# acg-team/ProGraphMSA

Hardware: AMD Instinct MI355X
Metric: DP cell-updates/sec (GCUPS) + wall-clock on 256 seqs × 1000 aa, WAG (higher is better)
Workload: dtype f32

## Files before the change

include/pgm_hip.h:

```cpp
#ifndef PGM_HIP_H_
#define PGM_HIP_H_

#include <stdint.h>
#include <stddef.h>

#ifdef __cplusplus
extern "C" {
#endif

#define PGM_OK 0
#define PGM_ERR_INVALID 1
#define PGM_ERR_DEVICE 2
#define PGM_ERR_BACKTRACK 3
#define PGM_ERR_NOMEM 4

#define PGM_GAP 0xFFFFFFFFu


typedef struct pgm_graph {
    uint32_t n;
    uint32_t dim;
    const double *sites;
    const int32_t *e_rowptr;
    const uint32_t *e_col;
    const float *e_val;
    const int32_t *r_rowptr;
    const uint32_t *r_col;
    const uint32_t *r_units;
} pgm_graph;

typedef struct pgm_model {
    const double *M;
    const double *pi;
} pgm_model;

typedef struct pgm_scores {
    float gap_init, gap_extend, match_init, end_match, end_gap, end_skip;
    float start_gap, start_init, repeat_init, repeat_ext;
} pgm_scores;

typedef struct pgm_align_out {
    float score;
    uint32_t n_tr_indels;
    uint32_t len;
    int32_t status;
    uint32_t *map1;
    uint32_t *map2;
} pgm_align_out;

typedef struct pgm_ctx pgm_ctx;
typedef struct pgm_align_batch pgm_align_batch;

int pgm_device_count(void);
int pgm_ctx_create(int device, pgm_ctx **out);
void pgm_ctx_destroy(pgm_ctx *ctx);
const char *pgm_last_error(void);
int pgm_ctx_device_info(pgm_ctx *ctx, char *name, size_t name_len, int *cu_count);

int pgm_align_graphs_batch(pgm_ctx *ctx, uint32_t njobs, const pgm_graph *const *g1,
                           const pgm_graph *const *g2, const pgm_model *const *model,
                           const pgm_scores *scores, pgm_align_out *out);

int pgm_align_batch_create(pgm_ctx *ctx, uint32_t njobs, const pgm_graph *const *g1,
                           const pgm_graph *const *g2, const pgm_model *const *model,
                           const pgm_scores *scores, pgm_align_batch **out);
#define PGM_BATCH_KEEP_MATRICES 1u
int pgm_align_batch_create_ex(pgm_ctx *ctx, uint32_t njobs, const pgm_graph *const *g1,
                              const pgm_graph *const *g2, const pgm_model *const *model,
                              const pgm_scores *scores, uint32_t flags, pgm_align_batch **out);
typedef struct pgm_site_ref {
    const double *dev_sites;
    const uint32_t *node_map;
    uint32_t ncols;
} pgm_site_ref;
int pgm_align_batch_create_res(pgm_ctx *ctx, uint32_t njobs, const pgm_graph *const *g1,
                               const pgm_graph *const *g2, const pgm_model *const *model,
                               const pgm_scores *scores, uint32_t flags, const pgm_site_ref *res1,
                               const pgm_site_ref *res2, pgm_align_batch **out);
int pgm_align_graphs_batch_res(pgm_ctx *ctx, uint32_t njobs, const pgm_graph *const *g1,
                               const pgm_graph *const *g2, const pgm_model *const *model,
                               const pgm_scores *scores, const pgm_site_ref *res1,
                               const pgm_site_ref *res2, pgm_align_out *out);
int pgm_align_batch_run(pgm_ctx *ctx, pgm_align_batch *b);
int pgm_align_batch_fetch(pgm_ctx *ctx, pgm_align_batch *b, pgm_align_out *out);
void pgm_align_batch_destroy(pgm_ctx *ctx, pgm_align_batch *b);
uint64_t pgm_align_batch_cells(const pgm_align_batch *b);
int pgm_align_batch_time(pgm_ctx *ctx, pgm_align_batch *b, int reps, float *ms_prep,
                         float *ms_emission, float *ms_fill, float *ms_traceback);
int pgm_align_batch_stage_times(pgm_align_batch *b, int reset, float *ms_prep, float *ms_emission, float *ms_fill,
                                uint32_t *launches);
int pgm_align_batch_job_times(pgm_ctx *ctx, pgm_align_batch *b, uint64_t *ticks);
int pgm_align_batch_test_stall(pgm_align_batch *b, uint32_t job, uint32_t band, uint32_t spin_limit);
int pgm_test_cu_shares(uint32_t cus, double lean_cost, uint32_t nlean, double band_cost, uint32_t nbands, double rest_cost,
                       uint32_t nrest, uint32_t ncrit, double longest_chain, uint32_t *out4);
#define PGM_PLAN_HEAD 23
#define PGM_PLAN_DHEAD 9
#define PGM_PLAN_JOB 19
int pgm_test_batch_plan(uint32_t njobs, const pgm_graph *const *g1, const pgm_graph *const *g2, const pgm_model *const *model,
                        const pgm_scores *scores, uint32_t flags, const pgm_site_ref *res1, const pgm_site_ref *res2, uint32_t cus,
                        uint32_t *head, double *dhead, uint32_t *job_fields, uint32_t *items, uint32_t *bands, uint32_t *lean_list, int32_t *tblist);
int pgm_align_batch_read_matrices(pgm_ctx *ctx, pgm_align_batch *b, uint32_t job, float *M,
                                  float *X, float *Y, float *W, float *S);

int pgm_nw_pairs_batch(pgm_ctx *ctx, uint32_t dim, const int32_t *score, int32_t gap_open,
                       int32_t gap_extend, uint32_t nseq, const int8_t *syms,
                       const uint32_t *offs, uint32_t npairs, const uint32_t *pi,
                       const uint32_t *pj, int32_t *counts, uint32_t *gaps);
#define PGM_NW_REDUCED 1u
int pgm_nw_pairs_submit(pgm_ctx *ctx, uint32_t dim, const int32_t *score, int32_t gap_open,
                        int32_t gap_extend, uint32_t nseq, const int8_t *syms,
                        const uint32_t *offs, uint32_t npairs, const uint32_t *pi,
                        const uint32_t *pj, uint32_t flags, int32_t *counts, uint32_t *gaps, int *ticket);
int pgm_nw_pairs_wait(pgm_ctx *ctx, int ticket);
float pgm_nw_last_kernel_ms(pgm_ctx *ctx);
void *pgm_host_alloc(size_t bytes);
void pgm_host_free(void *p);

int pgm_csprofile_load(pgm_ctx *ctx, uint32_t K, uint32_t ncols, const double *lprofiles,
                       const double *centre, const double *priors);
int pgm_csprofile_create_batch(pgm_ctx *ctx, uint32_t nseq, const int8_t *syms,
                               const uint32_t *offs, const double *tau, const double *pi,
                               const double *p_uniform, double *out, const uint64_t *out_offs);
int pgm_csprofile_create_batch_res(pgm_ctx *ctx, uint32_t nseq, const int8_t *syms,
                                   const uint32_t *offs, const double *tau, const double *pi,
                                   const double *p_uniform, const double **dev);
float pgm_csprofile_last_kernel_ms(pgm_ctx *ctx);

typedef struct pgm_mldist_model {
    uint32_t dim;
    const double *Q, *V, *Vi, *sigma;
    double dist_max, var_max, var_min, cutoff_dist, min_dist, max_dist, indel_rate;
    int32_t mldist, mldist_gap;
} pgm_mldist_model;
int pgm_mldist_batch(pgm_ctx *ctx, const pgm_mldist_model *model, uint32_t npairs, const int32_t *counts,
                     const uint32_t *gaps, const double *seqlen, double *dist, double *var);

int pgm_prealigned_counts_batch(pgm_ctx *ctx, uint32_t dim, uint32_t nrows, uint32_t ncols, const int8_t *rows,
                                uint32_t npairs, const uint32_t *pi, const uint32_t *pj, int32_t *counts,
                                uint32_t *gaps);
int pgm_kmer_cosine(pgm_ctx *ctx, uint32_t nseq, uint32_t ncols, const int32_t *counts, double *cosine);
int pgm_kmer_cosine_multi(pgm_ctx *ctx, uint32_t nfam, const uint32_t *nseq, uint32_t ncols, const int32_t *counts, double *cosine);
int pgm_prealigned_counts_multi(pgm_ctx *ctx, uint32_t dim, uint32_t nfam, const uint32_t *nrows, const uint32_t *ncols,
                                const int8_t *rows, uint32_t npairs, const uint32_t *fam, const uint32_t *pi, const uint32_t *pj,
                                int32_t *counts, uint32_t *gaps);
int pgm_prealigned_counts_resampled(pgm_ctx *ctx, uint32_t dim, uint32_t nrows, uint32_t ncols, const int8_t *rows, uint32_t nrep,
                                    const uint32_t *cols, uint32_t npairs, const uint32_t *pi, const uint32_t *pj, int32_t *counts,
                                    uint32_t *gaps);
float pgm_dist_last_kernel_ms(pgm_ctx *ctx);

typedef struct pgm_merge_job {
    uint32_t dim, n1, n2, nnodes;
    const double *sites1, *sites2;
    const double *P1, *P2;
    const uint32_t *k1, *k2;
    const uint8_t *g2_with_P1;
    double *profiles;
} pgm_merge_job;
int pgm_merge_profiles_batch(pgm_ctx *ctx, uint32_t njobs, const pgm_merge_job *jobs);
#define PGM_MERGE_RESIDENT 1u
int pgm_merge_profiles_batch_ex(pgm_ctx *ctx, uint32_t njobs, const pgm_merge_job *jobs, uint32_t flags,
                                const double **dev_profiles);
int pgm_resident_reset(pgm_ctx *ctx);
int pgm_resident_onehot(pgm_ctx *ctx, uint32_t dim, uint32_t nseq, const int8_t *syms, const uint32_t *offs,
                        const double **dev);
int pgm_resident_import(pgm_ctx *ctx, pgm_ctx *src_ctx, const double *src, uint64_t count, const double **dst);
float pgm_merge_last_kernel_ms(pgm_ctx *ctx);


typedef struct pgm_gapmask_job {
    const uint64_t *src;
    const uint32_t *mapping;
    uint64_t *dst;
    uint32_t nrows, ncols_in, ncols_out;
} pgm_gapmask_job;
int pgm_gapmask_extend_batch(pgm_ctx *ctx, uint32_t njobs, const pgm_gapmask_job *jobs);

typedef struct pgm_parsimony_job {
    const uint64_t *masks;
    const uint32_t *children;
    uint32_t nleaves, ncols;
} pgm_parsimony_job;
int pgm_gap_parsimony_batch(pgm_ctx *ctx, uint32_t njobs, const pgm_parsimony_job *jobs, uint32_t *scores);
float pgm_parsimony_last_kernel_ms(pgm_ctx *ctx);

#define PGM_WLS_MAX_N 32768
int pgm_wls_load(pgm_ctx *ctx, uint32_t n, const double *D, const double *W);

#define PGM_WLS_OUT 20
typedef struct pgm_wls_job {
    const int8_t *label;
    const double *offset;
    uint32_t nsub;
} pgm_wls_job;
int pgm_wls_pair_sums_batch(pgm_ctx *ctx, uint32_t njobs, const pgm_wls_job *jobs, double *out);
float pgm_wls_last_kernel_ms(pgm_ctx *ctx);
uint32_t pgm_wls_last_launches(pgm_ctx *ctx);

typedef struct pgm_bionj_join { uint32_t index1, index2; double dist1, dist2; } pgm_bionj_join;
#define PGM_BIONJ_MAX_N 32768
int pgm_bionj(pgm_ctx *ctx, uint32_t n, const double *D, const double *V, pgm_bionj_join *joins, double *final_d);
int pgm_bionj_multi(pgm_ctx *ctx, uint32_t nfam, const uint32_t *n, const double *D, const double *V,
                    pgm_bionj_join *joins, double *final_d);
uint32_t pgm_bionj_last_launches(pgm_ctx *ctx);
float pgm_bionj_last_kernel_ms(pgm_ctx *ctx);

typedef struct pgm_bionj_pair { uint32_t index1, index2; } pgm_bionj_pair;
int pgm_bionj_plan(pgm_ctx *ctx, uint32_t n, const double *D, const double *V, const pgm_bionj_pair *plan,
                   pgm_bionj_join *joins, double *final_d);
int pgm_bionj_plan_multi(pgm_ctx *ctx, uint32_t nfam, const uint32_t *n, const double *D, const double *V,
                         const pgm_bionj_pair *plan, pgm_bionj_join *joins, double *final_d);

int pgm_msa_agreement(pgm_ctx *ctx, uint32_t nrows, uint32_t ncols, uint32_t nrep, const int32_t *where,
                      uint32_t *res_hits , uint32_t *pair_hits );
float pgm_agreement_last_kernel_ms(pgm_ctx *ctx);

int pgm_transfer_min(pgm_ctx *ctx, uint32_t nleaves, uint32_t nref, const uint64_t *ref ,
                     uint32_t nrep, const uint32_t *rep_off ,
                     const uint64_t *rep , uint32_t *phi );
float pgm_transfer_last_kernel_ms(pgm_ctx *ctx);

#define PGM_TRANSFER_NONE 0xffffffffu
int pgm_transfer_taxa(pgm_ctx *ctx, uint32_t nleaves, uint32_t nref, const uint64_t *ref , const uint32_t *thr ,
                      uint32_t nrep, const uint32_t *rep_off , const uint64_t *rep ,
                      uint32_t *phi , uint32_t *arg , uint32_t *moved ,
                      uint32_t *counted );

#ifdef __cplusplus
}
#endif
#endif
```

prographmsa_amd/__init__.py:

```python
import ctypes as C
import os

_HERE = os.path.dirname(os.path.abspath(__file__))
LIB_PATH = os.path.join(_HERE, "lib", "libpgm_hip.so")
PGMSA_PATH = os.path.join(_HERE, "bin", "pgmsa")

PGM_OK, PGM_ERR_INVALID, PGM_ERR_DEVICE, PGM_ERR_BACKTRACK, PGM_ERR_NOMEM = 0, 1, 2, 3, 4
PGM_GAP = 0xFFFFFFFF
PGM_BATCH_KEEP_MATRICES = 1
PGM_NW_REDUCED = 1
PGM_MERGE_RESIDENT = 1


class pgm_graph(C.Structure):
    _fields_ = [("n", C.c_uint32), ("dim", C.c_uint32), ("sites", C.POINTER(C.c_double)),
                ("e_rowptr", C.POINTER(C.c_int32)), ("e_col", C.POINTER(C.c_uint32)), ("e_val", C.POINTER(C.c_float)),
                ("r_rowptr", C.POINTER(C.c_int32)), ("r_col", C.POINTER(C.c_uint32)), ("r_units", C.POINTER(C.c_uint32))]


class pgm_model(C.Structure):
    _fields_ = [("M", C.POINTER(C.c_double)), ("pi", C.POINTER(C.c_double))]


class pgm_scores(C.Structure):
    _fields_ = [(n, C.c_float) for n in ("gap_init", "gap_extend", "match_init", "end_match", "end_gap", "end_skip",
                                         "start_gap", "start_init", "repeat_init", "repeat_ext")]


class pgm_mldist_model(C.Structure):
    _fields_ = [("dim", C.c_uint32), ("Q", C.POINTER(C.c_double)), ("V", C.POINTER(C.c_double)), ("Vi", C.POINTER(C.c_double)),
                ("sigma", C.POINTER(C.c_double))] + [(n, C.c_double) for n in ("dist_max", "var_max", "var_min", "cutoff_dist", "min_dist", "max_dist", "indel_rate")] \
        + [("mldist", C.c_int32), ("mldist_gap", C.c_int32)]


class pgm_merge_job(C.Structure):
    _fields_ = [("dim", C.c_uint32), ("n1", C.c_uint32), ("n2", C.c_uint32), ("nnodes", C.c_uint32),
                ("sites1", C.POINTER(C.c_double)), ("sites2", C.POINTER(C.c_double)), ("P1", C.POINTER(C.c_double)), ("P2", C.POINTER(C.c_double)),
                ("k1", C.POINTER(C.c_uint32)), ("k2", C.POINTER(C.c_uint32)), ("g2_with_P1", C.POINTER(C.c_uint8)), ("profiles", C.POINTER(C.c_double))]


class pgm_site_ref(C.Structure):
    _fields_ = [("dev_sites", C.POINTER(C.c_double)), ("node_map", C.POINTER(C.c_uint32)), ("ncols", C.c_uint32)]


class pgm_gapmask_job(C.Structure):
    _fields_ = [("src", C.POINTER(C.c_uint64)), ("mapping", C.POINTER(C.c_uint32)), ("dst", C.POINTER(C.c_uint64)),
                ("nrows", C.c_uint32), ("ncols_in", C.c_uint32), ("ncols_out", C.c_uint32)]


class pgm_parsimony_job(C.Structure):
    _fields_ = [("masks", C.POINTER(C.c_uint64)), ("children", C.POINTER(C.c_uint32)), ("nleaves", C.c_uint32), ("ncols", C.c_uint32)]


class pgm_wls_job(C.Structure):
    _fields_ = [("label", C.POINTER(C.c_int8)), ("offset", C.POINTER(C.c_double)), ("nsub", C.c_uint32)]


class pgm_bionj_join(C.Structure):
    _fields_ = [("index1", C.c_uint32), ("index2", C.c_uint32), ("dist1", C.c_double), ("dist2", C.c_double)]


class pgm_bionj_pair(C.Structure):
    _fields_ = [("index1", C.c_uint32), ("index2", C.c_uint32)]


class pgm_align_out(C.Structure):
    _fields_ = [("score", C.c_float), ("n_tr_indels", C.c_uint32), ("len", C.c_uint32), ("status", C.c_int32),
                ("map1", C.POINTER(C.c_uint32)), ("map2", C.POINTER(C.c_uint32))]


EXPORTS = [
    "pgm_device_count", "pgm_ctx_create", "pgm_ctx_destroy", "pgm_last_error", "pgm_ctx_device_info",
    "pgm_align_graphs_batch", "pgm_align_batch_create", "pgm_align_batch_create_ex", "pgm_align_batch_create_res", "pgm_align_graphs_batch_res", "pgm_align_batch_run", "pgm_align_batch_fetch",
    "pgm_align_batch_destroy", "pgm_align_batch_cells", "pgm_align_batch_test_stall", "pgm_test_cu_shares", "pgm_test_batch_plan", "pgm_align_batch_stage_times", "pgm_align_batch_job_times", "pgm_align_batch_time", "pgm_align_batch_read_matrices",
    "pgm_nw_pairs_batch", "pgm_nw_pairs_submit", "pgm_nw_pairs_wait", "pgm_nw_last_kernel_ms", "pgm_host_alloc", "pgm_host_free", "pgm_csprofile_load", "pgm_csprofile_create_batch", "pgm_csprofile_create_batch_res",
    "pgm_csprofile_last_kernel_ms", "pgm_mldist_batch", "pgm_prealigned_counts_batch", "pgm_kmer_cosine", "pgm_dist_last_kernel_ms",
    "pgm_kmer_cosine_multi", "pgm_prealigned_counts_multi", "pgm_prealigned_counts_resampled",
    "pgm_merge_profiles_batch", "pgm_merge_profiles_batch_ex", "pgm_resident_reset", "pgm_resident_onehot", "pgm_resident_import", "pgm_merge_last_kernel_ms",
    "pgm_gapmask_extend_batch", "pgm_gap_parsimony_batch", "pgm_parsimony_last_kernel_ms",
    "pgm_wls_load", "pgm_wls_pair_sums_batch", "pgm_wls_last_kernel_ms", "pgm_wls_last_launches",
    "pgm_bionj", "pgm_bionj_multi", "pgm_bionj_last_launches", "pgm_bionj_last_kernel_ms",
    "pgm_bionj_plan", "pgm_bionj_plan_multi",
    "pgm_msa_agreement", "pgm_agreement_last_kernel_ms",
    "pgm_transfer_min", "pgm_transfer_last_kernel_ms", "pgm_transfer_taxa",
]


def _load():
    if not os.path.exists(LIB_PATH):
        raise ImportError("libpgm_hip.so is not built (%s); run `python -c 'import __graft_entry__ as g; g.build()'` "
                          "— there is no CPU fallback for the hot path" % LIB_PATH)
    lib = C.CDLL(LIB_PATH)
    vp, u32, i32 = C.c_void_p, C.c_uint32, C.c_int32
    PG, PM = C.POINTER(C.POINTER(pgm_graph)), C.POINTER(C.POINTER(pgm_model))
    sig = {
        "pgm_device_count": (C.c_int, []),
        "pgm_ctx_create": (C.c_int, [C.c_int, C.POINTER(vp)]),
        "pgm_ctx_destroy": (None, [vp]),
        "pgm_last_error": (C.c_char_p, []),
        "pgm_ctx_device_info": (C.c_int, [vp, C.c_char_p, C.c_size_t, C.POINTER(C.c_int)]),
        "pgm_align_graphs_batch": (C.c_int, [vp, u32, PG, PG, PM, C.POINTER(pgm_scores), C.POINTER(pgm_align_out)]),
        "pgm_align_batch_create": (C.c_int, [vp, u32, PG, PG, PM, C.POINTER(pgm_scores), C.POINTER(vp)]),
        "pgm_align_batch_create_ex": (C.c_int, [vp, u32, PG, PG, PM, C.POINTER(pgm_scores), u32, C.POINTER(vp)]),
        "pgm_align_batch_create_res": (C.c_int, [vp, u32, PG, PG, PM, C.POINTER(pgm_scores), u32, C.POINTER(pgm_site_ref), C.POINTER(pgm_site_ref), C.POINTER(vp)]),
        "pgm_align_graphs_batch_res": (C.c_int, [vp, u32, PG, PG, PM, C.POINTER(pgm_scores), C.POINTER(pgm_site_ref), C.POINTER(pgm_site_ref), C.POINTER(pgm_align_out)]),
        "pgm_align_batch_run": (C.c_int, [vp, vp]),
        "pgm_align_batch_fetch": (C.c_int, [vp, vp, C.POINTER(pgm_align_out)]),
        "pgm_align_batch_destroy": (None, [vp, vp]),
        "pgm_align_batch_cells": (C.c_uint64, [vp]),
        "pgm_align_batch_test_stall": (C.c_int, [vp, u32, u32, u32]),
        "pgm_test_cu_shares": (C.c_int, [u32, C.c_double, u32, C.c_double, u32, C.c_double, u32, u32, C.c_double, C.POINTER(C.c_uint32)]),
        "pgm_test_batch_plan": (C.c_int, [u32, PG, PG, PM, C.POINTER(pgm_scores), u32, C.POINTER(pgm_site_ref), C.POINTER(pgm_site_ref), u32,
                                          C.POINTER(u32), C.POINTER(C.c_double)] + [C.POINTER(u32)] * 4 + [C.POINTER(i32)]),
        "pgm_align_batch_stage_times": (C.c_int, [vp, C.c_int] + [C.POINTER(C.c_float)] * 3 + [C.POINTER(u32)]),
        "pgm_align_batch_job_times": (C.c_int, [vp, vp, C.POINTER(C.c_uint64)]),
        "pgm_align_batch_time": (C.c_int, [vp, vp, C.c_int] + [C.POINTER(C.c_float)] * 4),
        "pgm_align_batch_read_matrices": (C.c_int, [vp, vp, u32] + [C.POINTER(C.c_float)] * 5),
        "pgm_nw_pairs_batch": (C.c_int, [vp, u32, C.POINTER(i32), i32, i32, u32, C.POINTER(C.c_int8), C.POINTER(u32), u32,
                                         C.POINTER(u32), C.POINTER(u32), C.POINTER(i32), C.POINTER(u32)]),
        "pgm_nw_pairs_submit": (C.c_int, [vp, u32, C.POINTER(i32), i32, i32, u32, C.POINTER(C.c_int8), C.POINTER(u32), u32,
                                          C.POINTER(u32), C.POINTER(u32), u32, C.POINTER(i32), C.POINTER(u32), C.POINTER(C.c_int)]),
        "pgm_nw_pairs_wait": (C.c_int, [vp, C.c_int]),
        "pgm_host_alloc": (vp, [C.c_size_t]),
        "pgm_host_free": (None, [vp]),
        "pgm_nw_last_kernel_ms": (C.c_float, [vp]),
        "pgm_csprofile_load": (C.c_int, [vp, u32, u32] + [C.POINTER(C.c_double)] * 3),
        "pgm_csprofile_create_batch": (C.c_int, [vp, u32, C.POINTER(C.c_int8), C.POINTER(u32)] + [C.POINTER(C.c_double)] * 4
                                       + [C.POINTER(C.c_uint64)]),
        "pgm_csprofile_create_batch_res": (C.c_int, [vp, u32, C.POINTER(C.c_int8), C.POINTER(u32)] + [C.POINTER(C.c_double)] * 3
                                           + [C.POINTER(C.POINTER(C.c_double))]),
        "pgm_csprofile_last_kernel_ms": (C.c_float, [vp]),
        "pgm_mldist_batch": (C.c_int, [vp, C.POINTER(pgm_mldist_model), u32, C.POINTER(i32), C.POINTER(u32)] + [C.POINTER(C.c_double)] * 3),
        "pgm_prealigned_counts_batch": (C.c_int, [vp, u32, u32, u32, C.POINTER(C.c_int8), u32, C.POINTER(u32), C.POINTER(u32), C.POINTER(i32), C.POINTER(u32)]),
        "pgm_kmer_cosine": (C.c_int, [vp, u32, u32, C.POINTER(i32), C.POINTER(C.c_double)]),
        "pgm_dist_last_kernel_ms": (C.c_float, [vp]),
        "pgm_kmer_cosine_multi": (C.c_int, [vp, u32, C.POINTER(u32), u32, C.POINTER(i32), C.POINTER(C.c_double)]),
        "pgm_prealigned_counts_multi": (C.c_int, [vp, u32, u32, C.POINTER(u32), C.POINTER(u32), C.POINTER(C.c_int8), u32, C.POINTER(u32), C.POINTER(u32),
                                                  C.POINTER(u32), C.POINTER(i32), C.POINTER(u32)]),
        "pgm_prealigned_counts_resampled": (C.c_int, [vp, u32, u32, u32, C.POINTER(C.c_int8), u32, C.POINTER(u32), u32, C.POINTER(u32), C.POINTER(u32),
                                                      C.POINTER(i32), C.POINTER(u32)]),
        "pgm_merge_profiles_batch": (C.c_int, [vp, u32, C.POINTER(pgm_merge_job)]),
        "pgm_merge_profiles_batch_ex": (C.c_int, [vp, u32, C.POINTER(pgm_merge_job), u32, C.POINTER(C.POINTER(C.c_double))]),
        "pgm_resident_reset": (C.c_int, [vp]),
        "pgm_resident_onehot": (C.c_int, [vp, u32, u32, C.POINTER(C.c_int8), C.POINTER(u32), C.POINTER(C.POINTER(C.c_double))]),
        "pgm_resident_import": (C.c_int, [vp, vp, C.POINTER(C.c_double), C.c_uint64, C.POINTER(C.POINTER(C.c_double))]),
        "pgm_merge_last_kernel_ms": (C.c_float, [vp]),
        "pgm_gapmask_extend_batch": (C.c_int, [vp, u32, C.POINTER(pgm_gapmask_job)]),
        "pgm_gap_parsimony_batch": (C.c_int, [vp, u32, C.POINTER(pgm_parsimony_job), C.POINTER(u32)]),
        "pgm_parsimony_last_kernel_ms": (C.c_float, [vp]),
        "pgm_wls_load": (C.c_int, [vp, u32, C.POINTER(C.c_double), C.POINTER(C.c_double)]),
        "pgm_wls_pair_sums_batch": (C.c_int, [vp, u32, C.POINTER(pgm_wls_job), C.POINTER(C.c_double)]),
        "pgm_wls_last_kernel_ms": (C.c_float, [vp]),
        "pgm_wls_last_launches": (C.c_uint32, [vp]),
        "pgm_bionj": (C.c_int, [vp, u32, C.POINTER(C.c_double), C.POINTER(C.c_double), C.POINTER(pgm_bionj_join), C.POINTER(C.c_double)]),
        "pgm_bionj_multi": (C.c_int, [vp, u32, C.POINTER(u32), C.POINTER(C.c_double), C.POINTER(C.c_double), C.POINTER(pgm_bionj_join), C.POINTER(C.c_double)]),
        "pgm_bionj_last_launches": (C.c_uint32, [vp]),
        "pgm_bionj_last_kernel_ms": (C.c_float, [vp]),
        "pgm_bionj_plan": (C.c_int, [vp, u32, C.POINTER(C.c_double), C.POINTER(C.c_double), C.POINTER(pgm_bionj_pair), C.POINTER(pgm_bionj_join), C.POINTER(C.c_double)]),
        "pgm_bionj_plan_multi": (C.c_int, [vp, u32, C.POINTER(u32), C.POINTER(C.c_double), C.POINTER(C.c_double), C.POINTER(pgm_bionj_pair), C.POINTER(pgm_bionj_join), C.POINTER(C.c_double)]),
        "pgm_msa_agreement": (C.c_int, [vp, u32, u32, u32, C.POINTER(i32), C.POINTER(u32), C.POINTER(u32)]),
        "pgm_agreement_last_kernel_ms": (C.c_float, [vp]),
        "pgm_transfer_min": (C.c_int, [vp, u32, u32, C.POINTER(C.c_uint64), u32, C.POINTER(u32), C.POINTER(C.c_uint64), C.POINTER(u32)]),
        "pgm_transfer_last_kernel_ms": (C.c_float, [vp]),
        "pgm_transfer_taxa": (C.c_int, [vp, u32, u32, C.POINTER(C.c_uint64), C.POINTER(u32), u32, C.POINTER(u32), C.POINTER(C.c_uint64),
                                        C.POINTER(u32), C.POINTER(u32), C.POINTER(u32), C.POINTER(u32)]),
    }
    for name, (res, args) in sig.items():
        fn = getattr(lib, name)
        fn.restype = res
        fn.argtypes = args
    return lib


lib = _load()


class PgmError(RuntimeError):
    pass


def check(rc, what="libpgm_hip"):
    if rc != PGM_OK:
        raise PgmError("%s failed (%d): %s" % (what, rc, lib.pgm_last_error().decode()))


class Context:

    def __init__(self, device=0):
        self.handle = C.c_void_p()
        check(lib.pgm_ctx_create(device, C.byref(self.handle)), "pgm_ctx_create")

    def device_info(self):
        buf = C.create_string_buffer(256)
        cu = C.c_int()
        check(lib.pgm_ctx_device_info(self.handle, buf, 256, C.byref(cu)))
        return buf.value.decode(), cu.value

    def prealigned_counts_resampled(self, dim, rows, cols, pi, pj):
        import numpy as np
        rows = np.ascontiguousarray(rows, np.int8)
        cols = np.ascontiguousarray(cols, np.uint32)
        pi = np.ascontiguousarray(pi, np.uint32)
        pj = np.ascontiguousarray(pj, np.uint32)
        nrep, npairs = cols.shape[0], len(pi)
        counts = np.zeros((nrep, npairs, dim * dim), np.int32)
        gaps = np.zeros((nrep, npairs), np.uint32)
        P = lambda a, t: a.ctypes.data_as(C.POINTER(t))
        check(lib.pgm_prealigned_counts_resampled(self.handle, dim, rows.shape[0], rows.shape[1], P(rows, C.c_int8), nrep, P(cols, C.c_uint32), npairs,
                                                  P(pi, C.c_uint32), P(pj, C.c_uint32), P(counts, C.c_int32), P(gaps, C.c_uint32)), "pgm_prealigned_counts_resampled")
        return counts, gaps

    def msa_agreement(self, where, res_hits=None, pair_hits=None):
        import numpy as np
        where = np.ascontiguousarray(where, np.int32)
        nrep, nrows, ncols = where.shape
        if res_hits is None: res_hits = np.zeros((nrows, ncols), np.uint32)
        if pair_hits is None: pair_hits = np.zeros((nrows, nrows), np.uint32)
        for o, shape in ((res_hits, (nrows, ncols)), (pair_hits, (nrows, nrows))):
            if o.dtype != np.uint32 or o.shape != shape or not o.flags.c_contiguous: raise ValueError("msa_agreement: output array of the wrong kind")
        P = lambda a, t: a.ctypes.data_as(C.POINTER(t))
        check(lib.pgm_msa_agreement(self.handle, nrows, ncols, nrep, P(where, C.c_int32), P(res_hits, C.c_uint32), P(pair_hits, C.c_uint32)), "pgm_msa_agreement")
        return res_hits, pair_hits

    def transfer_min(self, nleaves, ref, rep_off, rep, phi=None):
        import numpy as np
        words = (nleaves + 63) // 64
        ref = np.ascontiguousarray(ref, np.uint64)
        rep_off = np.ascontiguousarray(rep_off, np.uint32)
        rep = np.ascontiguousarray(rep, np.uint64).reshape(-1, words)
        if ref.ndim != 2 or ref.shape[1] != words or rep_off.ndim != 1 or len(rep_off) < 1 or rep.shape[0] != int(rep_off[-1]):
            raise ValueError("transfer_min: input array of the wrong shape")
        nref, nrep = ref.shape[0], len(rep_off) - 1
        if phi is None: phi = np.zeros((nref, nrep), np.uint32)
        if phi.dtype != np.uint32 or phi.shape != (nref, nrep) or not phi.flags.c_contiguous: raise ValueError("transfer_min: output array of the wrong kind")
        P = lambda a, t: a.ctypes.data_as(C.POINTER(t))
        check(lib.pgm_transfer_min(self.handle, nleaves, nref, P(ref, C.c_uint64), nrep, P(rep_off, C.c_uint32), P(rep, C.c_uint64) if rep.size else None,
                                   P(phi, C.c_uint32)), "pgm_transfer_min")
        return phi

    def transfer_taxa(self, nleaves, ref, thr, rep_off, rep, out=None):
        import numpy as np
        words = (nleaves + 63) // 64
        ref = np.ascontiguousarray(ref, np.uint64)
        thr = np.ascontiguousarray(thr, np.uint32)
        rep_off = np.ascontiguousarray(rep_off, np.uint32)
        rep = np.ascontiguousarray(rep, np.uint64).reshape(-1, words)
        if ref.ndim != 2 or ref.shape[1] != words or thr.shape != (ref.shape[0],) or rep_off.ndim != 1 or len(rep_off) < 1 or rep.shape[0] != int(rep_off[-1]):
            raise ValueError("transfer_taxa: input array of the wrong shape")
        nref, nrep = ref.shape[0], len(rep_off) - 1
        shapes = [(nref, nrep), (nref, nrep), (nref, nleaves), (nref,)]
        if out is None: out = tuple(np.zeros(s, np.uint32) for s in shapes)
        if len(out) != 4 or any(a.dtype != np.uint32 or a.shape != s or not a.flags.c_contiguous for a, s in zip(out, shapes)):
            raise ValueError("transfer_taxa: output array of the wrong kind")
        P = lambda a, t: a.ctypes.data_as(C.POINTER(t))
        check(lib.pgm_transfer_taxa(self.handle, nleaves, nref, P(ref, C.c_uint64), P(thr, C.c_uint32), nrep, P(rep_off, C.c_uint32),
                                    P(rep, C.c_uint64) if rep.size else None, *[P(a, C.c_uint32) for a in out]), "pgm_transfer_taxa")
        return tuple(out)

    def close(self):
        if self.handle:
            lib.pgm_ctx_destroy(self.handle)
            self.handle = C.c_void_p()

    def __del__(self):
        try:
            self.close()
        except Exception:
            pass
```

prographmsa_amd/csrc/pgm_align_kernels.h:

```cpp
#ifndef PGM_ALIGN_KERNELS_H_
#define PGM_ALIGN_KERNELS_H_

#include <hip/hip_runtime.h>
#include <math.h>
#include <type_traits>
#include "pgm_device.h"

#define PGM_NEG_INF (-INFINITY)

__device__ __forceinline__ float pgm_ls_log_add(float x, float add) {
    const float a = 2.44247459618085927548717403238913328776812604856113966238617812902399112761292613763080658235564f;
    const float b = -4.2040783745848554315883301529007786406310628696382695994938550046831869207082846248658671f;
    const float c = -0.72123729809042963774358701619456664388406302428056983119308906451199556380646306f;
    const uint32_t bits = __float_as_uint(x);
    const float e = (float)((int32_t)(bits >> 23) - 126);
    const float d = __uint_as_float(((bits << 9) >> 9) ^ 0x3f000000u);
    float t = __fdiv_rn(b, __fsub_rn(d, c));
    const float u = __fadd_rn(e, a);
    t = __fadd_rn(t, add);
    t = __fadd_rn(t, u);
    return t;
}

__device__ __forceinline__ float pgm_emission_finish(float num, float ay, float bx, float match_init) {
    float q = __fdiv_rn(num, __fmul_rn(ay, bx));
    if (q != q) q = __uint_as_float(0xFFC00000u);
    return pgm_ls_log_add(q, match_init);
}

template <int DMAX, int NODES>
__global__ void __launch_bounds__(NODES) pgm_prep_kernel(const PgmJob *__restrict__ jobs, int *__restrict__ sync, uint32_t sync_ints) {
    extern __shared__ float prep_lds[];
    {
        const uint32_t nthreads = gridDim.x * gridDim.y * gridDim.z * NODES;
        const uint32_t gid = ((blockIdx.z * gridDim.y + blockIdx.y) * gridDim.x + blockIdx.x) * NODES + threadIdx.x;
        for (uint32_t i = gid; i < sync_ints; i += nthreads) sync[i] = 0;
    }
    const PgmJob &J = jobs[blockIdx.x];
    const bool first = blockIdx.y == 0;
    const uint32_t n = first ? J.n1 : J.n2;
    const uint32_t v0 = blockIdx.z * NODES;
    if (v0 >= n) return;
    if (J.tabhdr && J.tabhdr[0] == 0) {
        const uint32_t nc = J.dim + 2u;
        bool any = n - 1u >= v0 && n - 1u < v0 + (uint32_t)NODES;
        for (uint32_t c = 0; c < nc; ++c) {
            const uint32_t r = (uint32_t)J.tabhdr[1u + (first ? 0u : nc) + c];
            any = any || (r != 0u && r - 1u >= v0 && r - 1u < v0 + (uint32_t)NODES);
        }
        if (!any) return;
    }
    const uint32_t D = J.dim, DP = J.dp, ST = D + 1;
    float *Mf = prep_lds;
    float *pif = prep_lds + D * D;
    float *nl = pif + D;
    const uint32_t nn = min((uint32_t)NODES, n - v0);
    {
        const int32_t *pp = first ? J.pp1 : J.pp2;
        const uint32_t *pc = first ? J.pc1 : J.pc2, *pu = first ? J.pu1 : J.pu2;
        const float *pv = first ? J.pv1 : J.pv2;
        PgmTbNode *rec = (first ? J.tb1 : J.tb2) + v0;
        for (uint32_t i = threadIdx.x; i < nn * PGM_TB_PK; i += NODES) {
            const uint32_t node = i / PGM_TB_PK, k = i % PGM_TB_PK;
            const int32_t eb = pp[v0 + node];
            const uint32_t cnt = (uint32_t)(pp[v0 + node + 1] - eb);
            const int32_t e = cnt == 0u ? 0 : eb + (int32_t)min(k, cnt - 1u);
            if (k == 0) rec[node].cnt = cnt;
            rec[node].c[k] = pc[e]; rec[node].v[k] = pv[e]; rec[node].u[k] = pu[e];
        }
    }
    if (!first) for (uint32_t i = threadIdx.x; i < D * D; i += NODES) Mf[i] = (float)J.M[i];
    for (uint32_t i = threadIdx.x; i < D; i += NODES) pif[i] = (float)J.pi[i];
    const double *sites = first ? J.sites1 : J.sites2;
    const uint32_t *smap = first ? J.smap1 : J.smap2;
    float *dst = (first ? J.g1f : J.t2) + (size_t)DP * v0;
    for (uint32_t i = threadIdx.x; i < nn * D; i += NODES) {
        const uint32_t node = v0 + i / D;
        const float g = (float)sites[(size_t)D * (smap ? smap[node] : node) + i % D];
        nl[(i / D) * ST + (i % D)] = g;
        if (first && DP == D) dst[i] = g;
    }
    __syncthreads();
    const uint32_t v = threadIdx.x;
    float g[DMAX];
    float acc = 0.0f;
    if (v < nn) {
#pragma unroll
        for (int k = 0; k < DMAX; ++k) g[k] = ((uint32_t)k < D) ? nl[v * ST + k] : 0.0f;
        float l0 = 0.0f, l1 = 0.0f, l2 = 0.0f, l3 = 0.0f;
        const uint32_t aligned = D / 4u * 4u;
#pragma unroll
        for (int k = 0; k + 3 < DMAX; k += 4) {
            if ((uint32_t)k < aligned) {
                l0 = __fadd_rn(l0, __fmul_rn(g[k], pif[k]));
                l1 = __fadd_rn(l1, __fmul_rn(g[k + 1], pif[k + 1]));
                l2 = __fadd_rn(l2, __fmul_rn(g[k + 2], pif[k + 2]));
                l3 = __fadd_rn(l3, __fmul_rn(g[k + 3], pif[k + 3]));
            }
        }
        acc = __fadd_rn(0.0f, __fadd_rn(__fadd_rn(l0, l2), __fadd_rn(l1, l3)));
#pragma unroll
        for (int k = 0; k < DMAX; ++k)
            if ((uint32_t)k >= aligned && (uint32_t)k < D) acc = __fadd_rn(acc, __fmul_rn(g[k], pif[k]));
        (first ? J.a1 : J.b2)[v0 + v] = acc;
    }
    if (first) {
        if (DP != D && v < nn) {
#pragma unroll
            for (int k = 0; k < DMAX; ++k) if ((uint32_t)k < DP) dst[(size_t)DP * v + k] = g[k];
        }
        return;
    }
    __syncthreads();
    if (v < nn) {
        for (uint32_t k = 0; k < D; ++k) {
            float t = 0.0f;
#pragma unroll
            for (int j = 0; j < DMAX; ++j)
                if ((uint32_t)j < D) t = __fadd_rn(t, __fmul_rn(Mf[j + D * k], g[j]));
            nl[v * ST + k] = t;
        }
    }
    __syncthreads();
    for (uint32_t i = threadIdx.x; i < nn * DP; i += NODES) {
        const uint32_t node = i / DP, k = i % DP;
        dst[i] = k < D ? nl[node * ST + k] : 0.0f;
    }
}

#define PGM_TAB_HDR 136
__global__ void __launch_bounds__(256) pgm_classify_kernel(const PgmJob *__restrict__ jobs) {
    const PgmJob &J = jobs[blockIdx.x];
    if (!J.tabhdr) return;
    const bool first = blockIdx.y == 0;
    const uint32_t n = first ? J.n1 : J.n2, D = J.dim;
    const double *sites = first ? J.sites1 : J.sites2;
    const uint32_t *smap = first ? J.smap1 : J.smap2;
    uint8_t *cls = (uint8_t *)(first ? J.cls1 : J.cls2);
    const float uni = (float)(1.0 / (double)D);
    for (uint32_t v = blockIdx.z * blockDim.x + threadIdx.x; v < n; v += gridDim.z * blockDim.x) {
        const double *col = sites + (size_t)D * (smap ? smap[v] : v);
        uint32_t nz = 0, sym = 0;
        bool same = true;
        float vs = 0.f;
        const float g0 = (float)col[0];
        for (uint32_t k = 0; k < D; ++k) {
            const float g = (float)col[k];
            if (g != 0.0f) { ++nz; sym = k; vs = g; }
            same = same && g == g0;
        }
        uint32_t c = 255u;
        if (nz == 0u) c = D + 1u;
        else if (nz == 1u && vs == 1.0f) c = sym;
        else if (same && g0 == uni) c = D;
        cls[v] = (uint8_t)c;
        if (c == 255u) atomicOr(J.tabhdr, 1);
        else atomicCAS(J.tabhdr + 1 + (first ? 0u : D + 2u) + c, 0, (int)v + 1);
    }
}

__device__ __forceinline__ size_t pgm_cell_index(const PgmJob &J, uint32_t y, uint32_t x) {
    const uint32_t b = y / PGM_ROWS, l = PGM_HALO + (y - b * PGM_ROWS);
    return ((size_t)b * J.tsteps + (x + l)) * 64u + l;
}
__device__ __forceinline__ float4 pgm_load_cell(const PgmJob &J, uint32_t y, uint32_t x) {
    return J.cells[pgm_cell_index(J, y, x)];
}

__device__ __forceinline__ float pgm_dpp_wave_shr1(float src, float lane0_value) {
    return __int_as_float(__builtin_amdgcn_update_dpp(__float_as_int(lane0_value), __float_as_int(src), 0x138, 0xf, 0xf, false));
}

#define PGM_GLOBAL __attribute__((address_space(1)))
typedef float pgm_v4f __attribute__((ext_vector_type(4)));
template <class T> __device__ __forceinline__ T pgm_gld(const T *p) { return *(const PGM_GLOBAL T *)(uintptr_t)p; }
#define PGM_EM_TB 4
template <int DP, int RB>
__global__ void __launch_bounds__(4 * PGM_ROWS) pgm_emission_skew_kernel(const PgmJob *__restrict__ jobs) {
    typedef float pgm_v2f __attribute__((ext_vector_type(2)));
    constexpr int NT = DP / 4;
    constexpr int COLS = 64 + PGM_EM_TB * PGM_BLOCK - PGM_HALO - 1;
    constexpr int STR = DP + 1;
    __shared__ pgm_v2f tp[(COLS + 1) * STR];
    __shared__ float bq[COLS];
    const PgmJob &J = jobs[blockIdx.z];
    const uint32_t tb0 = blockIdx.x * PGM_EM_TB;
    const uint32_t rsh = J.rshift, nvb = J.nb << rsh;
    if (tb0 >= J.nblk || 4u * RB * blockIdx.y >= nvb) return;
    if (J.tabhdr && pgm_gld(J.tabhdr) == 0) return;
    auto row_of = [&](uint32_t v, uint32_t lane_) { return ((((v >> rsh) << 6) + lane_) << rsh) | (v & ((1u << rsh) - 1u)); };
    auto sblock_of = [&](uint32_t v, uint32_t tb_) { return ((((size_t)(v >> rsh) * J.nblk + tb_) << rsh) | (v & ((1u << rsh) - 1u))); };
    const uint32_t t0 = tb0 * PGM_BLOCK;
    const int cbase = (int)t0 - 63;
    if ((DP == 20 || DP == 4) && RB == 1) {
        constexpr int TE = DP + 1;
        float *const tab = (float *)tp;
        static_assert(COLS * TE <= (COLS + 1) * STR * 2, "score table must fit the column staging area");
        static_assert(DP > 20 || TE <= 32, "row classes must fit As");
        __shared__ float As[32];
        const uint32_t fb0 = 4u * blockIdx.y + threadIdx.x / PGM_ROWS;
        const uint32_t fl = threadIdx.x % PGM_ROWS;
        const bool active = fb0 < nvb;
        int sym = DP;
        bool plain = true;
        float a_row = 0.f;
        if (active) {
            const uint32_t y = row_of(fb0, fl);
            const uint32_t yc = (y + 1 < J.n1) ? y : 0u;
            const float4 *src = (const float4 *)(J.g1f + (size_t)DP * yc);
            int nz = 0;
#pragma unroll
            for (int q = 0; q < NT; ++q) {
                const float4 v = src[q];
                const float vv[4] = {v.x, v.y, v.z, v.w};
#pragma unroll
                for (int u = 0; u < 4; ++u)
                    if (vv[u] != 0.0f) { ++nz; sym = 4 * q + u; plain = plain && vv[u] == 1.0f; }
            }
            plain = plain && nz <= 1;
            a_row = J.a1[yc];
        }
        if (threadIdx.x < 32) As[threadIdx.x] = 0.f;
        if (__syncthreads_and(plain ? 1 : 0)) {
            if (active) As[sym] = a_row;
            __syncthreads();
            const float mi = J.sc.match_init;
            constexpr int NE = (COLS * TE + 4 * PGM_ROWS - 1) / (4 * PGM_ROWS);
            float tt[NE], tb2[NE];
#pragma unroll
            for (int e = 0; e < NE; ++e) {
                const int i = (int)threadIdx.x + e * 4 * PGM_ROWS;
                const int ci = i / TE, k = i % TE, c = cbase + ci;
                const bool in = i < COLS * TE && c >= 0 && c <= (int)J.ncol;
                tb2[e] = in ? J.b2[c] : 0.f;
                tt[e] = (in && k < DP) ? J.t2[(size_t)DP * c + k] : 0.f;
            }
#pragma unroll
            for (int e = 0; e < NE; ++e) {
                const int i = (int)threadIdx.x + e * 4 * PGM_ROWS;
                if (i < COLS * TE) tab[i] = pgm_emission_finish(0.0f + tt[e], As[i % TE], tb2[e], mi);
            }
            __syncthreads();
            if (!active) return;
            PGM_GLOBAL pgm_v4f *const Sq = (PGM_GLOBAL pgm_v4f *)(uintptr_t)J.S;
            const int l = PGM_HALO + (int)fl;
#pragma unroll 1
            for (int w = 0; w < PGM_EM_TB; ++w) {
                const uint32_t tb = tb0 + w;
                if (tb >= J.nblk) break;
                float out[PGM_BLOCK];
#pragma unroll
                for (int i = 0; i < PGM_BLOCK; ++i) out[i] = tab[((int)(tb * PGM_BLOCK) + i - l - cbase) * TE + sym];
                PGM_GLOBAL pgm_v4f *dst = Sq + (sblock_of(fb0, tb) * 64u + (uint32_t)l) * (PGM_BLOCK / 4);
#pragma unroll
                for (int q = 0; q < PGM_BLOCK / 4; ++q) dst[q] = pgm_v4f{out[4 * q], out[4 * q + 1], out[4 * q + 2], out[4 * q + 3]};
            }
            return;
        }
    }
    const float4 *t2q = (const float4 *)J.t2;
    float *tpf = (float *)tp;
    for (int i = threadIdx.x; i < (COLS + 1) * NT; i += 4 * PGM_ROWS) {
        const int ci = i / NT, q = i % NT, c = cbase + ci;
        float4 v = make_float4(0.f, 0.f, 0.f, 0.f);
        if (c >= 0 && c <= (int)J.ncol) v = t2q[(size_t)NT * c + q];
        const float vv[4] = {v.x, v.y, v.z, v.w};
#pragma unroll
        for (int u = 0; u < 4; ++u) {
            const int k = 4 * q + u;
            if (ci < COLS) tpf[2 * (ci * STR + k)] = vv[u];
            if (ci > 0) tpf[2 * ((ci - 1) * STR + k) + 1] = vv[u];
        }
    }
    for (int i = threadIdx.x; i < COLS; i += 4 * PGM_ROWS) {
        const int col = cbase + i;
        bq[i] = (col >= 0 && col <= (int)J.ncol) ? J.b2[col] : 0.f;
    }
    __syncthreads();
    const uint32_t b0 = (4u * blockIdx.y + threadIdx.x / PGM_ROWS) * RB;
    const int l = PGM_HALO + (int)(threadIdx.x % PGM_ROWS);
    if (b0 >= nvb) return;
    float gy[RB][DP], ay[RB];
#pragma unroll
    for (int r = 0; r < RB; ++r) {
        const uint32_t y = row_of(b0 + (uint32_t)r, (uint32_t)(l - PGM_HALO));
        const uint32_t yc = (y + 1 < J.n1) ? y : 0u;
        const float4 *src = (const float4 *)(J.g1f + (size_t)DP * yc);
#pragma unroll
        for (int q = 0; q < NT; ++q) {
            const float4 v = src[q];
            gy[r][4 * q] = v.x; gy[r][4 * q + 1] = v.y; gy[r][4 * q + 2] = v.z; gy[r][4 * q + 3] = v.w;
        }
        ay[r] = J.a1[yc];
    }
    const float mi = J.sc.match_init;
    const uint32_t nblk = J.nblk;
    PGM_GLOBAL pgm_v4f *const Sq = (PGM_GLOBAL pgm_v4f *)(uintptr_t)J.S;
#pragma unroll 1
    for (int w = 0; w < PGM_EM_TB; ++w) {
        const uint32_t tb = tb0 + w;
        if (tb >= nblk) break;
        float out[RB][PGM_BLOCK];
#pragma unroll
        for (int i = 0; i < PGM_BLOCK; i += 2) {
            const int ci = (int)(tb * PGM_BLOCK) + i - l - cbase;
            const pgm_v2f *tc = tp + ci * STR;
            pgm_v2f acc[RB];
#pragma unroll
            for (int r = 0; r < RB; ++r) acc[r] = pgm_v2f{0.0f, 0.0f};
#pragma unroll
            for (int k = 0; k < DP; ++k) {
                const pgm_v2f tk = tc[k];
#pragma unroll
                for (int r = 0; r < RB; ++r) {
                    const pgm_v2f g = {gy[r][k], gy[r][k]};
                    acc[r] = acc[r] + g * tk;
                }
            }
#pragma unroll
            for (int r = 0; r < RB; ++r) {
                out[r][i] = pgm_emission_finish(acc[r].x, ay[r], bq[ci], mi);
                out[r][i + 1] = pgm_emission_finish(acc[r].y, ay[r], bq[ci + 1], mi);
            }
        }
#pragma unroll
        for (int r = 0; r < RB; ++r) {
            if (b0 + (uint32_t)r < nvb) {
                PGM_GLOBAL pgm_v4f *dst = Sq + (sblock_of(b0 + (uint32_t)r, tb) * 64u + (uint32_t)l) * (PGM_BLOCK / 4);
#pragma unroll
                for (int q = 0; q < PGM_BLOCK / 4; ++q) dst[q] = pgm_v4f{out[r][4 * q], out[r][4 * q + 1], out[r][4 * q + 2], out[r][4 * q + 3]};
            }
        }
    }
}

__device__ __forceinline__ int pgm_wave_max8(uint32_t v) {
    int m = __builtin_amdgcn_ballot_w64(v >= 8u) != 0 ? 8 : 0;
    m += __builtin_amdgcn_ballot_w64(v >= (uint32_t)(m + 4)) != 0 ? 4 : 0;
    m += __builtin_amdgcn_ballot_w64(v >= (uint32_t)(m + 2)) != 0 ? 2 : 0;
    m += __builtin_amdgcn_ballot_w64(v >= (uint32_t)(m + 1)) != 0 ? 1 : 0;
    return m;
}

__device__ __forceinline__ __amdgpu_buffer_rsrc_t pgm_band_rsrc(float4 *base, uint32_t bytes) {
    const uint64_t p = (uint64_t)base;
    const uint32_t lo = __builtin_amdgcn_readfirstlane((uint32_t)p), hi = __builtin_amdgcn_readfirstlane((uint32_t)(p >> 32));
    return __builtin_amdgcn_make_buffer_rsrc((void *)(((uint64_t)hi << 32) | lo), 0, __builtin_amdgcn_readfirstlane(bytes), 0x00020000);
}
__device__ __forceinline__ void pgm_store_cell_masked(__amdgpu_buffer_rsrc_t rsrc, uint32_t t, int lane, bool on, float Mv, float Xv, float Wv, float Yv) {
    typedef uint32_t pgm_v4u __attribute__((ext_vector_type(4)));
    pgm_v4u v;
    v.x = __float_as_uint(Mv); v.y = __float_as_uint(Xv); v.z = __float_as_uint(Wv); v.w = __float_as_uint(Yv);
    __builtin_amdgcn_raw_buffer_store_b128(v, rsrc, (on ? (uint32_t)lane * 16u : 0x80000000u) + t * 1024u, 0, 16);
}
__device__ __forceinline__ float4 pgm_gload4(const float4 *p) {
    const pgm_v4f v = *(const PGM_GLOBAL pgm_v4f *)(uintptr_t)p;
    return make_float4(v.x, v.y, v.z, v.w);
}
__device__ __forceinline__ float2 pgm_gload_cell_wy(const float4 *p) {
    const unsigned long long v = __hip_atomic_load((const PGM_GLOBAL unsigned long long *)(uintptr_t)p + 1, __ATOMIC_RELAXED, __HIP_MEMORY_SCOPE_AGENT);
    return make_float2(__uint_as_float((uint32_t)v), __uint_as_float((uint32_t)(v >> 32)));
}
__device__ __forceinline__ float2 pgm_load_cell_mx(const float4 *p) {
    const unsigned long long v = __hip_atomic_load((const PGM_GLOBAL unsigned long long *)(uintptr_t)p, __ATOMIC_RELAXED, __HIP_MEMORY_SCOPE_AGENT);
    return make_float2(__uint_as_float((uint32_t)v), __uint_as_float((uint32_t)(v >> 32)));
}
__device__ __forceinline__ float2 pgm_load_cell_wy(const float4 *p) {
    const unsigned long long v = __hip_atomic_load((const PGM_GLOBAL unsigned long long *)(uintptr_t)p + 1, __ATOMIC_RELAXED, __HIP_MEMORY_SCOPE_AGENT);
    return make_float2(__uint_as_float((uint32_t)v), __uint_as_float((uint32_t)(v >> 32)));
}

struct PgmPred {
    const int32_t *pp; const uint32_t *pc; const float *pv; const uint32_t *pu;
};
__device__ __forceinline__ float pgm_mark_value(const PgmPred &P, int32_t e) {
    const uint32_t u = P.pu[e];
    if (u == 0) return P.pv[e];
    const uint32_t units = u & 0x7fffffffu;
    if (units == 0) return INFINITY;
    return __fadd_rn(INFINITY, __fmul_rn(INFINITY, (float)(units - 1)));
}

struct PgmMapOut {
    uint32_t *m1, *m2;
    uint32_t len, cap;
    __device__ __forceinline__ void push(uint32_t y, uint32_t x) {
        if (len < cap) { m1[len] = y; m2[len] = x; }
        ++len;
    }
};

__device__ static void pgm_mark_alternative_path(const PgmJob &J, uint32_t start, uint32_t end, const PgmPred &P, PgmMapOut &mo, bool first) {
    const uint32_t len = end - start + 1;
    float *score = J.mark_score;
    uint32_t *prev = J.mark_prev;
    for (uint32_t i = 0; i < len; ++i) { score[i] = PGM_NEG_INF; prev[i] = 0xFFFFFFFFu; }
    score[0] = 0.0f;
    for (uint32_t i = 1; i < len; ++i) {
        const uint32_t real_ix = i + start;
        for (int32_t e = P.pp[real_ix]; e < P.pp[real_ix + 1]; ++e) {
            const uint32_t p = P.pc[e];
            if (p >= start && p <= end) {
                const uint32_t i2 = p - start;
                const float cand = __fsub_rn(score[i2], pgm_mark_value(P, e));
                if (score[i] <= cand) { score[i] = cand; prev[i] = i2; }
            }
        }
    }
    if (score[len - 1] > PGM_NEG_INF) {
        uint32_t i = prev[len - 1];
        while (i != 0) {
            if (first) mo.push(i + start, 0xFFFFFFFFu); else mo.push(0xFFFFFFFFu, i + start);
            i = prev[i];
        }
    }
}

__device__ __forceinline__ float pgm_emission_at(const PgmJob &J, uint32_t y, uint32_t x) {
    const uint32_t b = y / PGM_ROWS, l = PGM_HALO + (y - b * PGM_ROWS), t = x + l;
    return J.S[(((size_t)b * J.nblk + (t / PGM_BLOCK)) * 64u + l) * PGM_BLOCK + (t % PGM_BLOCK)];
}

#define PGM_TB_T 32
#define PGM_TB_BAND 6
#define PGM_TB_LK 4
struct PgmTbLds {
    float4 cell[PGM_TB_T * PGM_TB_T];
    float S[PGM_TB_T * PGM_TB_T];
    uint32_t p_cnt[2 * PGM_TB_T];
    uint32_t p_c[2 * PGM_TB_T * PGM_TB_PK];
    float p_v[2 * PGM_TB_T * PGM_TB_PK];
    uint32_t p_u[2 * PGM_TB_T * PGM_TB_PK];
    uint16_t succ[3 * PGM_TB_T * PGM_TB_T];
    uint32_t ty0, tx0;
    uint32_t ay, ax;
    int req;
    uint32_t len;
    int nbig;
    uint16_t big[128];
    uint16_t gtab[PGM_LK_NR][PGM_LK_W * PGM_LK_TAB] __attribute__((aligned(16)));
    uint2 mbuf[64];
    uint32_t grow, gcnt;
    uint32_t gnext[PGM_LK_NR];
};

#define PGM_LK_HW (PGM_LK_T + PGM_LK_H)
struct PgmLkLds {
    float4 cell[PGM_LK_HW * PGM_LK_HW];
    float S[PGM_LK_T * PGM_LK_T];
    uint32_t p_cnt[2 * PGM_LK_T];
    uint32_t p_c[2 * PGM_LK_T * PGM_TB_PK];
    float p_v[2 * PGM_LK_T * PGM_TB_PK];
    uint32_t p_u[2 * PGM_LK_T * PGM_TB_PK];
    uint16_t tab[PGM_LK_TAB] __attribute__((aligned(16)));
    int nbig;
    uint16_t big[PGM_LK_T * PGM_LK_T];
};
__device__ __forceinline__ uint16_t pgm_lk_code(uint32_t st, uint32_t dy, uint32_t dx) { return (uint16_t)(0x8000u | (st << 12) | (dy << 6) | dx); }

struct PgmPredView {
    uint32_t cnt;
    bool lds;
    uint32_t base;
};

__device__ static void pgm_traceback_publish(const PgmJob &J, const uint32_t len, const int tid, const int nthreads) {
    for (uint32_t i = (uint32_t)tid; i < len; i += (uint32_t)nthreads) {
        const uint32_t j = len - 1 - i;
        J.hmap1[i] = J.map1[j];
        J.hmap2[i] = J.map2[j];
    }
    __threadfence_system();
    __syncthreads();
    if (tid == 0) {
        const PgmJob::Result r = *J.result;
        J.hresult->score = r.score; J.hresult->n_tr_indels = r.n_tr_indels; J.hresult->len = r.len;
        __threadfence_system();
        __hip_atomic_store(&J.hresult->status, r.status, __ATOMIC_RELEASE, __HIP_MEMORY_SCOPE_SYSTEM);
    }
}

__device__ __attribute__((noinline)) static void pgm_traceback_job(const PgmJob &J, PgmTbLds &T, const int tid, const int nthreads,
                                         int *lq, int *lq_ids, const uint32_t jid) {
    constexpr uint32_t TT = PGM_TB_T;
    const uint32_t n1 = J.n1, n2 = J.n2;

    const PgmPred P1 = {J.pp1, J.pc1, J.pv1, J.pu1};
    const PgmPred P2 = {J.pp2, J.pc2, J.pv2, J.pu2};

    const bool loader = tid >= 64;
    auto stage = [&]() {
        const uint32_t ty0 = T.ty0, tx0 = T.tx0;
        constexpr uint32_t NT = 64u * PGM_WAVES;
        constexpr int NC = (int)((TT * TT) / NT), NP = (int)((2 * TT * PGM_TB_PK) / NT);
        static_assert(NC * NT == TT * TT && NP * NT == 2 * TT * PGM_TB_PK, "tile staging: whole rounds of the workgroup");
        float4 cv[NC];
        float sv[NC];
        uint32_t cslot[NC];
#pragma unroll
        for (int u = 0; u < NC; ++u) {
            const uint32_t i = (uint32_t)tid + NT * u;
            const uint32_t half = TT * (TT + 1u) / 2u;
            const bool up = i < half;
            const uint32_t m = up ? i : TT * TT - 1u - i;
            uint32_t d = (uint32_t)((sqrtf(8.0f * (float)m + 1.0f) - 1.0f) * 0.5f);
            while (d * (d + 1u) / 2u > m) --d;
            while ((d + 1u) * (d + 2u) / 2u <= m) ++d;
            const uint32_t k = m - d * (d + 1u) / 2u;
            const uint32_t ly = up ? k : TT - 1u - k, lx = up ? d - k : TT - 1u - (d - k);
            cslot[u] = ly * TT + lx;
            const uint32_t yy = min(ty0 + ly, n1 - 2), xx = min(tx0 + lx, n2 - 2);
            cv[u] = J.cells[pgm_cell_index(J, yy, xx)];
            const uint32_t ys = min(ty0 + i / TT, n1 - 2), xs = min(tx0 + i % TT, n2 - 2);
            sv[u] = pgm_emission_at(J, ys, xs);
        }
        uint32_t cnt[NP], ec[NP], eu[NP];
        float ev[NP];
#pragma unroll
        for (int u = 0; u < NP; ++u) {
            const uint32_t i = (uint32_t)tid + NT * u, slot = i / PGM_TB_PK, k = i % PGM_TB_PK;
            const bool row = slot < TT;
            const uint32_t v = min(row ? ty0 + slot : tx0 + (slot - TT), (row ? n1 : n2) - 1);
            const PgmTbNode *r = (row ? J.tb1 : J.tb2) + v;
            cnt[u] = r->cnt; ec[u] = r->c[k]; ev[u] = r->v[k]; eu[u] = r->u[k];
        }
#pragma unroll
        for (int u = 0; u < NC; ++u) {
            const uint32_t i = (uint32_t)tid + NT * u;
            T.cell[cslot[u]] = cv[u];
            T.S[i] = sv[u];
        }
        for (uint32_t i = (uint32_t)tid; i < 3u * TT * TT / 2u; i += NT) ((uint32_t *)T.succ)[i] = 0u;
        if (tid == 0) T.nbig = 0;
#pragma unroll
        for (int u = 0; u < NP; ++u) {
            const uint32_t i = (uint32_t)tid + NT * u, slot = i / PGM_TB_PK, k = i % PGM_TB_PK;
            const bool row = slot < TT;
            const bool inr = (row ? ty0 + slot : tx0 + (slot - TT)) < (row ? n1 : n2);
            if (k == 0) T.p_cnt[slot] = inr ? cnt[u] : 0xFFFFFFFFu;
            T.p_c[i] = ec[u]; T.p_v[i] = ev[u]; T.p_u[i] = eu[u];
        }
    };
    const pgm_scores sc = J.sc;
    const int band = J.has_extras ? PGM_TB_BAND : PGM_TB_BAND / 2;
    auto links = [&]() {
        const uint32_t ty0 = T.ty0, tx0 = T.tx0;
        const int adiag = (int)(T.ay - ty0) - (int)(T.ax - tx0);
        const uint32_t NDIAG = 2u * (uint32_t)band + 1u;
        for (uint32_t task = (uint32_t)tid; task < 3u * NDIAG * TT; task += (uint32_t)nthreads) {
            const uint32_t lx = task % TT, st_task = task / (NDIAG * TT);
            const int lyi = (int)lx + adiag + (int)((task / TT) % NDIAG) - band;
            if (lyi < 0 || lyi >= (int)TT) continue;
            const uint32_t ly = (uint32_t)lyi, ci = ly * TT + lx, y = ty0 + ly, x = tx0 + lx;
            uint16_t lm = 0, lxs = 0, lys = 0;
            if (y + 1 < n1 && x + 1 < n2 && (y | x) != 0u) {
                const float4 c0 = T.cell[ci];
                const uint32_t cy = T.p_cnt[ly], cx = T.p_cnt[TT + lx];
                auto pick = [&](const float4 &c, uint32_t yp, uint32_t xp) -> uint16_t {
                    uint32_t st;
                    if ((yp | xp) == 0u) st = 0u;
                    else if (c.z == c.x) st = 0u;
                    else if (c.z == c.w) st = 2u;
                    else if (c.z == c.y) st = 1u;
                    else return (uint16_t)0;
                    return (uint16_t)(0x8000u | (st << 10) | ((yp - ty0) << 5) | (xp - tx0));
                };
                const int doff = (int)((task / TT) % NDIAG) - band;
                if (st_task == 0u && doff >= -1 && doff <= 1 && (cy > PGM_TB_LK || cx > PGM_TB_LK) && cy <= PGM_TB_PK && cx <= PGM_TB_PK && cy != 0u && cx != 0u && c0.x > PGM_NEG_INF) {
                    const int slot = __hip_atomic_fetch_add(&T.nbig, 1, __ATOMIC_RELAXED, __HIP_MEMORY_SCOPE_WORKGROUP);
                    if (slot < 128) T.big[slot] = (uint16_t)ci;
                }
                if (st_task == 0u && cy <= PGM_TB_LK && cx <= PGM_TB_LK && cy != 0u && cx != 0u && c0.x > PGM_NEG_INF) {
                    const float S = T.S[ci];
                    uint32_t yp[PGM_TB_LK], xp[PGM_TB_LK];
                    float yv[PGM_TB_LK], xv[PGM_TB_LK];
                    bool ok = true;
#pragma unroll
                    for (int k = 0; k < PGM_TB_LK; ++k) {
                        yp[k] = T.p_c[ly * PGM_TB_PK + k]; yv[k] = T.p_v[ly * PGM_TB_PK + k];
                        xp[k] = T.p_c[(TT + lx) * PGM_TB_PK + k]; xv[k] = T.p_v[(TT + lx) * PGM_TB_PK + k];
                        ok = ok && ((uint32_t)k >= cy || yp[k] >= ty0) && ((uint32_t)k >= cx || xp[k] >= tx0);
                    }
                    float wz[PGM_TB_LK][PGM_TB_LK];
#pragma unroll
                    for (int ky = 0; ky < PGM_TB_LK; ++ky)
#pragma unroll
                        for (int kx = 0; kx < PGM_TB_LK; ++kx)
                            wz[ky][kx] = T.cell[min((yp[ky] - ty0) * TT + (xp[kx] - tx0), TT * TT - 1u)].z;
                    float best = INFINITY;
                    uint32_t wy = 0, wx = 0, wky = 0, wkx = 0;
#pragma unroll
                    for (int ky = 0; ky < PGM_TB_LK; ++ky)
#pragma unroll
                        for (int kx = 0; kx < PGM_TB_LK; ++kx) {
                            const float d = fabsf(__fsub_rn(c0.x, __fsub_rn(__fsub_rn(__fadd_rn(wz[ky][kx], S), yv[ky]), xv[kx])));
                            if ((uint32_t)ky < cy && (uint32_t)kx < cx && best > d) { best = d; wy = yp[ky]; wx = xp[kx]; wky = ky; wkx = kx; }
                        }
                    bool rep_edge = false;
                    float4 wc = c0;
                    if (ok && best < INFINITY) {
                        rep_edge = (T.p_u[ly * PGM_TB_PK + wky] | T.p_u[(TT + lx) * PGM_TB_PK + wkx]) != 0u;
                        wc = T.cell[(wy - ty0) * TT + (wx - tx0)];
                    }
                    if (ok && best < INFINITY && !rep_edge) lm = pick(wc, wy, wx);
                }
                if (st_task == 2u && cy == 1u && c0.w > PGM_NEG_INF) {
                    float best = INFINITY;
                    bool ok = true, rep_edge = false, open = false;
                    uint32_t wy = 0;
                    float4 wc = c0;
                    for (uint32_t k = 0; k < cy; ++k) {
                        const uint32_t yp = T.p_c[ly * PGM_TB_PK + k];
                        if (yp < ty0) { ok = false; break; }
                        const float yv = T.p_v[ly * PGM_TB_PK + k];
                        const float4 c = T.cell[(yp - ty0) * TT + lx];
                        const bool ru = T.p_u[ly * PGM_TB_PK + k] != 0u;
                        float d = fabsf(__fsub_rn(c0.w, __fsub_rn(__fadd_rn(c.w, sc.gap_extend), yv)));
                        if (best > d) { best = d; wy = yp; wc = c; rep_edge = ru; open = false; }
                        d = fabsf(__fsub_rn(c0.w, __fsub_rn(__fadd_rn(c.z, sc.gap_init), yv)));
                        if (best > d) { best = d; wy = yp; wc = c; rep_edge = ru; open = true; }
                    }
                    if (ok && best < INFINITY && !rep_edge)
                        lys = open ? pick(wc, wy, x) : (uint16_t)(0x8000u | (2u << 10) | ((wy - ty0) << 5) | lx);
                }
                if (st_task == 1u && cx == 1u && c0.y > PGM_NEG_INF) {
                    float best = INFINITY;
                    bool ok = true, rep_edge = false, open = false;
                    uint32_t wx = 0;
                    float4 wc = c0;
                    for (uint32_t k = 0; k < cx; ++k) {
                        const uint32_t xp = T.p_c[(TT + lx) * PGM_TB_PK + k];
                        if (xp < tx0) { ok = false; break; }
                        const float xv = T.p_v[(TT + lx) * PGM_TB_PK + k];
                        const float4 c = T.cell[ly * TT + (xp - tx0)];
                        const bool ru = T.p_u[(TT + lx) * PGM_TB_PK + k] != 0u;
// ... 1960 lines not shown
```

prographmsa_amd/csrc/pgm_capi.hip:

```cpp
#include <hip/hip_runtime.h>

#include <algorithm>
#include <cmath>
#include <cstdio>
#include <thread>
#include <atomic>
#include <chrono>
#include <queue>
#include <cstdlib>
#include <cstring>
#include <numeric>
#include <mutex>
#include <string>
#include <unordered_set>
#include <vector>
#include <sys/mman.h>

#include "pgm_align_kernels.h"
#include "pgm_crit_kernels.h"
#include "pgm_nw_kernels.h"
#include "pgm_csprofile_kernels.h"
#include "pgm_dist_kernels.h"
#include "pgm_merge_kernels.h"
#include "pgm_parsimony_kernels.h"
#include "pgm_wls_kernels.h"
#include "pgm_bionj_kernels.h"
#include "pgm_agreement_kernels.h"
#include "pgm_transfer_kernels.h"
#include "pgm_pool.h"
#include "pgm_plan.h"
static_assert(kC3Bytes == PGM_C3_BYTES, "pgm_plan.h plans the LDS of a crit3 sweep with PGM_C3_BYTES");

static thread_local std::string g_err;
static int fail(int code, const std::string &m) { g_err = m; return code; }
#define HIPCHK(x)                                                                                   \
    do {                                                                                            \
        hipError_t e_ = (x);                                                                        \
        if (e_ != hipSuccess)                                                                       \
            return fail(PGM_ERR_DEVICE, std::string(#x) + ": " + hipGetErrorString(e_));            \
    } while (0)

struct PgmNwState;
struct pgm_ctx {
    int device = 0;
    PgmNwState *nw = nullptr;
    int nw_per_cu = 0;
    struct ResChunk { uint8_t *p; size_t cap; };
    std::vector<ResChunk> res_chunks;
    size_t res_chunk = 0, res_off = 0;
    hipStream_t stream = nullptr;
    hipStream_t stream2 = nullptr;
    hipStream_t stream3 = nullptr;
    hipStream_t stream4 = nullptr;
    enum { C_IN, C_WORK, C_CELLS, C_OUT, C_S, C_HOST, C_HIN, C_SMALL, C_SLOTS };
    void *cache_ptr[C_SLOTS] = {};
    size_t cache_bytes[C_SLOTS] = {};
    hipDeviceProp_t prop;
    float nw_ms = 0, cs_ms = 0, ml_ms = 0, merge_ms = 0, pars_ms = 0, wls_ms = 0;
    uint32_t wls_n = 0, wls_launches = 0;
    float bionj_ms = 0;
    float agree_ms = 0;
    float transfer_ms = 0;
    uint32_t bionj_launches = 0;
    enum { SC_DEV = 36, SC_HOST = 4 };
    void *sc_dev[SC_DEV] = {};
    size_t sc_dev_bytes[SC_DEV] = {};
    void *sc_host[SC_HOST] = {};
    size_t sc_host_bytes[SC_HOST] = {};
    hipEvent_t sc_ev[2] = {nullptr, nullptr};
    uint32_t csK = 0, csC = 0;
    double *cs_lprofiles = nullptr, *cs_centre = nullptr, *cs_priors = nullptr;
};

static pgm_pool::Pool &lib_pool() {
    static pgm_pool::Pool pool(std::max(1u, std::min(16u, std::thread::hardware_concurrency())));
    return pool;
}

static std::mutex g_pinned_mu;
static std::unordered_set<void *> g_pinned_registered;
static hipError_t pinned_alloc(size_t bytes, void **out) {
    const size_t H = (size_t)2 << 20, len = (std::max<size_t>(bytes, 1) + H - 1) / H * H;
    void *p = getenv("PGM_PINNED_MALLOC") ? nullptr : aligned_alloc(H, len);
    if (p) {
        (void)madvise(p, len, MADV_HUGEPAGE);
        (void)lib_pool().run(len / H, len >= 8 * H ? 16u : 1u, [&](size_t c) { for (size_t o = 0; o < H; o += 4096) ((volatile char *)p)[c * H + o] = 0; });
        if (hipHostRegister(p, len, hipHostRegisterDefault) == hipSuccess) {
            std::lock_guard<std::mutex> g(g_pinned_mu);
            g_pinned_registered.insert(p);
            *out = p;
            return hipSuccess;
        }
        (void)hipGetLastError();
        free(p);
    }
    return hipHostMalloc(out, bytes, hipHostMallocDefault);
}
static void pinned_free(void *p) {
    if (!p) return;
    bool reg;
    { std::lock_guard<std::mutex> g(g_pinned_mu); reg = g_pinned_registered.erase(p) != 0; }
    if (reg) { (void)hipHostUnregister(p); free(p); }
    else (void)hipHostFree(p);
}
static void slot_free(int slot, void *p) {
    if (slot == pgm_ctx::C_HIN) pinned_free(p);
    else if (slot == pgm_ctx::C_HOST) (void)hipHostFree(p);
    else (void)hipFree(p);
}

struct pgm_align_batch {
    uint32_t njobs = 0;
    uint64_t cells = 0;
    uint32_t maxdim = 0, maxnb = 0, maxn = 0, maxnblk = 0;
    std::vector<PgmJob> jobs;
    std::vector<uint32_t> order;
    BatchSchedule sched;
    uint8_t *d_in = nullptr;
    uint8_t *d_work = nullptr;
    uint8_t *d_cells = nullptr;
    uint8_t *d_out = nullptr;
    uint8_t *d_S = nullptr;
    uint8_t *d_small = nullptr;
    size_t in_bytes = 0, work_bytes = 0, cell_bytes = 0, out_bytes = 0, s_bytes = 0, small_bytes = 0;
    size_t cap[8] = {0, 0, 0, 0, 0, 0, 0, 0};
    uint8_t *h_out = nullptr;
    uint8_t *h_in = nullptr;
    int *h_flag = nullptr;
    int *d_sync = nullptr;
    size_t sync_ints = 0;
    uint32_t lq_off = 0;
    PgmJob *d_jobs = nullptr;
    uint32_t *d_order = nullptr;
    PgmItem *d_items = nullptr;
    uint32_t *d_lean = nullptr;
    PgmItem *d_bands = nullptr;
    int2 *d_tblist = nullptr;
    unsigned long long *d_times = nullptr;
    int *d_tabhdr = nullptr;
    hipEvent_t ev_fork = nullptr, ev_join = nullptr;
    hipEvent_t ev_join_b = nullptr, ev_join_c = nullptr;
    uint32_t test_spin_limit = 0, test_stall_job = 0xFFFFFFFFu, test_stall_band = 0;
    double acc_ms[3] = {0, 0, 0};
    uint32_t acc_n = 0;
    bool ev_pending = false;
    std::vector<size_t> res_off, map1_off, map2_off;
    hipEvent_t ev[5] = {nullptr, nullptr, nullptr, nullptr, nullptr};
};
static const struct BatchBuffer { int slot; size_t reserve_mb; uint8_t *pgm_align_batch::*ptr; size_t pgm_align_batch::*bytes; } kBatchBuffers[6] = {
    {pgm_ctx::C_IN, 128, &pgm_align_batch::d_in, &pgm_align_batch::in_bytes}, {pgm_ctx::C_WORK, 256, &pgm_align_batch::d_work, &pgm_align_batch::work_bytes},
    {pgm_ctx::C_CELLS, 2048, &pgm_align_batch::d_cells, &pgm_align_batch::cell_bytes}, {pgm_ctx::C_OUT, 8, &pgm_align_batch::d_out, &pgm_align_batch::out_bytes},
    {pgm_ctx::C_S, 1024, &pgm_align_batch::d_S, &pgm_align_batch::s_bytes}, {pgm_ctx::C_SMALL, 4, &pgm_align_batch::d_small, &pgm_align_batch::small_bytes}};

extern "C" {

const char *pgm_last_error(void) { return g_err.c_str(); }

int pgm_device_count(void) {
    int n = 0;
    if (hipGetDeviceCount(&n) != hipSuccess) return 0;
    return n;
}

__global__ void pgm_warm_kernel() {}

int pgm_ctx_create(int device, pgm_ctx **out) {
    if (!out) return fail(PGM_ERR_INVALID, "null out");
    *out = nullptr;
    int n = 0;
    HIPCHK(hipGetDeviceCount(&n));
    if (device < 0 || device >= n) return fail(PGM_ERR_DEVICE, "no such HIP device");
    HIPCHK(hipSetDevice(device));
    pgm_ctx *c = new pgm_ctx;
    c->device = device;
    HIPCHK(hipGetDeviceProperties(&c->prop, device));
    HIPCHK(hipStreamCreateWithFlags(&c->stream, hipStreamNonBlocking));
    HIPCHK(hipStreamCreateWithFlags(&c->stream2, hipStreamNonBlocking));
    HIPCHK(hipStreamCreateWithFlags(&c->stream3, hipStreamNonBlocking));
    {
        int lo = 0, hi = 0;
        if (hipDeviceGetStreamPriorityRange(&lo, &hi) != hipSuccess) { (void)hipGetLastError(); lo = hi = 0; }
        if (hipStreamCreateWithPriority(&c->stream4, hipStreamNonBlocking, hi) != hipSuccess) {
            (void)hipGetLastError();
            HIPCHK(hipStreamCreateWithFlags(&c->stream4, hipStreamNonBlocking));
        }
    }
    hipLaunchKernelGGL(pgm_warm_kernel, dim3(1), dim3(64), 0, c->stream);
    HIPCHK(hipGetLastError());
    HIPCHK(hipStreamSynchronize(c->stream));
    {
        void *h = nullptr, *d = nullptr;
        const size_t wb = (size_t)1 << 20;
        if (hipHostMalloc(&h, wb, hipHostMallocDefault) == hipSuccess && hipMalloc(&d, wb) == hipSuccess) {
            (void)hipMemcpyAsync(d, h, wb, hipMemcpyHostToDevice, c->stream);
            (void)hipMemcpyAsync(h, d, wb, hipMemcpyDeviceToHost, c->stream);
            (void)hipStreamSynchronize(c->stream);
        }
        if (h) (void)hipHostFree(h);
        if (d) (void)hipFree(d);
    }
    (void)lib_pool().run(64, 16u, [](size_t) {});
    {
        void *p = nullptr;
        const size_t sb = (size_t)128 << 20;
        if (!getenv("PGM_NO_STAGING_RESERVE") && pinned_alloc(sb, &p) == hipSuccess) { c->cache_ptr[pgm_ctx::C_HIN] = p; c->cache_bytes[pgm_ctx::C_HIN] = sb; }
        else (void)hipGetLastError();
        const size_t rb = (size_t)8 << 20;
        if (!getenv("PGM_NO_STAGING_RESERVE") && hipHostMalloc(&p, rb, hipHostMallocDefault) == hipSuccess) { c->cache_ptr[pgm_ctx::C_HOST] = p; c->cache_bytes[pgm_ctx::C_HOST] = rb; }
        else (void)hipGetLastError();
        if (!getenv("PGM_NO_STAGING_RESERVE") && !getenv("PGM_NO_DEVICE_RESERVE")) {
            for (const BatchBuffer &e : kBatchBuffers) {
                void *d = nullptr;
                if (hipMalloc(&d, e.reserve_mb << 20) == hipSuccess) { c->cache_ptr[e.slot] = d; c->cache_bytes[e.slot] = e.reserve_mb << 20; }
                else { (void)hipGetLastError(); break; }
            }
        }
    }
    *out = c;
    return PGM_OK;
}

static void nw_state_free(PgmNwState *st);
void pgm_ctx_destroy(pgm_ctx *ctx) {
    if (!ctx) return;
    (void)hipSetDevice(ctx->device);
    nw_state_free(ctx->nw);
    for (auto &c : ctx->res_chunks) if (c.p) (void)hipFree(c.p);
    if (ctx->cs_lprofiles) (void)hipFree(ctx->cs_lprofiles);
    if (ctx->cs_centre) (void)hipFree(ctx->cs_centre);
    if (ctx->cs_priors) (void)hipFree(ctx->cs_priors);
    for (int k = 0; k < pgm_ctx::SC_DEV; ++k) if (ctx->sc_dev[k]) (void)hipFree(ctx->sc_dev[k]);
    for (int k = 0; k < pgm_ctx::SC_HOST; ++k) if (ctx->sc_host[k]) pinned_free(ctx->sc_host[k]);
    for (int k = 0; k < 2; ++k) if (ctx->sc_ev[k]) (void)hipEventDestroy(ctx->sc_ev[k]);
    for (int k = 0; k < pgm_ctx::C_SLOTS; ++k)
        if (ctx->cache_ptr[k]) slot_free(k, ctx->cache_ptr[k]);
    if (ctx->stream4) (void)hipStreamDestroy(ctx->stream4);
    if (ctx->stream3) (void)hipStreamDestroy(ctx->stream3);
    if (ctx->stream2) (void)hipStreamDestroy(ctx->stream2);
    if (ctx->stream) (void)hipStreamDestroy(ctx->stream);
    delete ctx;
}

int pgm_ctx_device_info(pgm_ctx *ctx, char *name, size_t name_len, int *cu_count) {
    if (!ctx) return fail(PGM_ERR_INVALID, "null ctx");
    if (name && name_len) snprintf(name, name_len, "%s (%s)", ctx->prop.name, ctx->prop.gcnArchName);
    if (cu_count) *cu_count = ctx->prop.multiProcessorCount;
    return PGM_OK;
}

}

namespace {
static hipError_t cache_take(pgm_ctx *ctx, int slot, size_t bytes, void **out, size_t *got) {
    if (ctx->cache_ptr[slot] && ctx->cache_bytes[slot] >= bytes) {
        *out = ctx->cache_ptr[slot]; *got = ctx->cache_bytes[slot];
        ctx->cache_ptr[slot] = nullptr; ctx->cache_bytes[slot] = 0;
        return hipSuccess;
    }
    if (ctx->cache_ptr[slot]) {
        slot_free(slot, ctx->cache_ptr[slot]);
        ctx->cache_ptr[slot] = nullptr; ctx->cache_bytes[slot] = 0;
    }
    *got = bytes;
    if (slot == pgm_ctx::C_HIN) return pinned_alloc(bytes, out);
    return slot == pgm_ctx::C_HOST ? hipHostMalloc(out, bytes, hipHostMallocDefault) : hipMalloc(out, bytes);
}
static void cache_give(pgm_ctx *ctx, int slot, void *p, size_t bytes) {
    if (!p) return;
    if (ctx && (!ctx->cache_ptr[slot] || ctx->cache_bytes[slot] < bytes)) {
        if (ctx->cache_ptr[slot]) slot_free(slot, ctx->cache_ptr[slot]);
        ctx->cache_ptr[slot] = p; ctx->cache_bytes[slot] = bytes;
    } else {
        slot_free(slot, p);
    }
}

static hipError_t scratch_dev(pgm_ctx *ctx, int slot, size_t bytes, void **out) {
    bytes = std::max<size_t>(bytes, 16);
    if (ctx->sc_dev_bytes[slot] < bytes) {
        if (ctx->sc_dev[slot]) (void)hipFree(ctx->sc_dev[slot]);
        ctx->sc_dev[slot] = nullptr; ctx->sc_dev_bytes[slot] = 0;
        const size_t want = bytes + bytes / 4;
        hipError_t e = hipMalloc(&ctx->sc_dev[slot], want);
        if (e != hipSuccess) return e;
        ctx->sc_dev_bytes[slot] = want;
    }
    *out = ctx->sc_dev[slot];
    return hipSuccess;
}
static hipError_t scratch_host(pgm_ctx *ctx, int slot, size_t bytes, void **out) {
    bytes = std::max<size_t>(bytes, 16);
    if (ctx->sc_host_bytes[slot] < bytes) {
        if (ctx->sc_host[slot]) pinned_free(ctx->sc_host[slot]);
        ctx->sc_host[slot] = nullptr; ctx->sc_host_bytes[slot] = 0;
        const size_t want = bytes + bytes / 4;
        hipError_t e = pinned_alloc(want, &ctx->sc_host[slot]);
        if (e != hipSuccess) return e;
        ctx->sc_host_bytes[slot] = want;
    }
    *out = ctx->sc_host[slot];
    return hipSuccess;
}
static hipError_t scratch_events(pgm_ctx *ctx) {
    for (int k = 0; k < 2; ++k)
        if (!ctx->sc_ev[k]) { hipError_t e = hipEventCreate(&ctx->sc_ev[k]); if (e != hipSuccess) return e; }
    return hipSuccess;
}

static hipError_t classify_lean_jobs(pgm_ctx *ctx, pgm_align_batch *b) {
    if (!b->d_tabhdr || b->njobs == 0) return hipSuccess;
    hipError_t e = hipMemsetAsync(b->d_tabhdr, 0, 4 * (size_t)PGM_TAB_HDR * b->njobs, ctx->stream);
    if (e != hipSuccess) return e;
    hipLaunchKernelGGL(pgm_classify_kernel, dim3(b->njobs, 2, (b->maxn + 1023) / 1024), dim3(256), 0, ctx->stream, b->d_jobs);
    return hipGetLastError();
}

#define PGM_STATUS_PENDING 0x7ffffff0
struct PrepTier { uint32_t tier, threads; size_t lds; };
static PrepTier prep_tier(uint32_t maxdim) {
    const uint32_t tier = alphabet_tier(maxdim), threads = tier == 64u ? 64u : 256u;
    return {tier, threads, ((size_t)maxdim * maxdim + maxdim + threads * ((size_t)maxdim + 1)) * sizeof(float)};
}
static hipError_t launch_all(pgm_ctx *ctx, pgm_align_batch *b, bool timed) {
    hipStream_t s = ctx->stream;
    const BatchSchedule &S = b->sched;
    hipError_t e;
    for (uint32_t i = 0; i < b->njobs; ++i) ((PgmJob::Result *)(b->h_out + b->res_off[i]))->status = PGM_STATUS_PENDING;
    if (timed && (e = hipEventRecord(b->ev[0], s)) != hipSuccess) return e;
    const PrepTier T = prep_tier(b->maxdim);
    const dim3 pg(b->njobs, 2, (b->maxn + T.threads - 1) / T.threads);
    if (T.tier == 4) hipLaunchKernelGGL((pgm_prep_kernel<4, 256>), pg, dim3(256), T.lds, s, b->d_jobs, b->d_sync, (uint32_t)b->sync_ints);
    else if (T.tier == 20) hipLaunchKernelGGL((pgm_prep_kernel<20, 256>), pg, dim3(256), T.lds, s, b->d_jobs, b->d_sync, (uint32_t)b->sync_ints);
    else hipLaunchKernelGGL((pgm_prep_kernel<64, 64>), pg, dim3(64), T.lds, s, b->d_jobs, b->d_sync, (uint32_t)b->sync_ints);
    if ((e = hipGetLastError()) != hipSuccess) return e;
    if (timed && (e = hipEventRecord(b->ev[1], s)) != hipSuccess) return e;
    const dim3 eg((b->maxnblk + PGM_EM_TB - 1) / PGM_EM_TB, (b->maxnb + 3) / 4, b->njobs);
    if (T.tier == 4) hipLaunchKernelGGL((pgm_emission_skew_kernel<4, 1>), eg, dim3(4 * PGM_ROWS), 0, s, b->d_jobs);
    else if (T.tier == 20) hipLaunchKernelGGL((pgm_emission_skew_kernel<20, 1>), eg, dim3(4 * PGM_ROWS), 0, s, b->d_jobs);
    else hipLaunchKernelGGL((pgm_emission_skew_kernel<64, 1>), eg, dim3(4 * PGM_ROWS), 0, s, b->d_jobs);
    if ((e = hipGetLastError()) != hipSuccess) return e;
    if (timed && (e = hipEventRecord(b->ev[2], s)) != hipSuccess) return e;
    const uint32_t spin_limit = b->test_spin_limit ? b->test_spin_limit : PGM_SPIN_LIMIT, stall_job = b->test_stall_job, stall_band = b->test_stall_band;
    const bool fork = S.nlean != 0;
    const bool bandk = S.nbands != 0;
    const bool tbk = (S.nitems != 0 || bandk) && (S.ntb + S.ntb_c + S.ntb_b) != 0;
    const bool critk = S.ncrit != 0;
    if ((fork || bandk || critk) && (e = hipEventRecord(b->ev_fork, s)) != hipSuccess) return e;
    if (critk && (e = hipStreamWaitEvent(ctx->stream4, b->ev_fork, 0)) != hipSuccess) return e;
    if (fork && (e = hipStreamWaitEvent(ctx->stream2, b->ev_fork, 0)) != hipSuccess) return e;
    if (bandk && (e = hipStreamWaitEvent(ctx->stream3, b->ev_fork, 0)) != hipSuccess) return e;
    const uint32_t nrest = S.nitems - S.ncrit;
    hipStream_t sc = critk ? s : ctx->stream4, sr = critk ? ctx->stream4 : s;
    auto sweep = [&](hipStream_t st, uint32_t workers, const PgmItem *list, uint32_t n, bool c3, uint32_t ticket_off) {
        if (c3) hipLaunchKernelGGL(pgm_crit_kernel, dim3(workers), dim3(64 * PGM_C3_WAVES), 0, st, b->d_jobs, list, n, b->d_sync, spin_limit, stall_job, stall_band, ticket_off);
        else hipLaunchKernelGGL(pgm_fill_kernel, dim3(workers), dim3(64 * PGM_WAVES), 0, st, b->d_jobs, list, n, b->d_sync, spin_limit, stall_job, stall_band, ticket_off);
    };
    auto tracebacks = [&](hipStream_t st, uint32_t workers, uint32_t first, uint32_t n, uint32_t lq_off, uint32_t sybase) {
        hipLaunchKernelGGL(pgm_tb_kernel, dim3(workers), dim3(64 * PGM_WAVES), 0, st, b->d_jobs, b->d_tblist + first, n, b->d_sync, b->test_spin_limit, lq_off, sybase, 1u);
    };
    if (critk) sweep(sc, S.ncrit_workers, b->d_items, S.ncrit, S.crit_c3, (uint32_t)PGM_SY_CRIT_TICKET);
    if (nrest != 0) sweep(sr, S.nworkers, b->d_items + S.ncrit, nrest, S.rest_c3, 1u);
    if ((e = hipGetLastError()) != hipSuccess) return e;
    if (fork) {
        hipLaunchKernelGGL((pgm_lean_kernel<2>), dim3(S.nlean_workers), dim3(64 * PGM_WAVES), 0, ctx->stream2, b->d_jobs, b->d_lean, S.nlean, b->d_sync, spin_limit);
        if ((e = hipGetLastError()) != hipSuccess) return e;
    }
    const uint32_t njp = (b->njobs + 3u) / 4u * 4u;
    if (bandk) {
        hipLaunchKernelGGL(pgm_band_kernel, dim3(S.nband_workers), dim3(64 * PGM_WAVES), 0, ctx->stream3, b->d_jobs, b->d_bands, S.nbands_narrow, S.nbands, S.nband_workers - S.nwide_workers, b->d_sync, spin_limit, stall_job, stall_band);
        if ((e = hipGetLastError()) != hipSuccess) return e;
        if (tbk && S.ntb_b) tracebacks(ctx->stream3, S.ntb_b_workers, S.ntb + S.ntb_c, S.ntb_b, b->lq_off + njp, 8u);
        if ((e = hipGetLastError()) != hipSuccess) return e;
        if ((e = hipEventRecord(b->ev_join_b, ctx->stream3)) != hipSuccess) return e;
    }
    if (critk) {
        if (tbk && S.ntb_c) tracebacks(sc, S.ncrit_workers, S.ntb, S.ntb_c, b->lq_off + 2 * njp, 16u);
        if ((e = hipGetLastError()) != hipSuccess) return e;
    }
    if (tbk && S.ntb) {
        tracebacks(sr, S.ntb_workers, 0u, S.ntb, b->lq_off, 0u);
        if ((e = hipGetLastError()) != hipSuccess) return e;
    }
    if (critk && (e = hipEventRecord(b->ev_join_c, ctx->stream4)) != hipSuccess) return e;
    if (bandk && (e = hipStreamWaitEvent(s, b->ev_join_b, 0)) != hipSuccess) return e;
    if (critk && (e = hipStreamWaitEvent(s, b->ev_join_c, 0)) != hipSuccess) return e;
    if (fork && ((e = hipEventRecord(b->ev_join, ctx->stream2)) != hipSuccess || (e = hipStreamWaitEvent(s, b->ev_join, 0)) != hipSuccess)) return e;
    if (timed && (e = hipEventRecord(b->ev[3], s)) != hipSuccess) return e;
    if (timed && (e = hipEventRecord(b->ev[4], s)) != hipSuccess) return e;
    return hipSuccess;
}
struct SmallLayout { size_t sync, jobs, order, items, lean, tblist, bands, times, tabhdr, total_bands; bool any_lean; };
static SmallLayout layout_small(pgm_align_batch *b) {
    SmallLayout s;
    const uint32_t njobs = b->njobs;
    s.total_bands = 0; s.any_lean = false;
    for (const PgmJob &J : b->jobs) { s.total_bands += J.nb; s.any_lean = s.any_lean || (J.lean && !J.keep_cells); }
    DevLayout SM;
    s.sync = SM.take(b->sync_ints * sizeof(int)); s.jobs = SM.take(sizeof(PgmJob) * std::max(1u, njobs));
    s.order = SM.take(4 * (size_t)std::max(1u, njobs)); s.items = SM.take(sizeof(PgmItem) * std::max<size_t>(1, s.total_bands));
    s.lean = SM.take(4 * (size_t)std::max(1u, njobs)); s.tblist = SM.take(8 * (size_t)std::max(1u, njobs));
    s.bands = SM.take(sizeof(PgmItem) * std::max<size_t>(1, s.total_bands)); s.times = SM.take(16 * (size_t)std::max(1u, njobs) + 16);
    s.tabhdr = SM.take(s.any_lean ? 4 * (size_t)PGM_TAB_HDR * njobs : 16);
    b->small_bytes = SM.bytes;
    return s;
}

static double now_ms() { return std::chrono::duration<double, std::milli>(std::chrono::steady_clock::now().time_since_epoch()).count(); }

struct BatchAlloc {
    std::atomic<int> state{0};
    hipError_t err = hipSuccess, host_err = hipSuccess;
    uint8_t *h_out_dev = nullptr;
    double ms_dev = 0, ms_host = 0, ms_slot[6] = {0, 0, 0, 0, 0, 0};
};
static void take_batch_buffers(pgm_ctx *ctx, pgm_align_batch *b, SmallLayout sm, BatchAlloc *A) {
    const double ta0 = now_ms();
    hipError_t e2 = hipSetDevice(ctx->device);
    double tprev = ta0;
    for (int k = 0; k < 6 && e2 == hipSuccess; ++k) {
        const BatchBuffer &s = kBatchBuffers[k];
        e2 = cache_take(ctx, s.slot, b->*s.bytes, (void **)&(b->*s.ptr), &b->cap[s.slot]);
        const double t = now_ms(); A->ms_slot[k] = t - tprev; tprev = t;
    }
    if (e2 == hipSuccess) {
        b->d_sync = (int *)(b->d_small + sm.sync);
        b->d_jobs = (PgmJob *)(b->d_small + sm.jobs);
        b->d_order = (uint32_t *)(b->d_small + sm.order);
        b->d_items = (PgmItem *)(b->d_small + sm.items);
        b->d_lean = (uint32_t *)(b->d_small + sm.lean);
        b->d_tblist = (int2 *)(b->d_small + sm.tblist);
        b->d_bands = (PgmItem *)(b->d_small + sm.bands);
        b->d_times = (unsigned long long *)(b->d_small + sm.times);
        b->d_tabhdr = sm.any_lean ? (int *)(b->d_small + sm.tabhdr) : nullptr;
    }
    A->err = e2;
    A->state.store(e2 == hipSuccess ? 1 : -1, std::memory_order_release);
    A->ms_dev = now_ms() - ta0;
    if (e2 == hipSuccess) {
        hipError_t e3 = cache_take(ctx, pgm_ctx::C_HOST, b->out_bytes + 64, (void **)&b->h_out, &b->cap[pgm_ctx::C_HOST]);
        if (e3 == hipSuccess) b->h_flag = (int *)(b->h_out + (b->out_bytes + 15) / 16 * 16);
        if (e3 == hipSuccess) e3 = hipHostGetDevicePointer((void **)&A->h_out_dev, b->h_out, 0);
        A->host_err = e3;
    }
    A->ms_host = now_ms() - ta0 - A->ms_dev;
}

struct CreateGuard {
    pgm_ctx *ctx;
    pgm_align_batch *b;
    std::thread alloc;
    ~CreateGuard() { if (alloc.joinable()) alloc.join(); if (b) pgm_align_batch_destroy(ctx, b); }
    pgm_align_batch *release() { pgm_align_batch *r = b; b = nullptr; return r; }
};

static void bind_job_pointers(pgm_align_batch *b, const std::vector<JobOff> &off, const pgm_site_ref *res1, const pgm_site_ref *res2, uint8_t *h_out_dev) {
    for (uint32_t i = 0; i < b->njobs; ++i) {
        PgmJob &J = b->jobs[i];
        const JobOff &o = off[i];
        uint8_t *in = b->d_in, *w = b->d_work, *ob = b->d_out;
        J.sites1 = site_ref_of(res1, i) ? res1[i].dev_sites : (const double *)(in + o.s1.sites);
        J.sites2 = site_ref_of(res2, i) ? res2[i].dev_sites : (const double *)(in + o.s2.sites);
        J.smap1 = o.s1.has_smap ? (const uint32_t *)(in + o.s1.smap) : nullptr;
        J.smap2 = o.s2.has_smap ? (const uint32_t *)(in + o.s2.smap) : nullptr;
        J.M = (const double *)(in + o.M); J.pi = (const double *)(in + o.pi);
        J.ni1 = (const PgmNode2 *)(in + o.s1.ni); J.ni2 = (const PgmNode2 *)(in + o.s2.ni);
        J.xp1 = (const int32_t *)(in + o.s1.xp); J.xp2 = (const int32_t *)(in + o.s2.xp);
        J.xc1 = (const uint32_t *)(in + o.s1.xc); J.xc2 = (const uint32_t *)(in + o.s2.xc);
        J.xv1 = (const float *)(in + o.s1.xv); J.xv2 = (const float *)(in + o.s2.xv);
        J.fp1 = (const int32_t *)(in + o.s1.fp); J.fe1 = (const uint2 *)(in + o.s1.fe);
        J.ov2 = (const uint2 *)(in + o.s2.ov);
        J.pp1 = (const int32_t *)(in + o.s1.pp); J.pp2 = (const int32_t *)(in + o.s2.pp);
        J.pc1 = (const uint32_t *)(in + o.s1.pc); J.pc2 = (const uint32_t *)(in + o.s2.pc);
        J.pv1 = (const float *)(in + o.s1.pv); J.pv2 = (const float *)(in + o.s2.pv);
        J.pu1 = (const uint32_t *)(in + o.s1.pu); J.pu2 = (const uint32_t *)(in + o.s2.pu);
        J.g1f = (float *)(w + o.g1f); J.a1 = (float *)(w + o.a1);
        J.t2 = (float *)(w + o.t2); J.b2 = (float *)(w + o.aux2);
        J.map1 = (uint32_t *)(ob + o.map1); J.map2 = (uint32_t *)(ob + o.map2);
        J.mark_score = (float *)(w + o.ms); J.mark_prev = (uint32_t *)(w + o.mp);
        J.tb1 = (PgmTbNode *)(w + o.tb1); J.tb2 = (PgmTbNode *)(w + o.tb2);
        J.result = (PgmJob::Result *)(ob + o.res);
        J.hmap1 = (uint32_t *)(h_out_dev + o.map1); J.hmap2 = (uint32_t *)(h_out_dev + o.map2);
        J.hresult = (PgmJob::Result *)(h_out_dev + o.res);
        J.cells = (float4 *)(b->d_cells + o.cells);
        J.codes = (uint32_t *)(w + o.codes);
        J.endcell = (float4 *)(w + o.endcell);
        if (J.lean && !J.keep_cells && b->d_tabhdr) { J.cls1 = w + o.cls; J.cls2 = w + o.cls + J.n1; J.tabhdr = b->d_tabhdr + (size_t)PGM_TAB_HDR * i; }
        else { J.cls1 = nullptr; J.cls2 = nullptr; J.tabhdr = nullptr; }
        J.S = (float *)(b->d_S + o.S);
        J.prog = b->d_sync + o.prog;
        J.ltab = (uint16_t *)(w + o.ltab); J.lready = b->d_sync + o.lready; J.lrows = o.lrows; J.lcols = o.lcols;
        J.times = b->d_times + 2 * (size_t)i;
    }
}

static std::vector<uint32_t> size_order(const std::vector<PgmJob> &jobs) {
    std::vector<uint32_t> order(jobs.size());
    std::iota(order.begin(), order.end(), 0u);
    std::stable_sort(order.begin(), order.end(), [&](uint32_t x, uint32_t y) { return (uint64_t)jobs[x].n1 * jobs[x].n2 > (uint64_t)jobs[y].n1 * jobs[y].n2; });
    return order;
}
}

extern "C" {

int pgm_test_cu_shares(uint32_t cus, double lean_cost, uint32_t nlean, double band_cost, uint32_t nbands, double rest_cost, uint32_t nrest,
                       uint32_t ncrit, double longest_chain, uint32_t *out4) {
    if (!out4) return fail(PGM_ERR_INVALID, "null argument");
    const CuShares r = cu_shares(cus, lean_cost, nlean, band_cost, nbands, rest_cost, nrest, ncrit, longest_chain);
    out4[0] = r.lean; out4[1] = r.band; out4[2] = r.crit; out4[3] = r.rest;
    return PGM_OK;
}

int pgm_test_batch_plan(uint32_t njobs, const pgm_graph *const *g1, const pgm_graph *const *g2, const pgm_model *const *model,
                        const pgm_scores *scores, uint32_t flags, const pgm_site_ref *res1, const pgm_site_ref *res2, uint32_t cus,
                        uint32_t *head, double *dhead, uint32_t *job_fields, uint32_t *items, uint32_t *bands, uint32_t *lean_list, int32_t *tblist) {
    if (!head || !dhead || !items || !bands || (njobs && (!g1 || !g2 || !model || !scores || !job_fields || !lean_list || !tblist))) return fail(PGM_ERR_INVALID, "null argument");
    std::vector<char> two_chains(njobs, 0);
    for (uint32_t i = 0; i < njobs; ++i) two_chains[i] = job_is_two_chains(g1[i], g2[i]) ? 1 : 0;
    std::vector<PgmJob> jobs;
    BatchSizes Z;
    const int invalid = plan_sizes(njobs, g1, g2, model, scores, flags, res1, res2, two_chains, cus, jobs, Z);
    if (invalid >= 0) return fail(PGM_ERR_INVALID, "invalid job " + std::to_string(invalid));
    std::vector<uint8_t> image(std::max<size_t>(Z.in_base[njobs], 16));
    for (uint32_t i = 0; i < njobs; ++i)
        if (!plan_flatten_job(image.data(), Z.in_base[i], Z.in_base[i + 1], g1[i], g2[i], model[i], site_ref_of(res1, i), site_ref_of(res2, i), Z.pro, jobs[i], Z.off[i]))
            return fail(PGM_ERR_INVALID, "invalid graph in job " + std::to_string(i));
    const BatchSchedule S = plan_schedule(jobs, size_order(jobs), cus);
    const uint32_t h[PGM_PLAN_HEAD] = {njobs ? Z.pro.batch_dp : 0u, Z.pro.promote_bands, S.nitems, S.ncrit, S.nbands, S.nbands_narrow, S.nlean, S.ntb, S.ntb_c, S.ntb_b,
                                       S.nworkers, S.nlean_workers, S.nband_workers, S.nwide_workers, S.ncrit_workers, S.ntb_workers, S.ntb_b_workers,
                                       S.crit_c3, S.rest_c3, S.capacity, (uint32_t)S.total_b, (uint32_t)S.total, (uint32_t)S.total_c};
    const double d[PGM_PLAN_DHEAD] = {S.rsweep, S.t_goal, S.lean_cost, S.band_cost, S.band_end, S.other_cost, S.fill_end, S.crit_end, Z.pro.longest_crit_chain};
    memcpy(head, h, sizeof h);
    memcpy(dhead, d, sizeof d);
    for (uint32_t i = 0; i < njobs; ++i) {
        const PgmJob &J = jobs[i];
        const uint32_t f[PGM_PLAN_JOB] = {J.lean, J.has_extras, J.mode2, J.hD, J.hDX, J.slot_bytes, J.aux_off, J.ov_off, J.rh_off, J.c3_off, J.nov2, J.has_far, J.long1, J.long2,
                                          J.crit3, J.far_slack, J.nslots, Z.off[i].s1.ngeneric + Z.off[i].s2.ngeneric, Z.off[i].s1.nkill + Z.off[i].s2.nkill};
        memcpy(job_fields + (size_t)PGM_PLAN_JOB * i, f, sizeof f);
    }
    if (S.nitems) memcpy(items, S.items.data(), sizeof(PgmItem) * S.nitems);
    if (S.nbands) memcpy(bands, S.bands.data(), sizeof(PgmItem) * S.nbands);
    if (S.nlean) memcpy(lean_list, S.lean_list.data(), 4 * (size_t)S.nlean);
    if (S.ntb + S.ntb_c + S.ntb_b) memcpy(tblist, S.tblist.data(), 8 * (size_t)(S.ntb + S.ntb_c + S.ntb_b));
    return PGM_OK;
}

int pgm_align_batch_create(pgm_ctx *ctx, uint32_t njobs, const pgm_graph *const *g1, const pgm_graph *const *g2,
                           const pgm_model *const *model, const pgm_scores *scores, pgm_align_batch **out) {
    return pgm_align_batch_create_ex(ctx, njobs, g1, g2, model, scores, 0u, out);
}

int pgm_align_batch_create_ex(pgm_ctx *ctx, uint32_t njobs, const pgm_graph *const *g1, const pgm_graph *const *g2,
                              const pgm_model *const *model, const pgm_scores *scores, uint32_t flags, pgm_align_batch **out) {
    return pgm_align_batch_create_res(ctx, njobs, g1, g2, model, scores, flags, nullptr, nullptr, out);
}

int pgm_align_batch_create_res(pgm_ctx *ctx, uint32_t njobs, const pgm_graph *const *g1, const pgm_graph *const *g2,
                               const pgm_model *const *model, const pgm_scores *scores, uint32_t flags,
                               const pgm_site_ref *res1, const pgm_site_ref *res2, pgm_align_batch **out) {
    if (!ctx || !out || (njobs && (!g1 || !g2 || !model || !scores))) return fail(PGM_ERR_INVALID, "null argument");
    *out = nullptr;
    HIPCHK(hipSetDevice(ctx->device));
    const double tcs = now_ms();
    const bool cprof = getenv("PGM_HOST_PROFILE") != nullptr;
    const uint32_t cus = (uint32_t)ctx->prop.multiProcessorCount;
    BatchAlloc A;
    CreateGuard G{ctx, new pgm_align_batch, {}};
    pgm_align_batch *b = G.b;
    b->njobs = njobs;
    std::vector<char> two_chains(njobs, 0);
    (void)lib_pool().run(njobs, njobs >= 16 ? 16u : 1u, [&](size_t i) { two_chains[i] = job_is_two_chains(g1[i], g2[i]) ? 1 : 0; });
    BatchSizes Z;
    const int invalid = plan_sizes(njobs, g1, g2, model, scores, flags, res1, res2, two_chains, cus, b->jobs, Z);
    if (invalid >= 0) return fail(PGM_ERR_INVALID, "invalid job " + std::to_string(invalid));
    const std::vector<size_t> &in_base = Z.in_base;
    b->maxdim = Z.maxdim; b->maxnb = Z.maxnb; b->maxn = Z.maxn; b->maxnblk = Z.maxnblk; b->cells = Z.cells;
    b->res_off.resize(njobs); b->map1_off.resize(njobs); b->map2_off.resize(njobs);
    for (uint32_t i = 0; i < njobs; ++i) { b->res_off[i] = Z.off[i].res; b->map1_off[i] = Z.off[i].map1; b->map2_off[i] = Z.off[i].map2; }
    b->in_bytes = std::max<size_t>(in_base[njobs], 16);
    b->work_bytes = std::max<size_t>(Z.L.W.bytes, 16);
    b->cell_bytes = std::max<size_t>(Z.L.C.bytes, 16);
    b->out_bytes = std::max<size_t>(Z.L.O.bytes, 16);
    b->s_bytes = std::max<size_t>(Z.L.SL.bytes, 16);
    b->lq_off = (uint32_t)Z.L.sync_ints;
    b->sync_ints = Z.L.sync_ints + 3 * (((size_t)njobs + 3) / 4 * 4);
    const double tc0 = now_ms();
    const SmallLayout sm = layout_small(b);
    G.alloc = std::thread(take_batch_buffers, ctx, b, sm, &A);
    hipError_t e;
    if ((e = cache_take(ctx, pgm_ctx::C_HIN, b->in_bytes, (void **)&b->h_in, &b->cap[pgm_ctx::C_HIN])) != hipSuccess)
        return fail(PGM_ERR_DEVICE, std::string("hipHostMalloc: ") + hipGetErrorString(e));
    const double tc1 = now_ms();
    std::atomic<int> bad(-1), upload_err((int)hipSuccess);
    const uint32_t chunk_jobs = (uint32_t)std::max<size_t>(1, ((size_t)8 << 20) / std::max<size_t>(1, in_base[njobs] / std::max(1u, njobs)));
    std::vector<std::atomic<uint32_t>> chunk_done((njobs + chunk_jobs - 1) / chunk_jobs + 1);
    for (auto &cd : chunk_done) cd.store(0);
    (void)lib_pool().run(njobs, 16, [&](size_t job_index) {
        const uint32_t i = (uint32_t)job_index;
        if (!plan_flatten_job(b->h_in, in_base[i], in_base[i + 1], g1[i], g2[i], model[i], site_ref_of(res1, i), site_ref_of(res2, i), Z.pro, b->jobs[i], Z.off[i])) { bad.store((int)i); return; }
        const uint32_t c = i / chunk_jobs, c0 = c * chunk_jobs, c1 = std::min(njobs, c0 + chunk_jobs);
        if (chunk_done[c].fetch_add(1, std::memory_order_acq_rel) + 1 == c1 - c0) {
            int st;
            while ((st = A.state.load(std::memory_order_acquire)) == 0) std::this_thread::yield();
            if (st == 1) {
                (void)hipSetDevice(ctx->device);
                const hipError_t eu = hipMemcpyAsync(b->d_in + in_base[c0], b->h_in + in_base[c0], in_base[c1] - in_base[c0], hipMemcpyHostToDevice, ctx->stream);
                if (eu != hipSuccess) upload_err.store((int)eu);
            }
        }
    });
    if (bad.load() >= 0) return fail(PGM_ERR_INVALID, "invalid graph in job " + std::to_string(bad.load()));
    const double tc2 = now_ms();
    G.alloc.join();
    const double tc3 = now_ms();
    if (A.err != hipSuccess) return fail(A.err == hipErrorOutOfMemory ? PGM_ERR_NOMEM : PGM_ERR_DEVICE, std::string("hipMalloc: ") + hipGetErrorString(A.err));
    if (A.host_err != hipSuccess) return fail(PGM_ERR_DEVICE, std::string("hipHostMalloc: ") + hipGetErrorString(A.host_err));
    bind_job_pointers(b, Z.off, res1, res2, A.h_out_dev);
    b->order = size_order(b->jobs);
    b->sched = plan_schedule(b->jobs, b->order, cus);
    const BatchSchedule &S = b->sched;
    if (cprof && njobs)
        fprintf(stderr, "    work lists: longest chain of sweeps %.0f us, goal %.0f us; lean %zu jobs %.0f us-worker on %u CUs; bands %zu, %.0f us-worker on %u CUs (simulated end %.0f us); items %zu, %.0f us-worker on %u CUs (simulated end %.0f us), of the longest chains %zu on %u CUs (%.0f us)\n",
                S.rsweep, S.t_goal, (size_t)S.nlean, S.lean_cost, S.nlean_workers, S.total_b, S.band_cost, S.nband_workers, S.band_end, S.total, S.other_cost, S.capacity, S.fill_end, S.total_c, S.ncrit_workers, S.crit_end);
    const double tc4 = now_ms();
    if (S.nitems > std::max<size_t>(1, sm.total_bands)) return fail(PGM_ERR_DEVICE, "work list longer than the number of bands");
    if ((e = (hipError_t)upload_err.load()) != hipSuccess ||
        (e = hipMemcpyAsync(b->d_tblist, S.tblist.data(), 8 * S.tblist.size(), hipMemcpyHostToDevice, ctx->stream)) != hipSuccess ||
        (e = hipMemcpyAsync(b->d_jobs, b->jobs.data(), sizeof(PgmJob) * njobs, hipMemcpyHostToDevice, ctx->stream)) != hipSuccess ||
        (e = hipMemcpyAsync(b->d_order, b->order.data(), 4 * (size_t)njobs, hipMemcpyHostToDevice, ctx->stream)) != hipSuccess ||
        (e = hipMemcpyAsync(b->d_items, S.items.data(), sizeof(PgmItem) * S.items.size(), hipMemcpyHostToDevice, ctx->stream)) != hipSuccess ||
        (e = hipMemcpyAsync(b->d_lean, S.lean_list.data(), 4 * S.lean_list.size(), hipMemcpyHostToDevice, ctx->stream)) != hipSuccess ||
        (e = hipMemcpyAsync(b->d_bands, S.bands.data(), sizeof(PgmItem) * S.bands.size(), hipMemcpyHostToDevice, ctx->stream)) != hipSuccess ||
        (e = classify_lean_jobs(ctx, b)) != hipSuccess ||
        (e = hipStreamSynchronize(ctx->stream)) != hipSuccess)
        return fail(PGM_ERR_DEVICE, std::string("upload: ") + hipGetErrorString(e));
    for (int k = 0; k < 5; ++k) (void)hipEventCreate(&b->ev[k]);
    (void)hipEventCreateWithFlags(&b->ev_fork, hipEventDisableTiming);
    (void)hipEventCreateWithFlags(&b->ev_join, hipEventDisableTiming);
    (void)hipEventCreateWithFlags(&b->ev_join_b, hipEventDisableTiming);
    (void)hipEventCreateWithFlags(&b->ev_join_c, hipEventDisableTiming);
    if (cprof)
        fprintf(stderr, "    create: sizes %.2f ms, pinned input block %.2f, flatten %.2f, wait for the allocations %.2f (device %.2f, pinned results %.2f), work list %.2f, upload of %.1f MB %.2f\n",
                tc0 - tcs, tc1 - tc0, tc2 - tc1, tc3 - tc2, A.ms_dev, A.ms_host, tc4 - tc3, b->in_bytes / 1e6, now_ms() - tc4);
    if (cprof)
        fprintf(stderr, "    device buffers: inputs %.1f MB %.2f ms, work %.1f MB %.2f, cells %.1f MB %.2f, results %.1f MB %.2f, S %.1f MB %.2f, small %.2f\n",
                b->in_bytes / 1e6, A.ms_slot[0], b->work_bytes / 1e6, A.ms_slot[1], b->cell_bytes / 1e6, A.ms_slot[2], b->out_bytes / 1e6, A.ms_slot[3], b->s_bytes / 1e6, A.ms_slot[4], A.ms_slot[5]);
    *out = G.release();
    return PGM_OK;
}

int pgm_align_batch_run(pgm_ctx *ctx, pgm_align_batch *b) {
    if (!ctx || !b) return fail(PGM_ERR_INVALID, "null argument");
    if (b->njobs == 0) return PGM_OK;
    HIPCHK(hipSetDevice(ctx->device));
    HIPCHK(launch_all(ctx, b, true));
    b->ev_pending = true;
    return PGM_OK;
}

int pgm_align_batch_time(pgm_ctx *ctx, pgm_align_batch *b, int reps, float *ms_prep, float *ms_emission, float *ms_fill,
                         float *ms_traceback) {
    if (!ctx || !b || reps <= 0) return fail(PGM_ERR_INVALID, "bad argument");
    HIPCHK(hipSetDevice(ctx->device));
    double acc[4] = {0, 0, 0, 0};
    for (int r = 0; r < reps && b->njobs; ++r) {
        HIPCHK(launch_all(ctx, b, true));
        b->ev_pending = false;
        HIPCHK(hipEventSynchronize(b->ev[4]));
        for (int k = 0; k < 4; ++k) {
            float ms = 0;
            HIPCHK(hipEventElapsedTime(&ms, b->ev[k], b->ev[k + 1]));
            acc[k] += ms;
        }
    }
    if (ms_prep) *ms_prep = (float)(acc[0] / reps);
    if (ms_emission) *ms_emission = (float)(acc[1] / reps);
    if (ms_fill) *ms_fill = (float)(acc[2] / reps);
    if (ms_traceback) *ms_traceback = (float)(acc[3] / reps);
    return PGM_OK;
}

int pgm_align_batch_job_times(pgm_ctx *ctx, pgm_align_batch *b, uint64_t *ticks) {
    if (!ctx || !b || !ticks) return fail(PGM_ERR_INVALID, "null argument");
    HIPCHK(hipSetDevice(ctx->device));
    HIPCHK(hipStreamSynchronize(ctx->stream));
    if (b->njobs) HIPCHK(hipMemcpy(ticks, b->d_times, 16 * (size_t)b->njobs, hipMemcpyDeviceToHost));
    return PGM_OK;
}

int pgm_align_batch_fetch(pgm_ctx *ctx, pgm_align_batch *b, pgm_align_out *out) {
    if (!ctx || !b || (b->njobs && !out)) return fail(PGM_ERR_INVALID, "null argument");
    HIPCHK(hipSetDevice(ctx->device));
    if (b->njobs == 0) { HIPCHK(hipStreamSynchronize(ctx->stream)); return PGM_OK; }
    int rc = PGM_OK;
    HIPCHK(hipMemcpyAsync(b->h_flag, b->d_sync, sizeof(int), hipMemcpyDeviceToHost, ctx->stream));
    std::vector<uint8_t> copied(b->njobs, 0);
    auto collect = [&]() -> int {
        uint32_t n = 0;
        for (uint32_t i = 0; i < b->njobs; ++i) {
            if (copied[i]) { ++n; continue; }
            const PgmJob::Result *hr = (const PgmJob::Result *)(b->h_out + b->res_off[i]);
            const int32_t st = __atomic_load_n(&hr->status, __ATOMIC_ACQUIRE);
            if (st == PGM_STATUS_PENDING) continue;
            if (!out[i].map1 || !out[i].map2) return -1;
            const uint32_t len = hr->len;
            if (len > b->jobs[i].n1 + b->jobs[i].n2) return -2;
            out[i].score = hr->score; out[i].n_tr_indels = hr->n_tr_indels; out[i].len = len; out[i].status = st;
            memcpy(out[i].map1, b->h_out + b->map1_off[i], 4 * (size_t)len);
            memcpy(out[i].map2, b->h_out + b->map2_off[i], 4 * (size_t)len);
            copied[i] = 1; ++n;
        }
        return (int)n;
    };
    for (;;) {
        const int n = collect();
        if (n < 0) { (void)hipStreamSynchronize(ctx->stream); return fail(n == -1 ? PGM_ERR_INVALID : PGM_ERR_DEVICE, n == -1 ? "null mapping buffer" : "corrupt result length"); }
        if ((uint32_t)n == b->njobs) break;
        const hipError_t q = hipStreamQuery(ctx->stream);
        if (q == hipSuccess) break;
        if (q != hipErrorNotReady) return fail(PGM_ERR_DEVICE, std::string("fill kernel: ") + hipGetErrorString(q));
    }
    HIPCHK(hipStreamSynchronize(ctx->stream));
    if (b->ev_pending) {
        b->ev_pending = false;
        float ms[3] = {0, 0, 0};
        bool ok = true;
        for (int k = 0; k < 3; ++k) ok = ok && hipEventElapsedTime(&ms[k], b->ev[k], b->ev[k + 1]) == hipSuccess;
        if (ok) { for (int k = 0; k < 3; ++k) b->acc_ms[k] += ms[k]; ++b->acc_n; }
        else (void)hipGetLastError();
    }
    const int aborted = *b->h_flag;
    if (aborted) return fail(PGM_ERR_DEVICE, "fill kernel: a band hand-off timed out");
    for (uint32_t i = 0; i < b->njobs; ++i) {
        PgmJob::Result res;
        memcpy(&res, b->h_out + b->res_off[i], sizeof res);
        if (res.status == PGM_STATUS_PENDING) return fail(PGM_ERR_DEVICE, "fill kernel: a job's result record was never written");
        if (res.status != PGM_OK) rc = res.status;
        if (copied[i]) continue;
        out[i].score = res.score;
        out[i].n_tr_indels = res.n_tr_indels;
        out[i].len = res.len;
        out[i].status = res.status;
        if (res.status != PGM_OK) rc = res.status;
        if (!out[i].map1 || !out[i].map2) return fail(PGM_ERR_INVALID, "null mapping buffer");
        if (res.len > b->jobs[i].n1 + b->jobs[i].n2) return fail(PGM_ERR_DEVICE, "corrupt result length");
        memcpy(out[i].map1, b->h_out + b->map1_off[i], 4 * (size_t)res.len);
        memcpy(out[i].map2, b->h_out + b->map2_off[i], 4 * (size_t)res.len);
    }
    if (rc != PGM_OK) g_err = "backtracking failed";
    return rc;
}

void pgm_align_batch_destroy(pgm_ctx *ctx, pgm_align_batch *b) {
    if (!b) return;
    if (ctx) { (void)hipSetDevice(ctx->device); (void)hipStreamSynchronize(ctx->stream); }
    if (ctx && ctx->stream2) (void)hipStreamSynchronize(ctx->stream2);
    if (ctx && ctx->stream3) (void)hipStreamSynchronize(ctx->stream3);
    if (ctx && ctx->stream4) (void)hipStreamSynchronize(ctx->stream4);
    for (int k = 0; k < 5; ++k)
        if (b->ev[k]) (void)hipEventDestroy(b->ev[k]);
    if (b->ev_fork) (void)hipEventDestroy(b->ev_fork);
    if (b->ev_join) (void)hipEventDestroy(b->ev_join);
    if (b->ev_join_b) (void)hipEventDestroy(b->ev_join_b);
    if (b->ev_join_c) (void)hipEventDestroy(b->ev_join_c);
    for (const BatchBuffer &e : kBatchBuffers) cache_give(ctx, e.slot, b->*e.ptr, b->cap[e.slot]);
    cache_give(ctx, pgm_ctx::C_HOST, b->h_out, b->cap[pgm_ctx::C_HOST]);
    cache_give(ctx, pgm_ctx::C_HIN, b->h_in, b->cap[pgm_ctx::C_HIN]);
    delete b;
}

uint64_t pgm_align_batch_cells(const pgm_align_batch *b) { return b ? b->cells : 0; }

int pgm_align_batch_stage_times(pgm_align_batch *b, int reset, float *ms_prep, float *ms_emission, float *ms_fill, uint32_t *launches) {
    if (!b) return fail(PGM_ERR_INVALID, "null batch");
    const double n = b->acc_n ? (double)b->acc_n : 1.0;
    if (ms_prep) *ms_prep = (float)(b->acc_ms[0] / n);
    if (ms_emission) *ms_emission = (float)(b->acc_ms[1] / n);
    if (ms_fill) *ms_fill = (float)(b->acc_ms[2] / n);
    if (launches) *launches = b->acc_n;
    if (reset) { b->acc_ms[0] = b->acc_ms[1] = b->acc_ms[2] = 0; b->acc_n = 0; }
    return PGM_OK;
}

int pgm_align_batch_test_stall(pgm_align_batch *b, uint32_t job, uint32_t band, uint32_t spin_limit) {
    if (!b) return fail(PGM_ERR_INVALID, "null batch");
    b->test_stall_job = job; b->test_stall_band = band; b->test_spin_limit = spin_limit;
    return PGM_OK;
}

int pgm_align_graphs_batch(pgm_ctx *ctx, uint32_t njobs, const pgm_graph *const *g1, const pgm_graph *const *g2,
                           const pgm_model *const *model, const pgm_scores *scores, pgm_align_out *out) {
    return pgm_align_graphs_batch_res(ctx, njobs, g1, g2, model, scores, nullptr, nullptr, out);
}

int pgm_align_graphs_batch_res(pgm_ctx *ctx, uint32_t njobs, const pgm_graph *const *g1, const pgm_graph *const *g2,
                               const pgm_model *const *model, const pgm_scores *scores, const pgm_site_ref *res1, const pgm_site_ref *res2,
                               pgm_align_out *out) {
    pgm_align_batch *b = nullptr;
    const bool prof = getenv("PGM_HOST_PROFILE") != nullptr;
    const auto t0 = std::chrono::steady_clock::now();
    int rc = pgm_align_batch_create_res(ctx, njobs, g1, g2, model, scores, 0u, res1, res2, &b);
    if (rc != PGM_OK) return rc;
    const auto t1 = std::chrono::steady_clock::now();
    {
        static std::mutex device_turn[64];
        std::lock_guard<std::mutex> turn(device_turn[(unsigned)ctx->device % 64u]);
        rc = pgm_align_batch_run(ctx, b);
        if (rc == PGM_OK) rc = pgm_align_batch_fetch(ctx, b, out);
    }
    const auto t2 = std::chrono::steady_clock::now();
    pgm_align_batch_destroy(ctx, b);
    if (prof)
        fprintf(stderr, "  pgm_align_graphs_batch: %u jobs, create (flatten, allocate, upload, work list) %.2f ms, run + fetch %.2f ms, destroy %.2f ms\n", njobs,
                std::chrono::duration<double, std::milli>(t1 - t0).count(), std::chrono::duration<double, std::milli>(t2 - t1).count(),
                std::chrono::duration<double, std::milli>(std::chrono::steady_clock::now() - t2).count());
    return rc;
}

int pgm_align_batch_read_matrices(pgm_ctx *ctx, pgm_align_batch *b, uint32_t job, float *M, float *X, float *Y, float *W, float *S) {
    if (!ctx || !b || job >= b->njobs) return fail(PGM_ERR_INVALID, "bad argument");
    HIPCHK(hipSetDevice(ctx->device));
    HIPCHK(hipStreamSynchronize(ctx->stream));
    const PgmJob &J = b->jobs[job];
    const size_t N = (size_t)J.n1 * J.n2;
    if ((M || X || Y || W) && !J.keep_cells)
        return fail(PGM_ERR_INVALID, "the DP matrices of a chain-only job are only kept for a batch created with PGM_BATCH_KEEP_MATRICES");
    if (S && J.tabhdr) {
        int bad = 1;
        HIPCHK(hipMemcpy(&bad, J.tabhdr, sizeof(int), hipMemcpyDeviceToHost));
        if (bad == 0) return fail(PGM_ERR_INVALID, "the score matrix of a job of two sequence graphs is only stored for a batch created with PGM_BATCH_KEEP_MATRICES");
    }
    if (M || X || Y || W) {
        const uint32_t sh = J.rshift, R = 1u << sh;
        const size_t ncell = (size_t)J.nb * J.tsteps * 64u * R;
        std::vector<float4> cells(ncell);
        HIPCHK(hipMemcpy(cells.data(), J.cells, ncell * sizeof(float4), hipMemcpyDeviceToHost));
        float *dst[4] = {M, X, Y, W};
        for (int k = 0; k < 4; ++k)
            if (dst[k]) std::fill(dst[k], dst[k] + N, -INFINITY);
        for (uint32_t y = 0; y + 1 < J.n1; ++y)
            for (uint32_t x = 0; x < J.ncol; ++x) {
                const uint32_t bb = y >> (6u + sh), w = y & ((64u << sh) - 1u), l = w >> sh, r = w & (R - 1u);
                const float4 c = cells[((((size_t)bb * J.tsteps + (x + l)) << sh) | r) * 64u + l];
                const size_t i = (size_t)y + (size_t)J.n1 * x;
                if (M) M[i] = c.x;
                if (X) X[i] = c.y;
                if (Y) Y[i] = c.w;
                if (W) W[i] = c.z;
            }
    }
    if (S) {
        const uint32_t sh = J.rshift, R = 1u << sh;
        const size_t ns = (size_t)J.nb * J.nblk * 64u * PGM_BLOCK * R;
        std::vector<float> sk(ns);
        HIPCHK(hipMemcpy(sk.data(), J.S, ns * sizeof(float), hipMemcpyDeviceToHost));
        std::fill(S, S + N, 0.0f);
        for (uint32_t y = 0; y + 1 < J.n1; ++y)
            for (uint32_t x = 0; x < J.ncol; ++x) {
                const uint32_t bb = y >> (6u + sh), w = y & ((64u << sh) - 1u), l = w >> sh, r = w & (R - 1u), t = x + l;
                S[(size_t)y + (size_t)J.n1 * x] = sk[(((((size_t)bb * J.nblk + t / PGM_BLOCK) << sh) | r) * 64u + l) * PGM_BLOCK + t % PGM_BLOCK];
            }
    }
    return PGM_OK;
}

}

#include "pgm_nw_capi.inc"
#include "pgm_csprofile_capi.inc"
#include "pgm_dist_capi.inc"
#include "pgm_merge_capi.inc"
#include "pgm_parsimony_capi.inc"
#include "pgm_wls_capi.inc"
#include "pgm_bionj_capi.inc"
#include "pgm_agreement_capi.inc"
#include "pgm_transfer_capi.inc"
#include "pgm_transfer_taxa_capi.inc"
```

prographmsa_amd/csrc/pgm_device.h:

```cpp
#ifndef PGM_DEVICE_H_
#define PGM_DEVICE_H_

#include <stdint.h>
#include "../../include/pgm_hip.h"

#define PGM_MAX_DIM 64
#define PGM_HALO 0
#define PGM_ROWS 64
#define PGM_VL 16
#define PGM_BLOCK 8
#define PGM_NRING 128
#define PGM_KF 4
#define PGM_KF8 8
#define PGM_DCAP 28
#define PGM_PF 4
#define PGM_REMOTE_MAX 128
#define PGM_WAVES 8
#define PGM_WIDE_WAVES 4
#define PGM_POOL 163584
#define PGM_CPARTS 3
#define PGM_AUX_RES 0
#define PGM_AUX_SBLK 3072
#define PGM_AUX_EL 9216
#define PGM_AUX_CNT 13312
#define PGM_AUX_BYTES 13328

#define PGM_NF_COUNT 15u
#define PGM_NF_GENERIC 16u
#define PGM_NF_KILL 32u
#define PGM_NF_NLONG(f) (((f) >> 16) & 3u)
#define PGM_NF_NOV(f) (((f) >> 20) & 31u)
#define PGM_NF_OVI(f) (((f) >> 25) & 127u)
#define PGM_OV_ENT 16
#define PGM_OV_REC 128
#define PGM_NLONG 3
struct PgmNode2 {
    float cc, c2, c3;
    uint32_t flags;
    uint32_t fd[PGM_KF8];
    float fc[PGM_KF8];
};

#define PGM_TB_PK 8
struct PgmTbNode {
    uint32_t cnt;
    uint32_t c[PGM_TB_PK];
    float v[PGM_TB_PK];
    uint32_t u[PGM_TB_PK];
    uint32_t pad[7];
};

struct PgmJob {
    uint32_t n1, n2;
    uint32_t dim, dp;
    uint32_t nb;
    uint32_t ncol;
    uint32_t tsteps;
    uint32_t maxn;
    uint32_t has_extras;
    uint32_t has_far;
    uint32_t mode2;
    uint32_t far_slack;
    uint32_t aux_off;
    uint32_t hD, hDX;
    uint32_t slot_bytes;
    uint32_t nslots;
    uint32_t rshift;
    uint32_t lean;
    uint32_t crit3;
    uint32_t c3_off;
    uint32_t long1, long2;
    pgm_scores sc;

    const double *sites1, *sites2;
    const uint32_t *smap1, *smap2;
    const double *M, *pi;
    const PgmNode2 *ni1, *ni2;
    const int32_t *xp1, *xp2;
    const uint32_t *xc1, *xc2;
    const float *xv1, *xv2;
    const int32_t *fp1;
    const uint2 *fe1;
    const uint2 *ov2;
    uint32_t nov2, ov_off;
    uint32_t rh_off;
    const int32_t *pp1, *pp2;
    const uint32_t *pc1, *pc2;
    const float *pv1, *pv2;
    const uint32_t *pu1, *pu2;

    PgmTbNode *tb1, *tb2;
    float *g1f;
    float *a1;
    float *t2;
    float *b2;

    float *S;
    uint32_t nblk;
    const uint8_t *cls1, *cls2;
    int *tabhdr;

    uint32_t *codes;
    float4 *endcell;
    uint32_t keep_cells;

    uint16_t *ltab;
    int *lready;
    uint32_t lrows, lcols;

    unsigned long long *times;

    float4 *cells;
    int *prog;

    uint32_t *map1, *map2;
    float *mark_score;
    uint32_t *mark_prev;
    struct Result { float score; uint32_t n_tr_indels; uint32_t len; int32_t status; } *result;
    uint32_t *hmap1, *hmap2;
    Result *hresult;
};


#define PGM_SY_BAND_TICKET 3
#define PGM_SY_CRIT_TICKET 4
#define PGM_SY_WIDE_TICKET 5
#define PGM_SY_LQ_N 32
#define PGM_SY_TB_DONE 33
#define PGM_SY_TBQ_N 34
#define PGM_LK_W 4u
#define PGM_LK_T 32u
#define PGM_LK_NR 4u
#define PGM_LK_MIN_ROWS 1216u
#define PGM_LK_H 16u
#define PGM_LK_TAB (3u * PGM_LK_T * PGM_LK_T)
__host__ __device__ inline uint32_t pgm_lk_first(uint32_t n1, uint32_t n2, uint32_t lcols, uint32_t r) {
    const uint32_t w = lcols < PGM_LK_W ? lcols : PGM_LK_W;
    const uint64_t xc = ((uint64_t)(PGM_LK_T * r + PGM_LK_T / 2u) * (n2 - 1u)) / (n1 - 1u);
    const uint32_t g = (uint32_t)(xc / PGM_LK_T);
    const uint32_t lo = g >= w / 2u ? g - w / 2u : 0u;
    return lo + w > lcols ? lcols - w : lo;
}

struct PgmItem {
    uint32_t job, band;
    uint32_t prio, count;
};

#endif
```

prographmsa_amd/csrc/pgm_plan.h:

```cpp
#ifndef PGM_PLAN_H_
#define PGM_PLAN_H_

#include <hip/hip_vector_types.h>

#include <algorithm>
#include <cmath>
#include <cstring>
#include <numeric>
#include <queue>
#include <vector>

#include "pgm_device.h"

namespace {

constexpr double kTauChain = 0.45;
constexpr double kTauExtras = 0.65;
constexpr double kTauMode2 = 0.6;
constexpr double kTauCrit = 0.42;
constexpr double kTauLean = 0.34;
constexpr double kEager = 0.7;
constexpr double kLag = PGM_ROWS + 3.0 * PGM_BLOCK;
constexpr double kLagCritEst = 80.0;
constexpr double kLagWideEst = 78.0;
// ... 27 lines not shown
};

struct SideOff {
    size_t sites, ni, xp, xc, xv, pp, pc, pv, pu, fp, fe, ov;
    size_t smap = 0;
    bool has_smap = false;
    uint32_t nodes_with_extras;
    uint32_t has_long;
    uint32_t maxd_cap;
    uint32_t maxd_kf8;
    uint32_t far_nodes;
    uint32_t maxd;
    uint32_t far_dmin;
    uint32_t remote;
    uint32_t nov;
    uint32_t ngeneric;
    uint32_t nkill;
    std::vector<uint32_t> cp, cd;
    std::vector<float> cv;
};

static int flatten_side(const pgm_graph *g, const pgm_scores &sc, Arena &A, SideOff &o, const pgm_site_ref *res = nullptr) {
    const uint32_t n = g->n;
    const bool resident = res && res->dev_sites;
    if (n < 2 || (!g->sites && !resident) || !g->e_rowptr) return PGM_ERR_INVALID;
    static thread_local std::vector<float> xv, pv;
    static thread_local std::vector<int32_t> xp, pp;
    static thread_local std::vector<uint32_t> xc, pc, pu;
    static thread_local std::vector<PgmNode2> ni;
    xv.clear(); pv.clear(); xc.clear(); pc.clear(); pu.clear();
    xp.assign(n + 1, 0); pp.assign(n + 1, 0);
    ni.resize(n);
    o.nodes_with_extras = 0; o.has_long = 0; o.maxd_cap = 1; o.maxd_kf8 = 1; o.nkill = 0;
    o.cp.assign(n + 1, 0); o.cd.clear(); o.cv.clear();
    for (uint32_t v = 0; v < n; ++v) {
        PgmNode2 &I = ni[v];
        memset(&I, 0, sizeof I);
        I.cc = I.c2 = I.c3 = INFINITY;
        for (int k = 0; k < PGM_KF8; ++k) I.fc[k] = INFINITY;
        auto place = [&](uint32_t from, float val) {
            const uint32_t d = v - from;
            if (d == 1 && I.cc == INFINITY && val != INFINITY) { I.cc = val; return; }
            xc.push_back(from); xv.push_back(val);
            if (val == INFINITY) return;
            if (d <= (uint32_t)PGM_DCAP) o.maxd_cap = std::max(o.maxd_cap, d); else o.has_long = 1;
            if (d == 2 && I.c2 == INFINITY) { I.c2 = val; return; }
            if (d == 3 && I.c3 == INFINITY) { I.c3 = val; return; }
            o.cd.push_back(d); o.cv.push_back(val);
        };
        const int32_t eb = g->e_rowptr[v], ee = g->e_rowptr[v + 1];
        if (eb > ee || eb < 0) return PGM_ERR_INVALID;
        for (int32_t e = eb; e < ee; ++e) {
            const uint32_t from = g->e_col[e];
            if (from >= v) return PGM_ERR_INVALID;
            const float c = g->e_val[e];
            const float val = (c == 0) ? INFINITY : c + 10000.0f;
            pc.push_back(from); pv.push_back(val); pu.push_back(0u);
            place(from, val);
        }
        if (g->r_rowptr) {
            if (g->r_rowptr[v] > g->r_rowptr[v + 1] || g->r_rowptr[v] < 0) return PGM_ERR_INVALID;
            for (int32_t e = g->r_rowptr[v]; e < g->r_rowptr[v + 1]; ++e) {
                const uint32_t from = g->r_col[e];
                if (from >= v) return PGM_ERR_INVALID;
                const uint32_t units = g->r_units[e];
                const float val = (units == 0) ? INFINITY : sc.repeat_init + sc.repeat_ext * (float)(units - 1);
                pc.push_back(from); pv.push_back(val); pu.push_back(0x80000000u | units);
                place(from, val);
            }
        }
        xp[v + 1] = (int32_t)xc.size();
        pp[v + 1] = (int32_t)pc.size();
        o.cp[v + 1] = (uint32_t)o.cd.size();
        {
            uint32_t dm = I.c3 != INFINITY ? 3u : (I.c2 != INFINITY ? 2u : 1u);
            bool small = o.cp[v + 1] - o.cp[v] <= (uint32_t)PGM_KF8;
            for (uint32_t k = o.cp[v]; k < o.cp[v + 1] && small; ++k) { if (o.cd[k] > (uint32_t)PGM_DCAP) small = false; else dm = std::max(dm, o.cd[k]); }
            if (small) o.maxd_kf8 = std::max(o.maxd_kf8, dm);
        }
        if (v > 0 && v + 1 < n && pp[v + 1] == pp[v]) { I.flags |= PGM_NF_KILL; ++o.nkill; }
        o.nodes_with_extras += (xp[v + 1] > xp[v]);
    }
    if (xc.empty()) { xc.push_back(0); xv.push_back(0); }
    if (pc.empty()) { pc.push_back(0); pv.push_back(0); pu.push_back(0); }
    o.smap = 0; o.has_smap = false;
    if (resident) {
        if (res->ncols == 0 || (!res->node_map && n > res->ncols)) return PGM_ERR_INVALID;
        if (res->node_map) for (uint32_t v = 0; v < n; ++v) if (res->node_map[v] >= res->ncols) return PGM_ERR_INVALID;
        o.sites = 0;
        if (res->node_map) { o.smap = A.put(res->node_map, 4 * (size_t)n); o.has_smap = true; }
    } else o.sites = A.put(g->sites, sizeof(double) * (size_t)g->dim * n);
    o.ni = A.put(ni.data(), sizeof(PgmNode2) * ni.size());
    o.xp = A.put(xp.data(), 4 * xp.size());
    o.xc = A.put(xc.data(), 4 * xc.size());
    o.xv = A.put(xv.data(), 4 * xv.size());
    o.pp = A.put(pp.data(), 4 * pp.size());
    o.pc = A.put(pc.data(), 4 * pc.size());
    o.pv = A.put(pv.data(), 4 * pv.size());
    o.pu = A.put(pu.data(), 4 * pu.size());
    o.fp = A.put(nullptr, 4 * ((size_t)n + 1));
    o.fe = A.put(nullptr, 8 * std::max<size_t>(1, o.cd.size()));
    o.ov = A.put(nullptr, 8 * (size_t)PGM_OV_REC * PGM_OV_ENT);
    return PGM_OK;
}

static void finalize_side(uint8_t *base, uint32_t n, SideOff &o, int side, bool mode2, bool allow_long, bool allow_ov) {
    PgmNode2 *ni = (PgmNode2 *)(base + o.ni);
    int32_t *fp = (int32_t *)(base + o.fp);
    uint2 *fe = (uint2 *)(base + o.fe), *ov = (uint2 *)(base + o.ov);
    o.nov = 0;
    o.far_nodes = 0; o.maxd = 1; o.far_dmin = PGM_DCAP + 1; o.remote = 0; o.ngeneric = 0;
    uint32_t band_entries = 0, band_remote = 0, nfe = 0;
    fp[0] = 0;
    for (uint32_t v = 0; v < n; ++v) {
        PgmNode2 &I = ni[v];
        const uint32_t kill = I.flags & PGM_NF_KILL;
        const uint32_t c0 = o.cp[v], c1 = o.cp[v + 1], nc = c1 - c0;
        if (side == 0 && (v & 63u) == 0) { band_entries = 0; band_remote = 0; }
        uint32_t dmax = 1, nloc = 0, nrem = 0, novf = 0, ovi = 0;
        if (I.c2 != INFINITY) dmax = 2;
        if (I.c3 != INFINITY) dmax = 3;
        bool generic = false;
        if (!mode2) {
            if (nc > (uint32_t)PGM_KF) generic = true;
            for (uint32_t k = c0; k < c1 && !generic; ++k) {
                if (o.cd[k] > (uint32_t)PGM_DCAP) { generic = true; break; }
                I.fd[nloc] = o.cd[k]; I.fc[nloc] = o.cv[k]; ++nloc;
                dmax = std::max(dmax, o.cd[k]);
                o.far_dmin = std::min(o.far_dmin, o.cd[k]);
            }
        } else if (side == 0) {
            const uint32_t lane = v & 63u;
            for (uint32_t k = c0; k < c1; ++k) nrem += (o.cd[k] > (uint32_t)PGM_DCAP || o.cd[k] > lane + (uint32_t)PGM_VL);
            if (band_entries + nc > 512u || band_remote + nrem > (uint32_t)PGM_REMOTE_MAX || nc > 255u || (nrem && !allow_long)) generic = true;
            else {
                for (uint32_t k = c0; k < c1; ++k) {
                    const uint32_t d = o.cd[k];
                    const bool rem = d > (uint32_t)PGM_DCAP || d > lane + (uint32_t)PGM_VL;
                    fe[nfe++] = make_uint2(d | (rem ? 0x80000000u : 0u), __builtin_bit_cast(uint32_t, o.cv[k]));
                    if (!rem) { dmax = std::max(dmax, d); o.far_dmin = std::min(o.far_dmin, d); ++nloc; }
                }
                band_entries += nc; band_remote += nrem;
            }
        } else {
            for (uint32_t k = c0; k < c1; ++k) nrem += o.cd[k] > (uint32_t)PGM_DCAP;
            const uint32_t nl_all = nc - nrem, ring_cap = (uint32_t)PGM_KF8 - std::min(nrem, (uint32_t)PGM_KF8);
            novf = nl_all > ring_cap ? nl_all - ring_cap : 0u;
            if (nrem > (uint32_t)PGM_NLONG || (nrem && !allow_long) || novf > (uint32_t)PGM_OV_ENT || (novf && (o.nov >= (uint32_t)PGM_OV_REC || !allow_ov))) generic = true;
            else {
                uint2 *rec = ov + (size_t)o.nov * PGM_OV_ENT;
                uint32_t nl = 0, no = 0;
                for (uint32_t k = c0; k < c1; ++k) {
                    const uint32_t d = o.cd[k];
                    if (d > (uint32_t)PGM_DCAP) { I.fd[PGM_KF8 - 1 - nl] = d; I.fc[PGM_KF8 - 1 - nl] = o.cv[k]; ++nl; continue; }
                    if (nloc < ring_cap) { I.fd[nloc] = d; I.fc[nloc] = o.cv[k]; ++nloc; }
                    else rec[no++] = make_uint2(d, __builtin_bit_cast(uint32_t, o.cv[k]));
                    dmax = std::max(dmax, d); o.far_dmin = std::min(o.far_dmin, d);
                }
                if (novf) { ovi = o.nov++; for (; no < (uint32_t)PGM_OV_ENT; ++no) rec[no] = make_uint2(1u, __builtin_bit_cast(uint32_t, (float)INFINITY)); }
            }
        }
        fp[v + 1] = (int32_t)nfe;
        if (generic) {
            I.c2 = I.c3 = INFINITY;
            for (int k = 0; k < PGM_KF8; ++k) { I.fd[k] = 0; I.fc[k] = INFINITY; }
            I.flags = PGM_NF_GENERIC | (1u << 8) | kill;
            ++o.ngeneric;
        } else {
            const bool rows2 = mode2 && side == 0;
            I.flags = (rows2 ? 0u : nloc) | (dmax << 8) | kill | ((mode2 && side == 1) ? (nrem << 16) | (novf << 20) | (ovi << 25) : 0u);
            o.maxd = std::max(o.maxd, dmax);
            o.far_nodes += (nloc + nrem) != 0;
            o.remote += nrem;
        }
    }
}

struct JobOff { SideOff s1, s2; size_t M, pi, g1f, a1, t2, aux2, map1, map2, ms, mp, res, cells, tb1, tb2, S, prog, codes, endcell, ltab, lready, cls; uint32_t lrows, lcols; };
struct BatchLayout { DevLayout W, C, O, SL; size_t sync_ints = 64; };
static void layout_job(BatchLayout &L, uint32_t n1, uint32_t n2, uint32_t dp, uint32_t rshift, bool lean, bool keep, JobOff &o) {
    const uint32_t R = 1u << rshift, rows = PGM_ROWS * R;
    const uint32_t nb = (n1 - 1 + rows - 1) / rows, tsteps = (n2 - 1) + 63;
    const uint32_t nblk = (tsteps + PGM_BLOCK - 1) / PGM_BLOCK, maxn = std::max(n1, n2);
    o.g1f = L.W.take(sizeof(float) * (size_t)dp * n1);
    o.a1 = L.W.take(sizeof(float) * n1);
    o.t2 = L.W.take(sizeof(float) * (size_t)dp * n2);
    o.aux2 = L.W.take(sizeof(float) * (size_t)n2);
    o.map1 = L.O.take(4 * (size_t)(n1 + n2), 16);
    o.map2 = L.O.take(4 * (size_t)(n1 + n2), 16);
    o.tb1 = L.W.take(sizeof(PgmTbNode) * (size_t)n1);
    o.tb2 = L.W.take(sizeof(PgmTbNode) * (size_t)n2);
    o.ms = L.W.take(4 * (size_t)maxn);
    o.mp = L.W.take(4 * (size_t)maxn);
    o.res = L.O.take(sizeof(PgmJob::Result), 16);
    o.cells = L.C.take(keep ? sizeof(float4) * (size_t)nb * tsteps * 64u * R : 16, 1024);
    o.codes = L.W.take(lean ? 4 * (size_t)nb * nblk * 64u * R : 16);
    o.endcell = L.W.take(16, 16);
    o.cls = L.W.take((lean && !keep) ? (size_t)n1 + n2 : 16, 16);
    o.S = L.SL.take(sizeof(float) * (size_t)nb * nblk * 64u * PGM_BLOCK * R, 1024);
    o.prog = L.sync_ints;
    L.sync_ints += (nb + 3) / 4 * 4;
    o.lrows = (!lean && n1 - 1 >= PGM_LK_MIN_ROWS && n2 - 1 >= 4 * PGM_LK_T) ? (n1 - 1 + PGM_LK_T - 1) / PGM_LK_T : 0u;
    o.lcols = (n2 - 1 + PGM_LK_T - 1) / PGM_LK_T;
    o.ltab = L.W.take(std::max<size_t>((size_t)o.lrows * PGM_LK_W * PGM_LK_TAB * 2, 16), 256);
    o.lready = L.sync_ints;
    L.sync_ints += ((size_t)o.lrows + 2 + 3) / 4 * 4;
}
static bool graph_is_chain(const pgm_graph *g) {
    if (g->r_rowptr && g->r_rowptr[g->n] != 0) return false;
    if (g->e_rowptr[0] != 0 || g->e_rowptr[1] != 0) return false;
    for (uint32_t v = 1; v < g->n; ++v) {
        const int32_t eb = g->e_rowptr[v], ee = g->e_rowptr[v + 1];
        if (eb < 0 || ee - eb != 1 || g->e_col[eb] != v - 1 || g->e_val[eb] == 0.0f) return false;
    }
    return true;
}


static size_t side_bound_bytes(size_t n, size_t dim, size_t E) {
    E = std::max<size_t>(E, 1);
    return n * dim * 8 + n * sizeof(PgmNode2) + 3 * (n + 1) * 4 + E * 28 + 8 * (size_t)PGM_OV_REC * PGM_OV_ENT + 16 * 16;
}
static size_t model_bound_bytes(size_t dim) { return (dim * dim + dim) * 8 + 64; }

static const pgm_site_ref *site_ref_of(const pgm_site_ref *r, uint32_t i) { return (r && r[i].dev_sites) ? &r[i] : nullptr; }
static bool job_is_two_chains(const pgm_graph *a, const pgm_graph *c) {
    return a && c && a->n >= 2 && c->n >= 2 && a->e_rowptr && c->e_rowptr && a->e_col && c->e_col && a->e_val && c->e_val && graph_is_chain(a) && graph_is_chain(c);
}

struct BatchPrologue {
    uint32_t batch_dp = 4u;
    double longest_crit_chain = 0.0;
    uint32_t promote_bands = 0xffffffffu;
};
static BatchPrologue plan_batch_prologue(const std::vector<PgmJob> &jobs, uint32_t cus) {
    BatchPrologue P;
    uint32_t batch_dim = 0;
    double crit_load = 0.0;
    for (const PgmJob &J : jobs) {
        batch_dim = std::max(batch_dim, J.dim);
        P.longest_crit_chain = std::max(P.longest_crit_chain, ((double)(row_bands(J.n1) - 1) * kLagCritEst + (double)(J.n2 - 1 + 63)) * kTauCrit);
        if (!J.lean) crit_load += (double)row_bands(J.n1) * (double)(J.n2 - 1 + 63) * kTauCrit;
    }
    P.batch_dp = alphabet_tier(batch_dim);
    if (crit_load <= 1.25 * (double)cus * P.longest_crit_chain) P.promote_bands = 8u;
    return P;
}

struct BatchSizes {
    BatchPrologue pro;
    BatchLayout L;
    std::vector<JobOff> off;
    std::vector<size_t> in_base;
    uint32_t maxdim = 0, maxnb = 0, maxn = 0, maxnblk = 0;
    uint64_t cells = 0;
};
static int plan_sizes(uint32_t njobs, const pgm_graph *const *g1, const pgm_graph *const *g2, const pgm_model *const *model, const pgm_scores *scores,
                      uint32_t flags, const pgm_site_ref *res1, const pgm_site_ref *res2, const std::vector<char> &two_chains, uint32_t cus,
                      std::vector<PgmJob> &jobs, BatchSizes &Z) {
    auto side_bound = [](const pgm_graph *g, const pgm_site_ref *res) -> size_t {
        const size_t n = g->n;
        size_t E = (size_t)std::max(0, g->e_rowptr ? g->e_rowptr[n] : 0);
        if (g->r_rowptr) E += (size_t)std::max(0, g->r_rowptr[n]);
        const size_t full = side_bound_bytes(n, g->dim, E);
        return (res && res->dev_sites) ? full - n * g->dim * 8 + n * 4 + 16 : full;
    };
    jobs.resize(njobs);
    Z.off.resize(njobs);
    Z.in_base.assign(njobs + 1, 0);
    for (uint32_t i = 0; i < njobs; ++i) {
        const pgm_graph *a = g1[i], *c = g2[i];
        if (!a || !c || !model[i] || a->dim != c->dim || a->dim == 0 || a->dim > PGM_MAX_DIM || a->n < 2 || c->n < 2 || !model[i]->M || !model[i]->pi ||
            (!a->sites && !site_ref_of(res1, i)) || !a->e_rowptr || (!c->sites && !site_ref_of(res2, i)) || !c->e_rowptr)
            return (int)i;
        PgmJob &J = jobs[i];
        memset(&J, 0, sizeof J);
        J.n1 = a->n; J.n2 = c->n; J.dim = a->dim;
        J.ncol = c->n - 1;
        J.tsteps = J.ncol + 63;
        constexpr uint32_t lean_rshift = 1u;
        J.lean = (two_chains[i] && ((uint64_t)J.tsteps * 1024u << lean_rshift) < (1ull << 30)) ? 1u : 0u;
        J.rshift = J.lean ? lean_rshift : 0u;
        J.nb = (a->n - 1 + (PGM_ROWS << J.rshift) - 1) / (PGM_ROWS << J.rshift);
        J.nblk = (J.tsteps + PGM_BLOCK - 1) / PGM_BLOCK;
        J.maxn = std::max(a->n, c->n);
        J.sc = scores[i];
        J.keep_cells = (!J.lean || (flags & PGM_BATCH_KEEP_MATRICES)) ? 1u : 0u;
        Z.maxnblk = std::max(Z.maxnblk, J.nblk);
        Z.maxn = std::max(Z.maxn, J.maxn);
        Z.maxdim = std::max(Z.maxdim, a->dim);
        Z.maxnb = std::max(Z.maxnb, J.nb << J.rshift);
        Z.cells += (uint64_t)(a->n - 2) * (c->n - 2);
        Z.in_base[i + 1] = Z.in_base[i] + side_bound(a, site_ref_of(res1, i)) + side_bound(c, site_ref_of(res2, i)) + model_bound_bytes(a->dim);
    }
    Z.pro = plan_batch_prologue(jobs, cus);
    for (uint32_t i = 0; i < njobs; ++i) {
        PgmJob &J = jobs[i];
        J.dp = Z.pro.batch_dp;
        layout_job(Z.L, J.n1, J.n2, J.dp, J.rshift, J.lean != 0, J.keep_cells != 0, Z.off[i]);
    }
    return -1;
}

static bool plan_job_sweep(PgmJob &J, uint8_t *base, SideOff &s1, SideOff &s2, const BatchPrologue &P) {
    J.has_extras = (s1.nodes_with_extras + s2.nodes_with_extras) > 0 ? 1u : 0u;
    if (J.lean && J.has_extras) return false;
    uint32_t hD = 16, hDX = 4;
    while (hD < s1.maxd_kf8 + s2.maxd_kf8 + (uint32_t)PGM_BLOCK) hD *= 2;
    while (hDX < s2.maxd_kf8 + 1) hDX *= 2;
    auto slot_head = [&](bool mode2) { return 2u * hD * (64u + PGM_VL) * 4u + hDX * 64u * 4u + PGM_NRING * (mode2 ? 80u : 48u); };
    const uint32_t nb_job = row_bands(J.n1);
    const bool allow_long = (uint64_t)J.nb * J.tsteps * 1024u < (1ull << 32);
    const bool has_long = (s1.has_long | s2.has_long) != 0 && allow_long;
    const double far_density = 0.5 * ((double)s1.cp[J.n1] / J.n1 + (double)s2.cp[J.n2] / J.n2);
    const double chain_wide = ((double)(nb_job - 1) * kLagWideEst + (double)(J.n2 - 1 + 63)) * (0.7 + 10.0 * far_density);
    const bool fits_wide = slot_head(false) <= kWideSlot && chain_wide <= 0.9 * P.longest_crit_chain;
    J.mode2 = (J.has_extras && ((hD >= kMode2MinHd && !fits_wide) || nb_job >= kMode2MinBands || nb_job >= P.promote_bands || has_long)) ? 1u : 0u;
    const bool mode2 = J.mode2 != 0;
    if (mode2) {
        while (hD < s1.maxd_cap + s2.maxd_cap + (uint32_t)PGM_BLOCK) hD *= 2;
        while (hDX < s2.maxd_cap + 1) hDX *= 2;
    }
    const uint32_t aux_bytes = mode2 ? (uint32_t)PGM_AUX_BYTES : 0u;
    finalize_side(base, J.n1, s1, 0, mode2, allow_long, false);
    finalize_side(base, J.n2, s2, 1, mode2, allow_long, slot_head(mode2) + aux_bytes + kOvBytes <= (uint32_t)PGM_POOL);
    J.nov2 = mode2 ? s2.nov : 0u;
    J.has_far = (s1.far_nodes + s2.far_nodes) > 0 ? 1u : 0u;
    J.long1 = (mode2 && s1.remote) ? 1u : 0u;
    J.long2 = (mode2 && s2.remote) ? 1u : 0u;
    const bool c3 = mode2 && !J.long1 && !J.long2 && J.nov2 == 0 && s1.ngeneric + s2.ngeneric == 0 && s1.nkill + s2.nkill == 0 &&
                    slot_head(true) + aux_bytes + kC3Bytes <= (uint32_t)PGM_POOL;
    if (c3 && hDX < 8u) hDX = 8u;
    J.hD = hD; J.hDX = hDX;
    J.slot_bytes = slot_head(mode2);
    J.aux_off = J.slot_bytes;
    J.slot_bytes += aux_bytes;
    J.ov_off = J.slot_bytes;
    if (J.nov2) J.slot_bytes += kOvBytes;
    J.rh_off = J.slot_bytes;
    if (J.long1 | J.long2) J.slot_bytes += 3u * 32u * 64u * 4u;
    J.c3_off = J.slot_bytes;
    J.crit3 = (c3 && J.slot_bytes + kC3Bytes <= (uint32_t)PGM_POOL) ? 1u : 0u;
    if (J.crit3) J.slot_bytes += kC3Bytes;
    J.far_slack = std::max(1u, std::min(4u, std::min(s1.far_dmin, s2.far_dmin)));
    J.nslots = mode2 ? 1u : std::max(1u, std::min((uint32_t)PGM_WAVES, (uint32_t)PGM_POOL / J.slot_bytes));
    if (J.lean) J.nslots = PGM_WAVES;
    return true;
}

static bool plan_flatten_job(uint8_t *base, size_t lo, size_t hi, const pgm_graph *a, const pgm_graph *c, const pgm_model *m,
                             const pgm_site_ref *r1, const pgm_site_ref *r2, const BatchPrologue &P, PgmJob &J, JobOff &o) {
    Arena A;
    A.base = base; A.off = lo; A.end = hi;
    if (flatten_side(a, J.sc, A, o.s1, r1) != PGM_OK || flatten_side(c, J.sc, A, o.s2, r2) != PGM_OK) return false;
    if (!plan_job_sweep(J, base, o.s1, o.s2, P)) return false;
    o.M = A.put(m->M, sizeof(double) * J.dim * J.dim);
    o.pi = A.put(m->pi, sizeof(double) * J.dim);
    return !A.overflow;
}


struct CuShares { uint32_t lean, band, crit, rest, rest_need; double t_goal, fl, fb; };
static CuShares cu_shares(uint32_t cus, double lean_cost, uint32_t nlean, double band_cost, uint32_t nbands, double rest_cost, uint32_t nrest, uint32_t ncrit, double rsweep) {
    CuShares r = {0u, 0u, 0u, 0u, 0u, 0.0, 1.0, 1.0};
    cus = std::max(1u, cus);
    const uint32_t queues = (nlean != 0) + (nbands != 0) + (nrest != 0);
    if (ncrit != 0 && cus > queues) r.crit = std::min(std::min(ncrit, cus / 2u), cus - queues);
    const uint32_t cap = std::max(1u, cus - r.crit);
    const double sum = (nlean ? lean_cost : 0.0) + (nbands ? band_cost : 0.0) + (nrest ? rest_cost : 0.0);
    const double t_par = std::max(1e-3, sum / cap);
    r.t_goal = std::max(std::max(rsweep, t_par), 1e-3);
    const double w = std::min(1.0, std::max(0.0, (rsweep / t_par - 1.0) / 0.5));
    r.fl = 1.0 - 0.4 * w; r.fb = 1.0 - 0.25 * w;
    auto need = [](double cost, double t, uint32_t most) { return (uint32_t)std::min<double>(most, std::max(1.0, std::ceil(cost / t))); };
    const uint32_t band_most = (nbands + PGM_WAVES - 1) / PGM_WAVES;
    uint32_t lean = nlean ? need(lean_cost, r.fl * r.t_goal, nlean) : 0u, band = nbands ? need(band_cost, r.fb * r.t_goal, band_most) : 0u;
    uint32_t rest = nrest ? need(rest_cost, r.t_goal, nrest) : 0u;
    if (lean + band + rest > cap) {
        const double scale = (double)cap / (double)(lean + band + rest);
        auto cut = [&](uint32_t v) { return v ? std::max(1u, (uint32_t)std::floor(v * scale)) : 0u; };
        lean = cut(lean); band = cut(band); rest = cut(rest);
        while (lean + band + rest > cap) {
            uint32_t *big = &rest; if (band > *big) big = &band; if (lean > *big) big = &lean;
            if (*big <= 1u) break;
            --*big;
        }
    }
    r.rest_need = rest;
    const uint32_t left = cap > lean + band + rest ? cap - lean - band - rest : 0u;
    if (nrest) rest = std::min(nrest, rest + left);
    else if (nbands) band = std::min(band_most, band + left);
    else if (nlean) lean = std::min(nlean, lean + left);
    r.lean = lean; r.band = band; r.rest = rest;
    return r;
}

struct BatchSchedule {
    std::vector<PgmItem> items;
    std::vector<PgmItem> bands;
    std::vector<uint32_t> lean_list;
    std::vector<int2> tblist;
    uint32_t nitems = 0, nbands = 0, nlean = 0;
    uint32_t ncrit = 0, nbands_narrow = 0, ntb = 0, ntb_c = 0, ntb_b = 0;
    uint32_t nworkers = 0, nlean_workers = 0, nband_workers = 0, nwide_workers = 0, ncrit_workers = 0, ntb_workers = 0, ntb_b_workers = 0;
    bool crit_c3 = false, rest_c3 = false;
    double rsweep = 0, t_goal = 0, lean_cost = 0, band_cost = 0, band_end = 0, other_cost = 0, fill_end = 0, crit_end = 0;
    size_t total_b = 0, total = 0, total_c = 0;
    uint32_t capacity = 0;
};

struct SimItem { double rem, dur, gap; uint32_t job, band, count; };
static double simulate_workers(const std::vector<std::vector<SimItem>> &pj, size_t count, uint32_t workers, double rmax, std::vector<PgmItem> &out) {
    out.clear();
    double end = 0.0;
    typedef std::pair<double, uint32_t> TE;
    std::priority_queue<double, std::vector<double>, std::greater<double>> free_at;
    for (uint32_t w = 0; w < std::max(1u, workers); ++w) free_at.push(0.0);
    std::priority_queue<TE> ready;
    std::priority_queue<TE, std::vector<TE>, std::greater<TE>> pending;
    std::vector<uint32_t> next(pj.size(), 0);
    for (uint32_t i = 0; i < pj.size(); ++i) if (!pj[i].empty()) ready.push({pj[i][0].rem, i});
    out.reserve(count);
    double now = 0.0;
    while (out.size() < count) {
        now = std::max(now, free_at.top());
        while (!pending.empty() && pending.top().first <= now) {
            const uint32_t j = pending.top().second; pending.pop();
            ready.push({pj[j][next[j]].rem, j});
        }
        if (ready.empty()) { now = pending.top().first; continue; }
        const uint32_t j = ready.top().second; ready.pop();
        const SimItem &it = pj[j][next[j]];
        out.push_back(PgmItem{it.job, it.band, it.rem > 0.6 * rmax ? 3u : (it.rem > 0.35 * rmax ? 2u : (it.rem > 0.2 * rmax ? 1u : 0u)), it.count});
        free_at.pop();
        free_at.push(now + it.dur);
        end = std::max(end, now + it.dur);
        if (++next[j] < pj[j].size()) pending.push({pj[j][next[j]].rem > kEager * rmax ? now : now + it.gap, j});
    }
    return end;
}

static uint32_t wide_share(uint32_t cus, size_t total_b, size_t total_w, double wide_cost, double band_cost) {
    if (total_w == 0) return 0u;
    if (total_b == 0) return cus;
    const uint32_t w = (uint32_t)std::lround(cus * wide_cost / band_cost);
    return std::max(1u, std::min(cus > 1u ? cus - 1u : 1u, w));
}

static BatchSchedule plan_schedule(const std::vector<PgmJob> &jobs, const std::vector<uint32_t> &order, uint32_t cus) {
    BatchSchedule S;
    const uint32_t njobs = (uint32_t)jobs.size();
    S.capacity = cus;
    if (njobs) {
        std::vector<std::vector<SimItem>> per_job(njobs), per_job_b(njobs), per_job_c(njobs), per_job_w(njobs);
        std::vector<double> chain_of(njobs, 0.0);
        size_t total = 0, total_b = 0, total_w = 0;
        double rmax = 1.0, rsweep = 1.0;
        for (uint32_t q = 0; q < njobs; ++q) {
            const uint32_t i = order[q];
            const PgmJob &J = jobs[i];
            const double tau = J.crit3 ? kTauCrit : (J.mode2 ? kTauMode2 : (J.has_extras ? kTauExtras : kTauChain));
            const double tb = (J.has_extras ? 0.3 : 0.2) * (double)(J.n1 + J.n2);
            if (J.lean) {
                const double rounds = std::ceil((double)J.nb / PGM_WAVES), first = std::min<double>(J.nb, PGM_WAVES);
                S.lean_cost += kTauLean * (rounds * J.tsteps + (first - 1.0) * 72.0) + 0.04 * (double)(J.n1 + J.n2);
                S.lean_list.push_back(i);
                continue;
            }
            const bool narrow = !J.mode2 && J.slot_bytes <= kNarrowSlot;
            const bool wide = !J.mode2 && !narrow && J.slot_bytes <= kWideSlot;
            const bool per_band = narrow || wide;
            if (!per_band) chain_of[i] = tau * ((double)(J.nb - 1) * kLag + J.tsteps);
            const uint32_t group = per_band ? 1u : J.nslots;
            for (uint32_t band = 0; band < J.nb; band += group) {
                const uint32_t cnt = std::min(group, J.nb - band);
                SimItem it;
                it.rem = tau * ((double)(J.nb - 1 - band) * kLag + J.tsteps) + tb;
                it.dur = tau * ((double)(cnt - 1) * kLag + J.tsteps);
                it.gap = tau * (double)cnt * kLag;
                it.job = i; it.band = band; it.count = cnt;
                (wide ? per_job_w : (narrow ? per_job_b : per_job))[i].push_back(it);
                rmax = std::max(rmax, it.rem);
                rsweep = std::max(rsweep, it.rem - tb);
            }
            total += per_job[i].size();
            total_b += per_job_b[i].size();
            total_w += per_job_w[i].size();
        }
        double band_cost = 0.0, crit_cost = 0.0, wide_cost = 0.0, other_cost = 0.0;
        for (uint32_t i = 0; i < njobs; ++i) {
            for (const SimItem &it : per_job[i]) other_cost += it.dur;
            for (const SimItem &it : per_job_b[i]) band_cost += it.dur / PGM_WAVES;
            for (const SimItem &it : per_job_w[i]) wide_cost += it.dur / PGM_WIDE_WAVES;
        }
        band_cost += wide_cost;
        auto in_crit = [&](uint32_t i) { return !per_job[i].empty() && chain_of[i] >= 0.85 * rsweep; };
        size_t total_c = 0;
        if (total != 0) {
            uint32_t ncj = 0, nrestj = 0;
            for (uint32_t i = 0; i < njobs; ++i) if (!per_job[i].empty()) { if (in_crit(i)) ++ncj; else ++nrestj; }
            if (ncj != 0 && nrestj != 0)
                for (uint32_t i = 0; i < njobs; ++i)
                    if (in_crit(i)) { total_c += per_job[i].size(); for (const SimItem &it : per_job[i]) crit_cost += it.dur; }
        }
        const uint32_t nlean = (uint32_t)S.lean_list.size(), band_units = (uint32_t)(total_b + 2 * total_w);
        CuShares sh = cu_shares(cus, S.lean_cost, nlean, band_cost, band_units, other_cost - crit_cost, (uint32_t)(total - total_c), (uint32_t)total_c, rsweep);
        if (total_c != 0 && sh.crit == 0) {
            total_c = 0; crit_cost = 0.0;
            sh = cu_shares(cus, S.lean_cost, nlean, band_cost, band_units, other_cost, (uint32_t)total, 0u, rsweep);
        }
        if (total_c != 0)
            for (uint32_t i = 0; i < njobs; ++i)
                if (in_crit(i)) per_job_c[i].swap(per_job[i]);
        total -= total_c;
        const double t_goal = sh.t_goal;
        uint32_t lean_cus = sh.lean, band_cus = sh.band, crit_cus = sh.crit;
        if (lean_cus) { const uint32_t rounds = (nlean + lean_cus - 1u) / lean_cus; lean_cus = (nlean + rounds - 1u) / rounds; }
        S.nlean_workers = lean_cus;
        double band_end = 0.0;
        uint32_t wide_cus = 0;
        if (total_b + total_w != 0) {
            std::vector<PgmItem> bands_w;
            const uint32_t most = std::max(band_cus, band_cus + (sh.rest > sh.rest_need ? sh.rest - sh.rest_need : 0u));
            auto run = [&](uint32_t n) {
                wide_cus = wide_share(n, total_b, total_w, wide_cost, band_cost);
                const uint32_t ncus = n > wide_cus ? n - wide_cus : (total_b ? 1u : 0u);
                double e = 0.0;
                if (total_b) e = simulate_workers(per_job_b, total_b, ncus * PGM_WAVES, rmax, S.bands);
                if (total_w) e = std::max(e, simulate_workers(per_job_w, total_w, wide_cus * PGM_WIDE_WAVES, rmax, bands_w));
                return e;
            };
            if (total != 0) {
                for (int it = 0; it < 3 && band_cus < most; ++it) {
                    band_end = run(band_cus);
                    if (band_end <= sh.fb * t_goal) break;
                    band_cus = std::min(most, std::max(band_cus + 1u, (uint32_t)std::ceil(band_cus * std::min(2.0, band_end / (sh.fb * t_goal)))));
                }
            }
            band_cus = std::max(1u, std::min<uint32_t>(std::min(band_cus, most), (uint32_t)((total_b + PGM_WAVES - 1) / PGM_WAVES + (total_w + PGM_WIDE_WAVES - 1) / PGM_WIDE_WAVES)));
            if (total_b && total_w) band_cus = std::max(band_cus, 2u);
            band_end = run(band_cus);
            if (total_b == 0) S.bands.clear();
            S.nbands_narrow = (uint32_t)S.bands.size();
            S.bands.insert(S.bands.end(), bands_w.begin(), bands_w.end());
            uint32_t nbj = 0;
            for (uint32_t i = 0; i < njobs; ++i) nbj += (!per_job_b[i].empty() || !per_job_w[i].empty());
            const uint32_t most_tb = std::max(band_cus, band_cus + (sh.rest > sh.rest_need ? sh.rest - sh.rest_need : 0u));
            if (nbj > band_cus) {
                const uint32_t rounds = (nbj + band_cus - 1u) / band_cus, want = rounds > 1u ? (nbj + rounds - 2u) / (rounds - 1u) : band_cus;
                if (want > band_cus && want <= most_tb && want <= band_cus + band_cus / 8u + 1u) {
                    band_cus = want;
                    wide_cus = wide_share(band_cus, total_b, total_w, wide_cost, band_cost);
                }
            }
        }
        S.nwide_workers = wide_cus;
        S.nband_workers = band_cus;
        if (total_c != 0) {
            uint32_t need = 0;
            for (uint32_t i = 0; i < njobs; ++i)
                if (!per_job_c[i].empty()) need += std::min<uint32_t>(jobs[i].nb, jobs[i].tsteps / (uint32_t)std::max(1.0, kLag) + 2u);
            crit_cus = std::max(1u, std::min(crit_cus, need));
        }
        S.capacity = std::max(1u, cus > lean_cus + band_cus + crit_cus ? cus - lean_cus - band_cus - crit_cus : 1u);
        S.ncrit_workers = crit_cus;
        std::vector<PgmItem> items_rest;
        S.crit_end = total_c ? simulate_workers(per_job_c, total_c, crit_cus, rmax, S.items) : 0.0;
        S.ncrit = (uint32_t)S.items.size();
        S.fill_end = simulate_workers(per_job, total, S.capacity, rmax, items_rest);
        S.items.insert(S.items.end(), items_rest.begin(), items_rest.end());
        S.rsweep = rsweep; S.t_goal = t_goal; S.band_cost = band_cost; S.band_end = band_end; S.other_cost = other_cost;
        S.total_b = total_b; S.total = total; S.total_c = total_c;
    }
    S.nitems = (uint32_t)S.items.size(); S.nbands = (uint32_t)S.bands.size(); S.nlean = (uint32_t)S.lean_list.size();
    S.nworkers = std::max(1u, std::min(S.capacity, S.nitems - S.ncrit));
    S.crit_c3 = S.ncrit != 0; S.rest_c3 = S.nitems > S.ncrit;
    std::vector<int> last_item(njobs, 0), group(njobs, 0);
    for (uint32_t k = 0; k < S.nitems; ++k) {
        const PgmItem &it = S.items[k];
        if (!jobs[it.job].crit3) (k < S.ncrit ? S.crit_c3 : S.rest_c3) = false;
        if (it.band + it.count == jobs[it.job].nb) last_item[it.job] = (int)k;
        if (k < S.ncrit) group[it.job] = 1;
    }
    for (const PgmItem &it : S.bands) group[it.job] = 2;
    uint32_t cnt[3] = {0, 0, 0};
    for (int pass = 0; pass < 3; ++pass)
        for (uint32_t q = 0; q < njobs; ++q) { const uint32_t i = order[q]; if (!jobs[i].lean && group[i] == pass) { S.tblist.push_back(make_int2((int)i, last_item[i])); ++cnt[pass]; } }
    S.ntb = cnt[0]; S.ntb_c = cnt[1]; S.ntb_b = cnt[2];
    const uint32_t all_cus = std::max(1u, cus) - S.nlean_workers;
    S.ntb_workers = std::max(1u, (S.ntb_b || S.ntb_c) ? S.nworkers : all_cus);
    S.ntb_b_workers = std::max(1u, (S.ntb || S.ntb_c) ? S.nband_workers : all_cus);
    if (S.bands.empty()) S.bands.push_back(PgmItem{0u, 0u, 0u, 0u});
    if (S.lean_list.empty()) S.lean_list.push_back(0u);
    if (S.tblist.empty()) S.tblist.push_back(make_int2(0, 0));
    return S;
}

}

#endif
```

Before: 81.15.

## Fuse prep and emission into one persistent ticketed precompute kernel

Replaces the separate prep and emission-skew launches with a single persistent kernel. Blocks pull tiles from an atomic ticket queue, and emission tiles spin-wait on a per-job counter until that job's prep tiles are done. This lets emission for early jobs overlap prep for later jobs and removes a launch boundary. For table-scored lean jobs it also skips prep slices the class table does not need. The cost is spin-wait synchronisation, a timeout/abort path, an extra host round-trip to read class headers at batch creation, and a changed way of splitting the prep/emission timing.

```diff
diff --git a/include/pgm_hip.h b/include/pgm_hip.h
--- a/include/pgm_hip.h
+++ b/include/pgm_hip.h
@@ -99,6 +99,11 @@
 int pgm_test_batch_plan(uint32_t njobs, const pgm_graph *const *g1, const pgm_graph *const *g2, const pgm_model *const *model,
                         const pgm_scores *scores, uint32_t flags, const pgm_site_ref *res1, const pgm_site_ref *res2, uint32_t cus,
                         uint32_t *head, double *dhead, uint32_t *job_fields, uint32_t *items, uint32_t *bands, uint32_t *lean_list, int32_t *tblist);
+#define PGM_TILE_EMISSION 0x80000000u
+#define PGM_TILE_SIDE2 0x40000000u
+int pgm_test_precompute_tiles(uint32_t njobs, const pgm_graph *const *g1, const pgm_graph *const *g2, const pgm_model *const *model,
+                              const pgm_scores *scores, uint32_t flags, const pgm_site_ref *res1, const pgm_site_ref *res2, uint32_t cus,
+                              uint32_t *head, uint32_t *tiles, uint32_t cap);
 int pgm_align_batch_read_matrices(pgm_ctx *ctx, pgm_align_batch *b, uint32_t job, float *M,
                                   float *X, float *Y, float *W, float *S);
 
diff --git a/prographmsa_amd/__init__.py b/prographmsa_amd/__init__.py
--- a/prographmsa_amd/__init__.py
+++ b/prographmsa_amd/__init__.py
@@ -72,7 +72,7 @@
 EXPORTS = [
     "pgm_device_count", "pgm_ctx_create", "pgm_ctx_destroy", "pgm_last_error", "pgm_ctx_device_info",
     "pgm_align_graphs_batch", "pgm_align_batch_create", "pgm_align_batch_create_ex", "pgm_align_batch_create_res", "pgm_align_graphs_batch_res", "pgm_align_batch_run", "pgm_align_batch_fetch",
-    "pgm_align_batch_destroy", "pgm_align_batch_cells", "pgm_align_batch_test_stall", "pgm_test_cu_shares", "pgm_test_batch_plan", "pgm_align_batch_stage_times", "pgm_align_batch_job_times", "pgm_align_batch_time", "pgm_align_batch_read_matrices",
+    "pgm_align_batch_destroy", "pgm_align_batch_cells", "pgm_align_batch_test_stall", "pgm_test_cu_shares", "pgm_test_batch_plan", "pgm_test_precompute_tiles", "pgm_align_batch_stage_times", "pgm_align_batch_job_times", "pgm_align_batch_time", "pgm_align_batch_read_matrices",
     "pgm_nw_pairs_batch", "pgm_nw_pairs_submit", "pgm_nw_pairs_wait", "pgm_nw_last_kernel_ms", "pgm_host_alloc", "pgm_host_free", "pgm_csprofile_load", "pgm_csprofile_create_batch", "pgm_csprofile_create_batch_res",
     "pgm_csprofile_last_kernel_ms", "pgm_mldist_batch", "pgm_prealigned_counts_batch", "pgm_kmer_cosine", "pgm_dist_last_kernel_ms",
     "pgm_kmer_cosine_multi", "pgm_prealigned_counts_multi", "pgm_prealigned_counts_resampled",
@@ -112,6 +112,8 @@
         "pgm_test_cu_shares": (C.c_int, [u32, C.c_double, u32, C.c_double, u32, C.c_double, u32, u32, C.c_double, C.POINTER(C.c_uint32)]),
         "pgm_test_batch_plan": (C.c_int, [u32, PG, PG, PM, C.POINTER(pgm_scores), u32, C.POINTER(pgm_site_ref), C.POINTER(pgm_site_ref), u32,
                                           C.POINTER(u32), C.POINTER(C.c_double)] + [C.POINTER(u32)] * 4 + [C.POINTER(i32)]),
+        "pgm_test_precompute_tiles": (C.c_int, [u32, PG, PG, PM, C.POINTER(pgm_scores), u32, C.POINTER(pgm_site_ref), C.POINTER(pgm_site_ref), u32,
+                                                C.POINTER(u32), C.POINTER(u32), u32]),
         "pgm_align_batch_stage_times": (C.c_int, [vp, C.c_int] + [C.POINTER(C.c_float)] * 3 + [C.POINTER(u32)]),
         "pgm_align_batch_job_times": (C.c_int, [vp, vp, C.POINTER(C.c_uint64)]),
         "pgm_align_batch_time": (C.c_int, [vp, vp, C.c_int] + [C.POINTER(C.c_float)] * 4),
diff --git a/prographmsa_amd/csrc/pgm_align_kernels.h b/prographmsa_amd/csrc/pgm_align_kernels.h
--- a/prographmsa_amd/csrc/pgm_align_kernels.h
+++ b/prographmsa_amd/csrc/pgm_align_kernels.h
@@ -28,18 +28,13 @@
     return pgm_ls_log_add(q, match_init);
 }
 
+template <class T> __device__ __forceinline__ void pgm_st_dev(T *p, T v) {
+    __hip_atomic_store((__attribute__((address_space(1))) T *)(uintptr_t)p, v, __ATOMIC_RELAXED, __HIP_MEMORY_SCOPE_AGENT);
+}
+#define PGM_PC_THREADS 256
 template <int DMAX, int NODES>
-__global__ void __launch_bounds__(NODES) pgm_prep_kernel(const PgmJob *__restrict__ jobs, int *__restrict__ sync, uint32_t sync_ints) {
-    extern __shared__ float prep_lds[];
-    {
-        const uint32_t nthreads = gridDim.x * gridDim.y * gridDim.z * NODES;
-        const uint32_t gid = ((blockIdx.z * gridDim.y + blockIdx.y) * gridDim.x + blockIdx.x) * NODES + threadIdx.x;
-        for (uint32_t i = gid; i < sync_ints; i += nthreads) sync[i] = 0;
-    }
-    const PgmJob &J = jobs[blockIdx.x];
-    const bool first = blockIdx.y == 0;
+__device__ __forceinline__ void pgm_prep_tile(const PgmJob &J, const bool first, const uint32_t v0, float *prep_lds, const uint32_t tid) {
     const uint32_t n = first ? J.n1 : J.n2;
-    const uint32_t v0 = blockIdx.z * NODES;
     if (v0 >= n) return;
     if (J.tabhdr && J.tabhdr[0] == 0) {
         const uint32_t nc = J.dim + 2u;
@@ -60,7 +55,7 @@
         const uint32_t *pc = first ? J.pc1 : J.pc2, *pu = first ? J.pu1 : J.pu2;
         const float *pv = first ? J.pv1 : J.pv2;
         PgmTbNode *rec = (first ? J.tb1 : J.tb2) + v0;
-        for (uint32_t i = threadIdx.x; i < nn * PGM_TB_PK; i += NODES) {
+        for (uint32_t i = tid; i < nn * PGM_TB_PK; i += PGM_PC_THREADS) {
             const uint32_t node = i / PGM_TB_PK, k = i % PGM_TB_PK;
             const int32_t eb = pp[v0 + node];
             const uint32_t cnt = (uint32_t)(pp[v0 + node + 1] - eb);
@@ -69,19 +64,19 @@
             rec[node].c[k] = pc[e]; rec[node].v[k] = pv[e]; rec[node].u[k] = pu[e];
         }
     }
-    if (!first) for (uint32_t i = threadIdx.x; i < D * D; i += NODES) Mf[i] = (float)J.M[i];
-    for (uint32_t i = threadIdx.x; i < D; i += NODES) pif[i] = (float)J.pi[i];
+    if (!first) for (uint32_t i = tid; i < D * D; i += PGM_PC_THREADS) Mf[i] = (float)J.M[i];
+    for (uint32_t i = tid; i < D; i += PGM_PC_THREADS) pif[i] = (float)J.pi[i];
     const double *sites = first ? J.sites1 : J.sites2;
     const uint32_t *smap = first ? J.smap1 : J.smap2;
     float *dst = (first ? J.g1f : J.t2) + (size_t)DP * v0;
-    for (uint32_t i = threadIdx.x; i < nn * D; i += NODES) {
+    for (uint32_t i = tid; i < nn * D; i += PGM_PC_THREADS) {
         const uint32_t node = v0 + i / D;
         const float g = (float)sites[(size_t)D * (smap ? smap[node] : node) + i % D];
         nl[(i / D) * ST + (i % D)] = g;
-        if (first && DP == D) dst[i] = g;
+        if (first && DP == D) pgm_st_dev(dst + i, g);
     }
     __syncthreads();
-    const uint32_t v = threadIdx.x;
+    const uint32_t v = tid;
     float g[DMAX];
     float acc = 0.0f;
     if (v < nn) {
@@ -102,12 +97,12 @@
 #pragma unroll
         for (int k = 0; k < DMAX; ++k)
             if ((uint32_t)k >= aligned && (uint32_t)k < D) acc = __fadd_rn(acc, __fmul_rn(g[k], pif[k]));
-        (first ? J.a1 : J.b2)[v0 + v] = acc;
+        pgm_st_dev((first ? J.a1 : J.b2) + v0 + v, acc);
     }
     if (first) {
         if (DP != D && v < nn) {
 #pragma unroll
-            for (int k = 0; k < DMAX; ++k) if ((uint32_t)k < DP) dst[(size_t)DP * v + k] = g[k];
+            for (int k = 0; k < DMAX; ++k) if ((uint32_t)k < DP) pgm_st_dev(dst + (size_t)DP * v + k, g[k]);
         }
         return;
     }
@@ -122,9 +117,9 @@
         }
     }
     __syncthreads();
-    for (uint32_t i = threadIdx.x; i < nn * DP; i += NODES) {
+    for (uint32_t i = tid; i < nn * DP; i += PGM_PC_THREADS) {
         const uint32_t node = i / DP, k = i % DP;
-        dst[i] = k < D ? nl[node * ST + k] : 0.0f;
+        pgm_st_dev(dst + i, k < D ? nl[node * ST + k] : 0.0f);
     }
 }
 
@@ -174,19 +169,23 @@
 #define PGM_GLOBAL __attribute__((address_space(1)))
 typedef float pgm_v4f __attribute__((ext_vector_type(4)));
 template <class T> __device__ __forceinline__ T pgm_gld(const T *p) { return *(const PGM_GLOBAL T *)(uintptr_t)p; }
-#define PGM_EM_TB 4
+typedef float pgm_v2f __attribute__((ext_vector_type(2)));
+template <int DP> struct PgmEmLds {
+    static constexpr int COLS = 64 + PGM_EM_TB * PGM_BLOCK - PGM_HALO - 1;
+    static constexpr int STR = DP + 1;
+    pgm_v2f tp[(COLS + 1) * STR];
+    float bq[COLS];
+    float As[32];
+};
 template <int DP, int RB>
-__global__ void __launch_bounds__(4 * PGM_ROWS) pgm_emission_skew_kernel(const PgmJob *__restrict__ jobs) {
-    typedef float pgm_v2f __attribute__((ext_vector_type(2)));
+__device__ __forceinline__ void pgm_emission_tile(const PgmJob &J, const uint32_t bx, const uint32_t by, PgmEmLds<DP> &L, const uint32_t tid) {
     constexpr int NT = DP / 4;
-    constexpr int COLS = 64 + PGM_EM_TB * PGM_BLOCK - PGM_HALO - 1;
-    constexpr int STR = DP + 1;
-    __shared__ pgm_v2f tp[(COLS + 1) * STR];
-    __shared__ float bq[COLS];
-    const PgmJob &J = jobs[blockIdx.z];
-    const uint32_t tb0 = blockIdx.x * PGM_EM_TB;
+    constexpr int COLS = PgmEmLds<DP>::COLS, STR = PgmEmLds<DP>::STR;
+    pgm_v2f *const tp = L.tp;
+    float *const bq = L.bq;
+    const uint32_t tb0 = bx * PGM_EM_TB;
     const uint32_t rsh = J.rshift, nvb = J.nb << rsh;
-    if (tb0 >= J.nblk || 4u * RB * blockIdx.y >= nvb) return;
+    if (tb0 >= J.nblk || 4u * RB * by >= nvb) return;
     if (J.tabhdr && pgm_gld(J.tabhdr) == 0) return;
     auto row_of = [&](uint32_t v, uint32_t lane_) { return ((((v >> rsh) << 6) + lane_) << rsh) | (v & ((1u << rsh) - 1u)); };
     auto sblock_of = [&](uint32_t v, uint32_t tb_) { return ((((size_t)(v >> rsh) * J.nblk + tb_) << rsh) | (v & ((1u << rsh) - 1u))); };
@@ -197,9 +196,9 @@
         float *const tab = (float *)tp;
         static_assert(COLS * TE <= (COLS + 1) * STR * 2, "score table must fit the column staging area");
         static_assert(DP > 20 || TE <= 32, "row classes must fit As");
-        __shared__ float As[32];
-        const uint32_t fb0 = 4u * blockIdx.y + threadIdx.x / PGM_ROWS;
-        const uint32_t fl = threadIdx.x % PGM_ROWS;
+        float *const As = L.As;
+        const uint32_t fb0 = 4u * by + tid / PGM_ROWS;
+        const uint32_t fl = tid % PGM_ROWS;
         const bool active = fb0 < nvb;
         int sym = DP;
         bool plain = true;
@@ -220,7 +219,7 @@
             plain = plain && nz <= 1;
             a_row = J.a1[yc];
         }
-        if (threadIdx.x < 32) As[threadIdx.x] = 0.f;
+        if (tid < 32) As[tid] = 0.f;
         if (__syncthreads_and(plain ? 1 : 0)) {
             if (active) As[sym] = a_row;
             __syncthreads();
@@ -229,7 +228,7 @@
             float tt[NE], tb2[NE];
 #pragma unroll
             for (int e = 0; e < NE; ++e) {
-                const int i = (int)threadIdx.x + e * 4 * PGM_ROWS;
+                const int i = (int)tid + e * 4 * PGM_ROWS;
                 const int ci = i / TE, k = i % TE, c = cbase + ci;
                 const bool in = i < COLS * TE && c >= 0 && c <= (int)J.ncol;
                 tb2[e] = in ? J.b2[c] : 0.f;
@@ -237,7 +236,7 @@
             }
 #pragma unroll
             for (int e = 0; e < NE; ++e) {
-                const int i = (int)threadIdx.x + e * 4 * PGM_ROWS;
+                const int i = (int)tid + e * 4 * PGM_ROWS;
                 if (i < COLS * TE) tab[i] = pgm_emission_finish(0.0f + tt[e], As[i % TE], tb2[e], mi);
             }
             __syncthreads();
@@ -260,7 +259,7 @@
     }
     const float4 *t2q = (const float4 *)J.t2;
     float *tpf = (float *)tp;
-    for (int i = threadIdx.x; i < (COLS + 1) * NT; i += 4 * PGM_ROWS) {
+    for (int i = tid; i < (COLS + 1) * NT; i += 4 * PGM_ROWS) {
         const int ci = i / NT, q = i % NT, c = cbase + ci;
         float4 v = make_float4(0.f, 0.f, 0.f, 0.f);
         if (c >= 0 && c <= (int)J.ncol) v = t2q[(size_t)NT * c + q];
@@ -272,13 +271,13 @@
             if (ci > 0) tpf[2 * ((ci - 1) * STR + k) + 1] = vv[u];
         }
     }
-    for (int i = threadIdx.x; i < COLS; i += 4 * PGM_ROWS) {
+    for (int i = tid; i < COLS; i += 4 * PGM_ROWS) {
         const int col = cbase + i;
         bq[i] = (col >= 0 && col <= (int)J.ncol) ? J.b2[col] : 0.f;
     }
     __syncthreads();
-    const uint32_t b0 = (4u * blockIdx.y + threadIdx.x / PGM_ROWS) * RB;
-    const int l = PGM_HALO + (int)(threadIdx.x % PGM_ROWS);
+    const uint32_t b0 = (4u * by + tid / PGM_ROWS) * RB;
+    const int l = PGM_HALO + (int)(tid % PGM_ROWS);
     if (b0 >= nvb) return;
     float gy[RB][DP], ay[RB];
 #pragma unroll
@@ -331,6 +330,80 @@
                 for (int q = 0; q < PGM_BLOCK / 4; ++q) dst[q] = pgm_v4f{out[r][4 * q], out[r][4 * q + 1], out[r][4 * q + 2], out[r][4 * q + 3]};
             }
         }
+    }
+}
+
+#define PGM_PC_TICKET 0
+#define PGM_PC_PREP_DONE 1
+#define PGM_PC_JOBS 4
+#define PGM_PC_SPIN_LIMIT (1u << 24)
+template <int DMAX, int NODES, int ROWS, int WAVES>
+__global__ void __launch_bounds__(PGM_PC_THREADS) __attribute__((amdgpu_waves_per_eu(WAVES, WAVES))) pgm_precompute_kernel(const PgmJob *__restrict__ jobs, const PgmTile *__restrict__ tiles, const uint32_t ntiles,
+                                                                        const uint32_t nprep, uint32_t *__restrict__ pc, const uint32_t *__restrict__ need,
+                                                                        const uint32_t epoch, int *__restrict__ sync, const uint32_t sync_ints,
+                                                                        unsigned long long *__restrict__ hclk, int *__restrict__ habort) {
+    static_assert(NODES % ROWS == 0 && ROWS <= PGM_PC_THREADS, "a prep tile is a whole number of passes of one node per thread");
+    constexpr size_t kPrepBytes = ((size_t)DMAX * DMAX + DMAX + (size_t)ROWS * (DMAX + 1)) * sizeof(float);
+    constexpr size_t kLdsBytes = kPrepBytes > sizeof(PgmEmLds<DMAX>) ? kPrepBytes : sizeof(PgmEmLds<DMAX>);
+    __shared__ __attribute__((aligned(16))) unsigned char lds[kLdsBytes];
+    __shared__ uint32_t s_ticket;
+    __shared__ int s_go;
+    for (uint32_t i = blockIdx.x * PGM_PC_THREADS + threadIdx.x; i < sync_ints; i += gridDim.x * PGM_PC_THREADS) sync[i] = 0;
+    const uint32_t base = epoch * (ntiles + gridDim.x);
+    if (threadIdx.x == 0) {
+        s_ticket = __hip_atomic_fetch_add(pc + PGM_PC_TICKET, 1u, __ATOMIC_RELAXED, __HIP_MEMORY_SCOPE_AGENT) - base;
+        s_go = 1;
+    }
+    __syncthreads();
+    uint32_t t = __builtin_amdgcn_readfirstlane(s_ticket);
+    while (t < ntiles) {
+        uint32_t next = 0;
+        if (threadIdx.x == 0) {
+            next = __hip_atomic_fetch_add(pc + PGM_PC_TICKET, 1u, __ATOMIC_RELAXED, __HIP_MEMORY_SCOPE_AGENT) - base;
+            if (t == 0u) __hip_atomic_store(hclk, (unsigned long long)__builtin_amdgcn_s_memrealtime(), __ATOMIC_RELAXED, __HIP_MEMORY_SCOPE_SYSTEM);
+        }
+        uint32_t tid = threadIdx.x;
+        asm volatile("" : "+v"(tid));
+        const PgmTile T = tiles[t];
+        const uint32_t job = T.job & PGM_TILE_JOB;
+        const PgmJob &J = jobs[job];
+        if (!(T.job & PGM_TILE_EMISSION)) {
+            const bool first = (T.job & PGM_TILE_SIDE2) == 0u;
+#pragma unroll 1
+            for (uint32_t p = 0; p < (uint32_t)(NODES / ROWS); ++p) {
+                if (p) __syncthreads();
+                pgm_prep_tile<DMAX, ROWS>(J, first, T.a * (uint32_t)NODES + p * (uint32_t)ROWS, (float *)lds, tid);
+            }
+            asm volatile("s_waitcnt vmcnt(0)" ::: "memory");
+            __syncthreads();
+            if (threadIdx.x == 0) {
+                __hip_atomic_fetch_add(pc + PGM_PC_JOBS + job, 1u, __ATOMIC_RELAXED, __HIP_MEMORY_SCOPE_AGENT);
+                const uint32_t done = __hip_atomic_fetch_add(pc + PGM_PC_PREP_DONE, 1u, __ATOMIC_RELAXED, __HIP_MEMORY_SCOPE_AGENT) - epoch * nprep;
+                if (done + 1u == nprep) __hip_atomic_store(hclk + 1, (unsigned long long)__builtin_amdgcn_s_memrealtime(), __ATOMIC_RELAXED, __HIP_MEMORY_SCOPE_SYSTEM);
+            }
+        } else {
+            if (threadIdx.x == 0) {
+                const uint32_t want = (epoch + 1u) * need[job];
+                uint32_t spins = 0;
+                while ((int32_t)(__hip_atomic_load(pc + PGM_PC_JOBS + job, __ATOMIC_RELAXED, __HIP_MEMORY_SCOPE_AGENT) - want) < 0) {
+                    if (++spins > PGM_PC_SPIN_LIMIT) {
+                        __hip_atomic_store(sync, 1, __ATOMIC_RELAXED, __HIP_MEMORY_SCOPE_AGENT);
+                        __hip_atomic_store(habort, 1, __ATOMIC_RELAXED, __HIP_MEMORY_SCOPE_SYSTEM);
+                        s_go = 0;
+                        break;
+                    }
+                    __builtin_amdgcn_s_sleep(8);
+                }
+                __builtin_amdgcn_fence(__ATOMIC_ACQUIRE, "agent");
+            }
+            __syncthreads();
+            if (!s_go) return;
+            pgm_emission_tile<DMAX, 1>(J, T.a, T.b, *(PgmEmLds<DMAX> *)lds, tid);
+        }
+        __syncthreads();
+        if (threadIdx.x == 0) s_ticket = next;
+        __syncthreads();
+        t = __builtin_amdgcn_readfirstlane(s_ticket);
     }
 }
 
diff --git a/prographmsa_amd/csrc/pgm_capi.hip b/prographmsa_amd/csrc/pgm_capi.hip
--- a/prographmsa_amd/csrc/pgm_capi.hip
+++ b/prographmsa_amd/csrc/pgm_capi.hip
@@ -56,6 +56,7 @@
     void *cache_ptr[C_SLOTS] = {};
     size_t cache_bytes[C_SLOTS] = {};
     hipDeviceProp_t prop;
+    int pc_blocks[3] = {1, 1, 1};
     float nw_ms = 0, cs_ms = 0, ml_ms = 0, merge_ms = 0, pars_ms = 0, wls_ms = 0;
     uint32_t wls_n = 0, wls_launches = 0;
     float bionj_ms = 0;
@@ -127,6 +128,11 @@
     uint8_t *h_out = nullptr;
     uint8_t *h_in = nullptr;
     int *h_flag = nullptr;
+    unsigned long long *h_clk = nullptr;
+    uint8_t *h_aux_dev = nullptr;
+    PgmTile *d_tiles = nullptr;
+    uint32_t *d_pc = nullptr, *d_need = nullptr;
+    uint32_t ntiles = 0, nprep = 0, pc_epoch = 0, pc_grid = 0;
     int *d_sync = nullptr;
     size_t sync_ints = 0;
     uint32_t lq_off = 0;
@@ -152,6 +158,8 @@
     {pgm_ctx::C_CELLS, 2048, &pgm_align_batch::d_cells, &pgm_align_batch::cell_bytes}, {pgm_ctx::C_OUT, 8, &pgm_align_batch::d_out, &pgm_align_batch::out_bytes},
     {pgm_ctx::C_S, 1024, &pgm_align_batch::d_S, &pgm_align_batch::s_bytes}, {pgm_ctx::C_SMALL, 4, &pgm_align_batch::d_small, &pgm_align_batch::small_bytes}};
 
+namespace { hipError_t precompute_occupancy(pgm_ctx *ctx); }
+
 extern "C" {
 
 const char *pgm_last_error(void) { return g_err.c_str(); }
@@ -188,6 +196,7 @@
     hipLaunchKernelGGL(pgm_warm_kernel, dim3(1), dim3(64), 0, c->stream);
     HIPCHK(hipGetLastError());
     HIPCHK(hipStreamSynchronize(c->stream));
+    HIPCHK(precompute_occupancy(c));
     {
         void *h = nullptr, *d = nullptr;
         const size_t wb = (size_t)1 << 20;
@@ -316,36 +325,44 @@
 }
 
 #define PGM_STATUS_PENDING 0x7ffffff0
-struct PrepTier { uint32_t tier, threads; size_t lds; };
-static PrepTier prep_tier(uint32_t maxdim) {
-    const uint32_t tier = alphabet_tier(maxdim), threads = tier == 64u ? 64u : 256u;
-    return {tier, threads, ((size_t)maxdim * maxdim + maxdim + threads * ((size_t)maxdim + 1)) * sizeof(float)};
+template <class F> static void with_precompute_kernel(uint32_t tier, F &&f) {
+    if (tier == 4) f(pgm_precompute_kernel<4, 256, 256, 8>);
+    else if (tier == 20) f(pgm_precompute_kernel<20, 256, 256, 6>);
+    else f(pgm_precompute_kernel<64, 64, 64, 3>);
+}
+hipError_t precompute_occupancy(pgm_ctx *ctx) {
+    const uint32_t tiers[3] = {4u, 20u, 64u};
+    for (int k = 0; k < 3; ++k) {
+        hipError_t e = hipSuccess;
+        with_precompute_kernel(tiers[k], [&](auto kern) { e = hipOccupancyMaxActiveBlocksPerMultiprocessor(&ctx->pc_blocks[k], kern, PGM_PC_THREADS, 0); });
+        if (e != hipSuccess) return e;
+        if (ctx->pc_blocks[k] < 1) ctx->pc_blocks[k] = 1;
+    }
+    return hipSuccess;
+}
+static uint32_t precompute_grid(const pgm_ctx *ctx, uint32_t tier, uint32_t ntiles) {
+    const uint32_t per_cu = (uint32_t)ctx->pc_blocks[tier == 4 ? 0 : tier == 20 ? 1 : 2];
+    return std::max(1u, std::min(ntiles, per_cu * (uint32_t)ctx->prop.multiProcessorCount));
 }
 static hipError_t launch_all(pgm_ctx *ctx, pgm_align_batch *b, bool timed) {
     hipStream_t s = ctx->stream;
     const BatchSchedule &S = b->sched;
     hipError_t e;
     for (uint32_t i = 0; i < b->njobs; ++i) ((PgmJob::Result *)(b->h_out + b->res_off[i]))->status = PGM_STATUS_PENDING;
+    b->h_flag[1] = 0;
     if (timed && (e = hipEventRecord(b->ev[0], s)) != hipSuccess) return e;
-    const PrepTier T = prep_tier(b->maxdim);
-    const dim3 pg(b->njobs, 2, (b->maxn + T.threads - 1) / T.threads);
-    if (T.tier == 4) hipLaunchKernelGGL((pgm_prep_kernel<4, 256>), pg, dim3(256), T.lds, s, b->d_jobs, b->d_sync, (uint32_t)b->sync_ints);
-    else if (T.tier == 20) hipLaunchKernelGGL((pgm_prep_kernel<20, 256>), pg, dim3(256), T.lds, s, b->d_jobs, b->d_sync, (uint32_t)b->sync_ints);
-    else hipLaunchKernelGGL((pgm_prep_kernel<64, 64>), pg, dim3(64), T.lds, s, b->d_jobs, b->d_sync, (uint32_t)b->sync_ints);
+    const uint32_t tier = alphabet_tier(b->maxdim), epoch = b->pc_epoch++;
+    with_precompute_kernel(tier, [&](auto k) {
+        hipLaunchKernelGGL(k, dim3(b->pc_grid), dim3(PGM_PC_THREADS), 0, s, b->d_jobs, b->d_tiles, b->ntiles, b->nprep, b->d_pc, b->d_need, epoch, b->d_sync,
+                           (uint32_t)b->sync_ints, (unsigned long long *)(b->h_aux_dev + 8), (int *)(b->h_aux_dev + 4));
+    });
     if ((e = hipGetLastError()) != hipSuccess) return e;
-    if (timed && (e = hipEventRecord(b->ev[1], s)) != hipSuccess) return e;
-    const dim3 eg((b->maxnblk + PGM_EM_TB - 1) / PGM_EM_TB, (b->maxnb + 3) / 4, b->njobs);
-    if (T.tier == 4) hipLaunchKernelGGL((pgm_emission_skew_kernel<4, 1>), eg, dim3(4 * PGM_ROWS), 0, s, b->d_jobs);
-    else if (T.tier == 20) hipLaunchKernelGGL((pgm_emission_skew_kernel<20, 1>), eg, dim3(4 * PGM_ROWS), 0, s, b->d_jobs);
-    else hipLaunchKernelGGL((pgm_emission_skew_kernel<64, 1>), eg, dim3(4 * PGM_ROWS), 0, s, b->d_jobs);
-    if ((e = hipGetLastError()) != hipSuccess) return e;
-    if (timed && (e = hipEventRecord(b->ev[2], s)) != hipSuccess) return e;
     const uint32_t spin_limit = b->test_spin_limit ? b->test_spin_limit : PGM_SPIN_LIMIT, stall_job = b->test_stall_job, stall_band = b->test_stall_band;
     const bool fork = S.nlean != 0;
     const bool bandk = S.nbands != 0;
     const bool tbk = (S.nitems != 0 || bandk) && (S.ntb + S.ntb_c + S.ntb_b) != 0;
     const bool critk = S.ncrit != 0;
-    if ((fork || bandk || critk) && (e = hipEventRecord(b->ev_fork, s)) != hipSuccess) return e;
+    if ((timed || fork || bandk || critk) && (e = hipEventRecord(b->ev_fork, s)) != hipSuccess) return e;
     if (critk && (e = hipStreamWaitEvent(ctx->stream4, b->ev_fork, 0)) != hipSuccess) return e;
     if (fork && (e = hipStreamWaitEvent(ctx->stream2, b->ev_fork, 0)) != hipSuccess) return e;
     if (bandk && (e = hipStreamWaitEvent(ctx->stream3, b->ev_fork, 0)) != hipSuccess) return e;
@@ -389,7 +406,7 @@
     if (timed && (e = hipEventRecord(b->ev[4], s)) != hipSuccess) return e;
     return hipSuccess;
 }
-struct SmallLayout { size_t sync, jobs, order, items, lean, tblist, bands, times, tabhdr, total_bands; bool any_lean; };
+struct SmallLayout { size_t sync, jobs, order, items, lean, tblist, bands, times, tabhdr, tiles, pc, need, total_bands, tile_cap; bool any_lean; };
 static SmallLayout layout_small(pgm_align_batch *b) {
     SmallLayout s;
     const uint32_t njobs = b->njobs;
@@ -401,6 +418,10 @@
     s.lean = SM.take(4 * (size_t)std::max(1u, njobs)); s.tblist = SM.take(8 * (size_t)std::max(1u, njobs));
     s.bands = SM.take(sizeof(PgmItem) * std::max<size_t>(1, s.total_bands)); s.times = SM.take(16 * (size_t)std::max(1u, njobs) + 16);
     s.tabhdr = SM.take(s.any_lean ? 4 * (size_t)PGM_TAB_HDR * njobs : 16);
+    s.tile_cap = 0;
+    for (const PgmJob &J : b->jobs) s.tile_cap += precompute_tile_bound(J, precompute_prep_nodes(alphabet_tier(b->maxdim)));
+    s.tiles = SM.take(sizeof(PgmTile) * std::max<size_t>(1, s.tile_cap));
+    s.pc = SM.take(4 * ((size_t)PGM_PC_JOBS + std::max(1u, njobs))); s.need = SM.take(4 * (size_t)std::max(1u, njobs));
     b->small_bytes = SM.bytes;
     return s;
 }
@@ -412,6 +433,7 @@
     hipError_t err = hipSuccess, host_err = hipSuccess;
     uint8_t *h_out_dev = nullptr;
     double ms_dev = 0, ms_host = 0, ms_slot[6] = {0, 0, 0, 0, 0, 0};
+    PrecomputeTiles tiles;
 };
 static void take_batch_buffers(pgm_ctx *ctx, pgm_align_batch *b, SmallLayout sm, BatchAlloc *A) {
     const double ta0 = now_ms();
@@ -432,17 +454,22 @@
         b->d_bands = (PgmItem *)(b->d_small + sm.bands);
         b->d_times = (unsigned long long *)(b->d_small + sm.times);
         b->d_tabhdr = sm.any_lean ? (int *)(b->d_small + sm.tabhdr) : nullptr;
+        b->d_tiles = (PgmTile *)(b->d_small + sm.tiles);
+        b->d_pc = (uint32_t *)(b->d_small + sm.pc);
+        b->d_need = (uint32_t *)(b->d_small + sm.need);
     }
     A->err = e2;
     A->state.store(e2 == hipSuccess ? 1 : -1, std::memory_order_release);
     A->ms_dev = now_ms() - ta0;
     if (e2 == hipSuccess) {
         hipError_t e3 = cache_take(ctx, pgm_ctx::C_HOST, b->out_bytes + 64, (void **)&b->h_out, &b->cap[pgm_ctx::C_HOST]);
-        if (e3 == hipSuccess) b->h_flag = (int *)(b->h_out + (b->out_bytes + 15) / 16 * 16);
+        if (e3 == hipSuccess) { b->h_flag = (int *)(b->h_out + (b->out_bytes + 15) / 16 * 16); b->h_clk = (unsigned long long *)(b->h_flag + 2); }
         if (e3 == hipSuccess) e3 = hipHostGetDevicePointer((void **)&A->h_out_dev, b->h_out, 0);
+        if (e3 == hipSuccess) b->h_aux_dev = A->h_out_dev + ((uint8_t *)b->h_flag - b->h_out);
         A->host_err = e3;
     }
     A->ms_host = now_ms() - ta0 - A->ms_dev;
+    if (e2 == hipSuccess && b->njobs) A->tiles = precompute_tiles(b->jobs, b->order, alphabet_tier(b->maxdim), nullptr, 0u);
 }
 
 struct CreateGuard {
@@ -545,6 +572,24 @@
     return PGM_OK;
 }
 
+int pgm_test_precompute_tiles(uint32_t njobs, const pgm_graph *const *g1, const pgm_graph *const *g2, const pgm_model *const *model,
+                              const pgm_scores *scores, uint32_t flags, const pgm_site_ref *res1, const pgm_site_ref *res2, uint32_t cus,
+                              uint32_t *head, uint32_t *tiles, uint32_t cap) {
+    if (!head || (cap && !tiles) || (njobs && (!g1 || !g2 || !model || !scores))) return fail(PGM_ERR_INVALID, "null argument");
+    std::vector<char> two_chains(njobs, 0);
+    for (uint32_t i = 0; i < njobs; ++i) two_chains[i] = job_is_two_chains(g1[i], g2[i]) ? 1 : 0;
+    std::vector<PgmJob> jobs;
+    BatchSizes Z;
+    const int invalid = plan_sizes(njobs, g1, g2, model, scores, flags, res1, res2, two_chains, cus, jobs, Z);
+    if (invalid >= 0) return fail(PGM_ERR_INVALID, "invalid job " + std::to_string(invalid));
+    const uint32_t tier = alphabet_tier(Z.maxdim);
+    const PrecomputeTiles P = precompute_tiles(jobs, size_order(jobs), tier, nullptr, 0u);
+    head[0] = (uint32_t)P.tiles.size(); head[1] = P.nprep; head[2] = njobs ? precompute_prep_nodes(tier) : 0u; head[3] = PGM_EM_TB;
+    static_assert(sizeof(PgmTile) == 12, "a packed tile is three words");
+    if (P.tiles.size() <= cap && !P.tiles.empty()) memcpy(tiles, P.tiles.data(), sizeof(PgmTile) * P.tiles.size());
+    return PGM_OK;
+}
+
 int pgm_align_batch_create(pgm_ctx *ctx, uint32_t njobs, const pgm_graph *const *g1, const pgm_graph *const *g2,
                            const pgm_model *const *model, const pgm_scores *scores, pgm_align_batch **out) {
     return pgm_align_batch_create_ex(ctx, njobs, g1, g2, model, scores, 0u, out);
@@ -584,6 +629,7 @@
     b->s_bytes = std::max<size_t>(Z.L.SL.bytes, 16);
     b->lq_off = (uint32_t)Z.L.sync_ints;
     b->sync_ints = Z.L.sync_ints + 3 * (((size_t)njobs + 3) / 4 * 4);
+    b->order = size_order(b->jobs);
     const double tc0 = now_ms();
     const SmallLayout sm = layout_small(b);
     G.alloc = std::thread(take_batch_buffers, ctx, b, sm, &A);
@@ -616,7 +662,6 @@
     if (A.err != hipSuccess) return fail(A.err == hipErrorOutOfMemory ? PGM_ERR_NOMEM : PGM_ERR_DEVICE, std::string("hipMalloc: ") + hipGetErrorString(A.err));
     if (A.host_err != hipSuccess) return fail(PGM_ERR_DEVICE, std::string("hipHostMalloc: ") + hipGetErrorString(A.host_err));
     bind_job_pointers(b, Z.off, res1, res2, A.h_out_dev);
-    b->order = size_order(b->jobs);
     b->sched = plan_schedule(b->jobs, b->order, cus);
     const BatchSchedule &S = b->sched;
     if (cprof && njobs)
@@ -632,10 +677,32 @@
         (e = hipMemcpyAsync(b->d_lean, S.lean_list.data(), 4 * S.lean_list.size(), hipMemcpyHostToDevice, ctx->stream)) != hipSuccess ||
         (e = hipMemcpyAsync(b->d_bands, S.bands.data(), sizeof(PgmItem) * S.bands.size(), hipMemcpyHostToDevice, ctx->stream)) != hipSuccess ||
         (e = classify_lean_jobs(ctx, b)) != hipSuccess ||
+        (e = hipMemsetAsync(b->d_pc, 0, 4 * ((size_t)PGM_PC_JOBS + njobs), ctx->stream)) != hipSuccess ||
         (e = hipStreamSynchronize(ctx->stream)) != hipSuccess)
         return fail(PGM_ERR_DEVICE, std::string("upload: ") + hipGetErrorString(e));
+    if (njobs) {
+        PrecomputeTiles &P = A.tiles;
+        if (b->d_tabhdr) {
+            const size_t tab_bytes = 4 * (size_t)PGM_TAB_HDR * njobs;
+            std::vector<int> tab_own;
+            int *tab = (int *)b->h_in;
+            if (tab_bytes > b->cap[pgm_ctx::C_HIN]) { tab_own.resize((size_t)PGM_TAB_HDR * njobs); tab = tab_own.data(); }
+            if ((e = hipMemcpyAsync(tab, b->d_tabhdr, tab_bytes, hipMemcpyDeviceToHost, ctx->stream)) != hipSuccess || (e = hipStreamSynchronize(ctx->stream)) != hipSuccess)
+                return fail(PGM_ERR_DEVICE, std::string("class headers: ") + hipGetErrorString(e));
+            bool any_table = false;
+            for (uint32_t i = 0; i < njobs && !any_table; ++i) any_table = b->jobs[i].lean && !b->jobs[i].keep_cells && tab[(size_t)PGM_TAB_HDR * i] == 0;
+            if (any_table) P = precompute_tiles(b->jobs, b->order, alphabet_tier(b->maxdim), tab, PGM_TAB_HDR);
+        }
+        if (P.tiles.size() > sm.tile_cap) return fail(PGM_ERR_DEVICE, "tile list longer than its bound");
+        b->ntiles = (uint32_t)P.tiles.size(); b->nprep = P.nprep;
+        b->pc_grid = precompute_grid(ctx, alphabet_tier(b->maxdim), b->ntiles);
+        if ((e = hipMemcpyAsync(b->d_tiles, P.tiles.data(), sizeof(PgmTile) * P.tiles.size(), hipMemcpyHostToDevice, ctx->stream)) != hipSuccess ||
+            (e = hipMemcpyAsync(b->d_need, P.need.data(), 4 * (size_t)njobs, hipMemcpyHostToDevice, ctx->stream)) != hipSuccess ||
+            (e = hipStreamSynchronize(ctx->stream)) != hipSuccess)
+            return fail(PGM_ERR_DEVICE, std::string("tile list: ") + hipGetErrorString(e));
+    }
     for (int k = 0; k < 5; ++k) (void)hipEventCreate(&b->ev[k]);
-    (void)hipEventCreateWithFlags(&b->ev_fork, hipEventDisableTiming);
+    (void)hipEventCreate(&b->ev_fork);
     (void)hipEventCreateWithFlags(&b->ev_join, hipEventDisableTiming);
     (void)hipEventCreateWithFlags(&b->ev_join_b, hipEventDisableTiming);
     (void)hipEventCreateWithFlags(&b->ev_join_c, hipEventDisableTiming);
@@ -649,6 +716,19 @@
     return PGM_OK;
 }
 
+static hipError_t launch_times(pgm_align_batch *b, float ms[4]) {
+    float head = 0;
+    hipError_t e;
+    if ((e = hipEventElapsedTime(&head, b->ev[0], b->ev_fork)) != hipSuccess || (e = hipEventElapsedTime(&ms[2], b->ev_fork, b->ev[3])) != hipSuccess ||
+        (e = hipEventElapsedTime(&ms[3], b->ev[3], b->ev[4])) != hipSuccess)
+        return e;
+    const unsigned long long c0 = __atomic_load_n(&b->h_clk[0], __ATOMIC_RELAXED), c1 = __atomic_load_n(&b->h_clk[1], __ATOMIC_RELAXED);
+    const float prep = c1 > c0 ? (float)((double)(c1 - c0) * 1e-5) : 0.0f;
+    ms[0] = std::min(prep, head);
+    ms[1] = head - ms[0];
+    return hipSuccess;
+}
+
 int pgm_align_batch_run(pgm_ctx *ctx, pgm_align_batch *b) {
     if (!ctx || !b) return fail(PGM_ERR_INVALID, "null argument");
     if (b->njobs == 0) return PGM_OK;
@@ -667,11 +747,9 @@
         HIPCHK(launch_all(ctx, b, true));
         b->ev_pending = false;
         HIPCHK(hipEventSynchronize(b->ev[4]));
-        for (int k = 0; k < 4; ++k) {
-            float ms = 0;
-            HIPCHK(hipEventElapsedTime(&ms, b->ev[k], b->ev[k + 1]));
-            acc[k] += ms;
-        }
+        float ms[4] = {0, 0, 0, 0};
+        HIPCHK(launch_times(b, ms));
+        for (int k = 0; k < 4; ++k) acc[k] += ms[k];
     }
     if (ms_prep) *ms_prep = (float)(acc[0] / reps);
     if (ms_emission) *ms_emission = (float)(acc[1] / reps);
@@ -723,14 +801,16 @@
     HIPCHK(hipStreamSynchronize(ctx->stream));
     if (b->ev_pending) {
         b->ev_pending = false;
-        float ms[3] = {0, 0, 0};
-        bool ok = true;
-        for (int k = 0; k < 3; ++k) ok = ok && hipEventElapsedTime(&ms[k], b->ev[k], b->ev[k + 1]) == hipSuccess;
-        if (ok) { for (int k = 0; k < 3; ++k) b->acc_ms[k] += ms[k]; ++b->acc_n; }
+        float ms[4] = {0, 0, 0, 0};
+        if (launch_times(b, ms) == hipSuccess) { for (int k = 0; k < 3; ++k) b->acc_ms[k] += ms[k]; ++b->acc_n; }
         else (void)hipGetLastError();
     }
-    const int aborted = *b->h_flag;
-    if (aborted) return fail(PGM_ERR_DEVICE, "fill kernel: a band hand-off timed out");
+    const int aborted = b->h_flag[0] | __atomic_load_n(&b->h_flag[1], __ATOMIC_RELAXED);
+    if (aborted) {
+        (void)hipMemset(b->d_pc, 0, 4 * ((size_t)PGM_PC_JOBS + b->njobs));
+        b->pc_epoch = 0;
+        return fail(PGM_ERR_DEVICE, b->h_flag[1] ? "precompute kernel: a wait for a job's prep tiles timed out" : "fill kernel: a band hand-off timed out");
+    }
     for (uint32_t i = 0; i < b->njobs; ++i) {
         PgmJob::Result res;
         memcpy(&res, b->h_out + b->res_off[i], sizeof res);
diff --git a/prographmsa_amd/csrc/pgm_device.h b/prographmsa_amd/csrc/pgm_device.h
--- a/prographmsa_amd/csrc/pgm_device.h
+++ b/prographmsa_amd/csrc/pgm_device.h
@@ -9,6 +9,7 @@
 #define PGM_ROWS 64
 #define PGM_VL 16
 #define PGM_BLOCK 8
+#define PGM_EM_TB 4
 #define PGM_NRING 128
 #define PGM_KF 4
 #define PGM_KF8 8
@@ -142,6 +143,11 @@
     return lo + w > lcols ? lcols - w : lo;
 }
 
+#define PGM_TILE_JOB 0x3fffffffu
+struct PgmTile {
+    uint32_t job, a, b;
+};
+
 struct PgmItem {
     uint32_t job, band;
     uint32_t prio, count;
diff --git a/prographmsa_amd/csrc/pgm_plan.h b/prographmsa_amd/csrc/pgm_plan.h
--- a/prographmsa_amd/csrc/pgm_plan.h
+++ b/prographmsa_amd/csrc/pgm_plan.h
@@ -353,6 +353,52 @@
     return -1;
 }
 
+inline uint32_t precompute_prep_nodes(uint32_t tier) { return tier == 64u ? 64u : 256u; }
+struct PrecomputeTiles {
+    std::vector<PgmTile> tiles;
+    std::vector<uint32_t> need;
+    uint32_t nprep = 0;
+};
+inline size_t precompute_tile_bound(const PgmJob &J, uint32_t nodes) {
+    const size_t nvb = (size_t)J.nb << J.rshift;
+    return (J.n1 + (size_t)nodes - 1) / nodes + (J.n2 + (size_t)nodes - 1) / nodes + (nvb + 3) / 4 * ((J.nblk + (size_t)PGM_EM_TB - 1) / PGM_EM_TB);
+}
+static PrecomputeTiles precompute_tiles(const std::vector<PgmJob> &jobs, const std::vector<uint32_t> &order, uint32_t tier, const int *tab, uint32_t tab_stride) {
+    PrecomputeTiles P;
+    const uint32_t nodes = precompute_prep_nodes(tier);
+    P.need.assign(jobs.size(), 0u);
+    auto table_scored = [&](uint32_t i) { return tab && jobs[i].lean && !jobs[i].keep_cells && tab[(size_t)tab_stride * i] == 0; };
+    for (uint32_t i : order) {
+        const PgmJob &J = jobs[i];
+        const bool table = table_scored(i);
+        for (uint32_t side = 0; side < 2; ++side) {
+            const uint32_t n = side ? J.n2 : J.n1, nc = J.dim + 2u;
+            for (uint32_t sl = 0; sl * nodes < n; ++sl) {
+                if (table) {
+                    const uint32_t v0 = sl * nodes;
+                    bool any = n - 1u >= v0 && n - 1u < v0 + nodes;
+                    for (uint32_t c = 0; c < nc && !any; ++c) {
+                        const uint32_t r = (uint32_t)tab[(size_t)tab_stride * i + 1u + (side ? nc : 0u) + c];
+                        any = r != 0u && r - 1u >= v0 && r - 1u < v0 + nodes;
+                    }
+                    if (!any) continue;
+                }
+                P.tiles.push_back(PgmTile{i | (side ? PGM_TILE_SIDE2 : 0u), sl, 0u});
+                ++P.need[i];
+            }
+        }
+    }
+    P.nprep = (uint32_t)P.tiles.size();
+    for (uint32_t i : order) {
+        const PgmJob &J = jobs[i];
+        if (table_scored(i)) continue;
+        const uint32_t nvb = J.nb << J.rshift;
+        for (uint32_t bg = 0; 4u * bg < nvb; ++bg)
+            for (uint32_t tg = 0; tg * PGM_EM_TB < J.nblk; ++tg) P.tiles.push_back(PgmTile{i | PGM_TILE_EMISSION, tg, bg});
+    }
+    return P;
+}
+
 static bool plan_job_sweep(PgmJob &J, uint8_t *base, SideOff &s1, SideOff &s2, const BatchPrologue &P) {
     J.has_extras = (s1.nodes_with_extras + s2.nodes_with_extras) > 0 ? 1u : 0u;
     if (J.lean && J.has_extras) return false;
```

New measurement: 80.79. Within noise of the previous version (-0.4%).
